# salesforce/LayoutDETR

Measured on AMD Instinct MI355X. Metric: images/sec G+D fwd-bwd, 256x256 bg x9 elems, higher is better.
Workload: dtype f32

## Files before the change

include/ldetr_hip.h:

```cpp
#ifndef LDETR_HIP_H
#define LDETR_HIP_H

#include <stdint.h>

#ifdef __cplusplus
extern "C" {
#endif

const char* ldetr_last_error(void);
int ldetr_abi_version(void);

int ldetr_debug_trace_tiles(int64_t* buffer);

int ldetr_set_split_bf16(int tiles);

int ldetr_engine_launch_counts(int64_t* f32_pipe, int64_t* bf16_split_pipe);

int ldetr_set_workspace(void* ptr, int64_t bytes);

typedef struct ldetr_tensor4 {
    int N, C, H, W;
    int64_t sn, sc, sh, sw;
} ldetr_tensor4;

typedef struct ldetr_epilogue {
    float alpha;
    const float* col_scale;
    const float* col_bias;
    const float* samp_scale;
    int64_t samp_ld;
    const float* residual;
    int64_t ldr;
    int act;
    float act_alpha;
    float act_gain;
    const float* mask_src;
    int64_t ldm;
    int mask_mode;
    float out_scale;
    float p_drop;
    uint64_t seed;
    const uint64_t* seed_ptr;
    int accumulate;
    float* a_rowsum;
} ldetr_epilogue;

int ldetr_bias_act_f32(const float* x, const float* b, const float* xref, const float* yref, const float* dy, float* y,
                       int64_t sizeX, int sizeB, int64_t stepB, int grad, int act, float alpha, float gain, float clamp,
                       void* stream);

int ldetr_upfirdn2d_f32(const float* x, const float* f, float* y, int N, int C, int inH, int inW,
                        const int64_t* x_strides_nchw, int fh, int fw, int64_t f_stride_h, int64_t f_stride_w,
                        int upx, int upy, int downx, int downy, int padx0, int padx1, int pady0, int pady1, int flip,
                        float gain, int outH, int outW, const int64_t* y_strides_nchw,
                        const float* act_bias, int has_act, float act_alpha, float act_gain, void* stream);

int ldetr_gemm_f32(const float* A, int64_t lda, int ta, const float* B, int64_t ldb, int tb, float* C, int64_t ldc,
                   int M, int N, int K, int splitk, const ldetr_epilogue* ep, int pix_per_sample, void* stream);

typedef struct ldetr_gemm_desc {
    const float* A; int64_t lda; int ta;
    const float* B; int64_t ldb; int tb;
    float* C; int64_t ldc;
    int M, N, K, splitk;
    const ldetr_epilogue* ep;
    int pix_per_sample;
} ldetr_gemm_desc;
int ldetr_gemm_pair_f32(const ldetr_gemm_desc* g0, const ldetr_gemm_desc* g1, void* stream);
int ldetr_gemm_pair_is_single_launch(const ldetr_gemm_desc* g0, const ldetr_gemm_desc* g1);

#define LDETR_GEMM_GROUP_MAX 32
int ldetr_gemm_small_group_f32(const ldetr_gemm_desc* g, const float* post_scale, int n, void* stream);

int ldetr_conv2d_fwd_f32(const float* x, const ldetr_tensor4* xt, const float* w, int Cout, int KH, int KW, int stride,
                         int pad, float* y, int64_t ldy, int OH, int OW, const float* in_scale, int64_t in_scale_ld,
                         const ldetr_epilogue* ep, void* stream);
int ldetr_conv2d_bwd_data_f32(const float* dy, const ldetr_tensor4* dyt, const float* w, int Cin, int KH, int KW,
                              int stride, int pad, float* dx, int64_t lddx, int IH, int IW, const float* dy_scale,
                              int64_t dy_scale_ld, const ldetr_epilogue* ep, void* stream);
int ldetr_conv2d_bwd_weight_f32(const float* x, const ldetr_tensor4* xt, const float* dy, const ldetr_tensor4* dyt,
                                float* dw, int KH, int KW, int stride, int pad, int splitk, const float* x_scale,
                                int64_t x_scale_ld, const float* dy_scale, int64_t dy_scale_ld, int accumulate, void* stream);

int ldetr_conv_transpose2d_fwd_f32(const float* x, const ldetr_tensor4* xt, const float* w, int Cout, int KH, int KW,
                                   int stride, int pad, float* y, int64_t ldy, int OH, int OW, const float* in_scale,
                                   int64_t in_scale_ld, const ldetr_epilogue* ep, void* stream);
int ldetr_conv_transpose2d_bwd_data_f32(const float* dy, const ldetr_tensor4* dyt, const float* w, int Cin, int KH,
                                        int KW, int stride, int pad, float* dx, int64_t lddx, int IH, int IW,
                                        const float* dy_scale, int64_t dy_scale_ld, const ldetr_epilogue* ep,
                                        void* stream);
int ldetr_conv_transpose2d_bwd_weight_f32(const float* x, const ldetr_tensor4* xt, const float* dy,
                                          const ldetr_tensor4* dyt, float* dw, int KH, int KW, int stride, int pad,
                                          int splitk, const float* x_scale, int64_t x_scale_ld, const float* dy_scale,
                                          int64_t dy_scale_ld, int accumulate, void* stream);

int ldetr_attention_fwd_f32(const float* q, int64_t ldq, const float* k, int64_t ldk, const float* v, int64_t ldv,
                            const unsigned char* key_padding_mask, float* out, int64_t ldo, float* lse, int B, int H,
                            int Lq, int Lk, int head_dim, float scale, float p_drop, uint64_t seed, const uint64_t* seed_ptr,
                            int causal, void* stream);
int ldetr_attention_bwd_f32(const float* q, int64_t ldq, const float* k, int64_t ldk, const float* v, int64_t ldv,
                            const unsigned char* key_padding_mask, const float* out, int64_t ldo, const float* lse,
                            const float* dout, int64_t lddo, float* dq, int64_t lddq, float* dk, int64_t lddk,
                            float* dv, int64_t lddv, int B, int H, int Lq, int Lk, int head_dim, float scale,
                            float p_drop, uint64_t seed, const uint64_t* seed_ptr, int causal, void* stream);

int ldetr_torgb_bwd_finish_f32(const float* dws, const float* s, const float* w, int B, int C, float* dw, float* ds, void* stream);

int ldetr_loss_combine_fwd_f32(const float* const* x, const float* w, const int* n, const int* fn, const int* red, int K, int ld,
                               float* vals, float* sums, float* total, void* stream);
int ldetr_loss_combine_bwd_f32(const float* const* x, const float* w, const int* n, const int* fn, const int* red, int K, int ld,
                               const float* g, float* grads, void* stream);
int ldetr_masked_mse_fwd_f32(const float* a, const float* b, const uint8_t* valid, int64_t rows, int D, int bdiv, float* out2, void* stream);
int ldetr_masked_mse_bwd_f32(const float* a, const float* b, const uint8_t* valid, int64_t rows, int D, int bdiv, const float* out2,
                             const float* g, float* da, void* stream);

typedef struct ldetr_ln_args {
    const float* x; const float* r; const float* gamma; const float* beta;
    float* y; float* z; float* mean; float* rstd;
    const float* dy; float* dx; float* dr; float* dgamma; float* dbeta;
    int64_t rows; int D; float eps, p_drop; uint64_t seed; const uint64_t* seed_ptr;
    const float* pos; int64_t pos_rows; float* ypos; const float* dy2;
    int r_parts; int64_t r_part_stride; const float* r_bias;
    const float* dy_parts; int dy_nparts; int64_t dy_part_stride;
} ldetr_ln_args;
int ldetr_layernorm_fwd_group_f32(const ldetr_ln_args* a, int n, void* stream);
int ldetr_layernorm_bwd_group_f32(const ldetr_ln_args* a, int n, void* stream);
int ldetr_sum_parts_f32(const float* base, const float* parts, int n_parts, int64_t part_stride, float* out, int64_t n, void* stream);

typedef struct ldetr_ffn_args {
    const float* x; int64_t ldx;
    const float* w1; const float* b1;
    const float* w2;
    float* h;
    float* ypart;
    int M, F;
    float p_drop; uint64_t seed; const uint64_t* seed_ptr;
    const float* dy;
    float* dxpart;
    float* dh;
} ldetr_ffn_args;
int ldetr_ffn_fwd_group_f32(const ldetr_ffn_args* a, int n, void* stream);
int ldetr_ffn_bwd_group_f32(const ldetr_ffn_args* a, int n, void* stream);

typedef struct ldetr_mha_small_args {
    const float* x; int64_t ldx;
    const float* w_in; const float* b_in; const float* w_out;
    const unsigned char* kpm;
    float* qkv; float* o; float* lse; float* ypart;
    int B, L;
    float scale, p_drop; uint64_t seed; const uint64_t* seed_ptr;
    const float* dr;
    float* dqkv; float* dxpart;
} ldetr_mha_small_args;
int ldetr_mha_small_fwd_group_f32(const ldetr_mha_small_args* a, int n, void* stream);
int ldetr_mha_small_bwd_group_f32(const ldetr_mha_small_args* a, int n, void* stream);

typedef struct ldetr_mha_cross_args {
    const float* x; int64_t ldx;
    const float* w_q; const float* b_q;
    const float* k; int64_t ldk; const float* v; int64_t ldv;
    const float* w_out;
    const unsigned char* kpm;
    float* q; float* o; float* lse; float* ypart;
    int B, Lq, Lk;
    float scale, p_drop; uint64_t seed; const uint64_t* seed_ptr;
    const float* dr;
    float* dq; float* dk; int64_t lddk; float* dv; int64_t lddv; float* dxpart;
} ldetr_mha_cross_args;
int ldetr_mha_cross_fwd_f32(const ldetr_mha_cross_args* a, void* stream);
int ldetr_mha_cross_bwd_f32(const ldetr_mha_cross_args* a, void* stream);

typedef struct ldetr_wgrad_desc {
    const float* A; int64_t lda; const float* B; int64_t ldb;
    float* dW; int64_t ldw; float* db;
    int M, rows, cols;
} ldetr_wgrad_desc;
int ldetr_wgrad_multi_f32(const ldetr_wgrad_desc* d, int n, void* stream);

int ldetr_colsum_f32(const float* a, float* red, int B, int64_t P, int C, void* stream);
int ldetr_act_bwd_reduce_f32(const float* dy, const float* y, float* dv, const float* bias, const float* demod,
                             float* dbias, float* ddemod, int B, int64_t P, int C, int act, float alpha, float gain,
                             void* stream);
int ldetr_mul_reduce_f32(const float* a, const float* x, const float* scale, float* out, float* red, int B, int64_t P,
                         int C, void* stream);
int ldetr_torgb_fwd_f32(const float* x, const float* w, const float* styles, const float* bias, float* y,
                        int B, int64_t P, int C, void* stream);
int ldetr_torgb_fwd_add_f32(const float* x, const float* w, const float* styles, const float* bias, const float* addend, float* y,
                            int B, int64_t P, int C, void* stream);
int ldetr_torgb_bwd_f32(const float* x, const float* dy, const float* w, const float* styles, float* dx, float* dws,
                        float* dbias, int B, int64_t P, int C, void* stream);
int ldetr_sg2_handoff_f32(const float* dxs, const float* x, const float* dy_rgb, float* dv, const float* s_conv, const float* s_rgb,
                          const float* w_rgb, const float* bias, const float* demod, float* ds_conv, float* dws_rgb, float* dbias_rgb,
                          float* dbias, float* ddemod, int B, int64_t P, int C, float alpha, float gain, void* stream);

int ldetr_maxpool3x3s2_fwd_f32(const float* x, float* y, unsigned char* idx, int N, int H, int W, int C, void* stream);
int ldetr_maxpool3x3s2_bwd_f32(const float* dy, const unsigned char* idx, float* dx, int N, int H, int W, int C,
                               void* stream);

int ldetr_grad_sanitize_f32(float* g, int64_t n, float scale, float nan_value, float posinf, float neginf,
                            void* stream);
int ldetr_adam_step_f32(float* p, const float* g, float* m, float* v, int64_t n, int64_t step, float lr, float beta1,
                        float beta2, float eps, int fuse_sanitize, float gscale, float nan_value, float posinf,
                        float neginf, void* stream);
int ldetr_adam_ema_step_f32(float* p, const float* g, float* m, float* v, int64_t n, int64_t step, float lr, float beta1, float beta2,
                            float eps, int fuse_sanitize, float gscale, float nan_value, float posinf, float neginf,
                            float* p_ema, float ema_beta, void* stream);
int ldetr_ema_lerp_f32(float* p_ema, const float* p, int64_t n, float beta, void* stream);

int ldetr_softmax_xent_fwd_f32(const float* logits, int64_t ld, const int64_t* targets, float* row_lse, float* loss_sum, float* count,
                               int64_t rows, int V, int64_t ignore_index, float label_smoothing, void* stream);
int ldetr_softmax_xent_bwd_f32(const float* logits, int64_t ld, const int64_t* targets, const float* row_lse, const float* count,
                               const float* grad_out, float* dlogits, int64_t ldd, int64_t rows, int V, int64_t ignore_index,
                               float label_smoothing, void* stream);

int ldetr_embedding_fwd_f32(const float* weight, const float* pos, const int64_t* ids, float* out, int64_t n, int d, int V, int T,
                            void* stream);
int ldetr_embedding_bwd_f32(const float* dy, const int64_t* ids, float* dweight, int64_t n, int d, int V, int64_t padding_idx,
                            void* stream);

int ldetr_resample_coeffs(int in_size, int out_size, int32_t* bounds, int32_t* weights, int64_t weights_capacity, int* ksize_out);
int ldetr_resize_normalize_u8(const uint8_t* src, int64_t images, int H, int W, int out_h, int out_w, const int32_t* hbounds,
                              const int32_t* hweights, int hksize, const int32_t* vbounds, const int32_t* vweights, int vksize,
                              uint8_t* tmp, uint8_t* out_u8, float* out_chw, float mean0, float mean1, float mean2, float std0,
                              float std1, float std2, void* stream);

#define LDETR_PAGE_FILTER_BLUR 1
#define LDETR_PAGE_FILTER_EDGE 2
int ldetr_page_filter_u8(const uint8_t* src, uint8_t* dst, int64_t images, int H, int W, int kind, float radius, void* stream);

int ldetr_demod_fwd_f32(const float* weight, int64_t so, int64_t si, int64_t sh, int64_t sw, const float* styles, float* dcoefs,
                        float* w2, int B, int O, int I, int KH, int KW, float eps, void* stream);
int ldetr_demod_bwd_f32(const float* weight, int64_t so, int64_t si, int64_t sh, int64_t sw, const float* styles, const float* dcoefs,
                        const float* w2, const float* grad_dcoefs, float* dweight, int accumulate_dweight, float* dstyles, int B, int O,
                        int I, int KH, int KW, void* stream);

#define LDETR_DEMOD_GROUP_MAX 24
typedef struct ldetr_demod_desc {
    const float* weight; int64_t so, si, sh, sw;
    const float* styles; float* dcoefs; float* w2;
    const float* grad_dcoefs; float* dweight; float* dstyles;
    int O, I, KH, KW;
} ldetr_demod_desc;
int ldetr_demod_group_fwd_f32(const ldetr_demod_desc* layers, int n, int B, float eps, void* stream);
int ldetr_demod_group_bwd_f32(const ldetr_demod_desc* layers, int n, int B, int accumulate_dweight, int add_dstyles, void* stream);

#define LDETR_AFFINE_GROUP_MAX 32
typedef struct ldetr_affine_desc {
    const float* ds; const float* A; float* dA; float* db;
    int C; float scale; float post;
} ldetr_affine_desc;
int ldetr_sg2_affine_bwd_f32(const ldetr_affine_desc* layers, int n, const float* latent, float* dlatent, int accumulate_dlatent,
                             float* scratch, int64_t scratch_floats, int B, int D, void* stream);

int ldetr_layout_losses_f32(const float* bbox, const float* bbox_ref, const uint8_t* valid, int B, int N, float* losses,
                            float* grads, void* stream);
int ldetr_layout_losses_bwd_f32(const float* grads, const float* grad_losses, int B, int N, float* dbbox, void* stream);

int ldetr_layout_finish_f32(const float* bbox_in, const int* num, const float* factors, const unsigned char* jitter, const unsigned char* mode,
                            float* bbox_out, float* overlap, float* alignment, int* order, int C, int K, int N, void* stream);

#define LDETR_FILTER_BILINEAR 0
#define LDETR_FILTER_LANCZOS 1
typedef struct ldetr_layout_raster_args {
    int struct_bytes;
    int B, N, S, nrow, n_colors, n_pages;
    const float* bbox;
    const uint8_t* valid;
    const int32_t* labels;
    const uint8_t* palette;
    const int32_t* page_wh;
    const uint8_t* pages;
    int64_t pages_bytes;
    const int64_t* page_table;
    const int32_t* page_index;
    const int32_t* coeffs;
    int64_t coeffs_len;
    const int64_t* cell_coeffs;
    int32_t* cells_dev;
    uint8_t* out;
} ldetr_layout_raster_args;
int ldetr_resample_coeffs_filter(int filter, int in_size, int out_size, int32_t* bounds, int32_t* weights, int64_t weights_capacity, int* ksize_out);
int ldetr_layout_raster_cell_size(int W, int H, int S, int* wn_out, int* hn_out);
int ldetr_layout_raster_u8(const ldetr_layout_raster_args* a, void* stream);

typedef struct ldetr_patch_resize_args {
    int struct_bytes;
    int n_jobs;
    const uint8_t* src0;
    int64_t src0_bytes;
    const uint8_t* src1;
    int64_t src1_bytes;
    uint8_t* dst;
    int64_t dst_bytes;
    const int64_t* jobs;
    const int32_t* tables;
    const int32_t* tables_host;
    int64_t tables_len;
    int32_t* jobs_dev;
} ldetr_patch_resize_args;
typedef struct ldetr_image_raster_args {
    int struct_bytes;
    int B, N, S, nrow;
    const float* bbox;
    const uint8_t* valid;
    const int32_t* rects;
    const int64_t* patch_off;
    const int64_t* page_off;
    const int32_t* page_wh;
    const uint8_t* pixels;
    int64_t pixels_bytes;
    const int32_t* coeffs;
    int64_t coeffs_len;
    const int64_t* cell_coeffs;
    int32_t* cells_dev;
    uint8_t* out;
} ldetr_image_raster_args;
int ldetr_patch_resize_u8(const ldetr_patch_resize_args* a, void* stream);
int ldetr_image_raster_u8(const ldetr_image_raster_args* a, void* stream);

#define LDETR_PNG_NOT_ELIGIBLE 3
#define LDETR_PNG_MALFORMED 4
typedef struct ldetr_png_decode_args {
    int struct_bytes;
    int n, H, W;
    int phases;
    int reserved;
    const uint8_t* files;
    int64_t files_bytes;
    const int64_t* file_off;
    const int64_t* file_off_dev;
    const int64_t* segments;
    const int64_t* segments_dev;
    int64_t n_segments;
    const int32_t* jobs;
    const int32_t* jobs_dev;
    int64_t n_jobs;
    uint8_t* scratch;
    int64_t scratch_bytes;
    uint8_t* dst;
} ldetr_png_decode_args;
int ldetr_png_scan(const uint8_t* file, int64_t file_bytes, int* width, int* height, int* channels, int64_t* segments, int64_t segments_capacity,
                   int64_t* segments_count, int32_t* row_starts, int64_t row_starts_capacity, int64_t* row_starts_count);
int ldetr_png_decode_u8(const ldetr_png_decode_args* a, void* stream);

typedef struct ldetr_png_encode_args {
    int struct_bytes;
    int H, W;
    int blocks;
    int filter;
    int reserved;
    const uint8_t* src;
    uint8_t* out;
    int64_t out_capacity;
    int64_t* total_bytes;
    uint8_t* workspace;
    int64_t workspace_bytes;
    int64_t* seg_table;
    int64_t seg_table_rows;
} ldetr_png_encode_args;
int ldetr_png_encode_bound(int H, int W, int64_t* out_bytes, int64_t* workspace_bytes);
int ldetr_png_encode_u8(const ldetr_png_encode_args* a, void* stream);
int ldetr_png_index_bytes(int H, int W, int64_t* bytes);

#define LDETR_PNG_INFLATE_CODE 1
#define LDETR_PNG_INFLATE_COUNT 2
#define LDETR_PNG_INFLATE_HEADER 4
#define LDETR_PNG_INFLATE_DISTANCE 8
#define LDETR_PNG_INFLATE_TRAILER 16
#define LDETR_PNG_INFLATE_FILTER 32
#define LDETR_PNG_INFLATE_STUCK 64
#define LDETR_PNG_INFLATE_TABLE 128
typedef struct ldetr_png_inflate_args {
    int struct_bytes;
    int n, H, W;
    int phases;
    int reserved;
    const uint8_t* files;
    int64_t files_bytes;
    const int64_t* file_off;
    const int64_t* file_off_dev;
    const int64_t* segments;
    const int64_t* segments_dev;
    const int64_t* index_off;
    const int64_t* index_off_dev;
    const int32_t* jobs;
    const int32_t* jobs_dev;
    int64_t n_jobs;
    uint8_t* scratch;
    int64_t scratch_bytes;
    uint8_t* dst;
    int32_t* status;
} ldetr_png_inflate_args;
int ldetr_png_scan_packed(const uint8_t* file, int64_t file_bytes, int* width, int* height, int64_t* segments, int64_t segments_capacity, int64_t* segments_count,
                          int64_t* index_offset, int32_t* row_starts, int64_t row_starts_capacity, int64_t* row_starts_count);
int ldetr_png_inflate_u8(const ldetr_png_inflate_args* a, void* stream);

int ldetr_lsap_f64(const double* cost, int batch, int n, int maximize, int* row_ind, int* col_ind, void* stream);

int ldetr_layoutnet_features_f32(const float* bbox, const int64_t* label, const uint8_t* padding_mask, const int* label_map, int map_len,
                                 const float* weights, int64_t weights_len, int num_label, int B, int N, float* out, void* stream);

int ldetr_layoutnet_forward_f32(const float* bbox, const int64_t* label, const uint8_t* padding_mask, const float* enc_weights,
                                int64_t enc_len, const float* dec_weights, int64_t dec_len, int num_label, int B, int N,
                                float* logit_disc, float* logit_cls, float* bbox_pred, float* features, void* stream);

int ldetr_feature_stats_f64(const float* x, int64_t n, int F, double* raw_mean, double* raw_cov, void* stream);

int ldetr_box_giou_pairwise_f32(const float* boxes1, const float* boxes2, int B, int N, int M, int cxcywh, float* iou, float* uni,
                                float* giou, double* cost, double cost_sign, void* stream);

int ldetr_bmm_strided_f32(const float* A, const int64_t* sa, const float* B, const int64_t* sb, float* C, const int64_t* sc,
                          int nb1, int nb2, int M, int N, int K, float alpha, void* stream);

int ldetr_p3_split_f32(const float* src, int64_t ld, void* dst, int64_t rows, int C, void* stream);
int ldetr_p3_merge_f32(const void* src, float* dst, int64_t ld, int64_t rows, int C, void* stream);
int ldetr_p3_weight_bwd(const float* w_ohwi, const float* o_scale, void* dst, int O, int KH, int KW, int I, void* stream);

int ldetr_p3_weight_prep(const int64_t* table_dev, int nconv, int total_blocks, void* stream);

typedef struct ldetr_p3_epilogue {
    float alpha;
    const float* col_scale;
    const float* col_bias;
    const void* residual_p3;
    const float* residual_f32;
    const void* relu_mask_p3;
    int relu;
} ldetr_p3_epilogue;

int ldetr_p3_conv2d_fwd(const void* x, int N, int H, int W, int Cin, const void* w, int Cout, int KH, int KW, int stride, int pad,
                        const ldetr_p3_epilogue* ep, void* out_p3, float* out_f32, void* stream);
int ldetr_p3_conv2d_fwd_dual(const void* x1, const void* x2, int N, int H, int W, int Cin, const void* w1, const void* w2, int Cout, int KH, int KW,
                             int stride, int pad, const ldetr_p3_epilogue* ep1, const ldetr_p3_epilogue* ep2, void* out1_p3, float* out1_f32,
                             void* out2_p3, float* out2_f32, void* stream);
int ldetr_p3_conv2d_bwd_data(const void* dy, int N, int OH, int OW, int Cout, const void* wb, int Cin, int KH, int KW, int stride, int pad,
                             int IH, int IW, const ldetr_p3_epilogue* ep, void* out_p3, float* out_f32, void* stream);
int ldetr_p3_conv2d_bwd_weight(const void* x, int N, int H, int W, int Cin, const void* dy, int Cout, int KH, int KW, int stride, int pad,
                               const float* dy_scale, float* dw, void* stream);
int ldetr_p3_conv2d_bwd_pair(const void* dy, int N, int OH, int OW, int Cout, const void* wb, const void* x, int Cin, int KH, int KW, int stride, int pad,
                             int IH, int IW, const ldetr_p3_epilogue* ep, void* dx_p3, float* dx_f32, const float* dy_scale, float* dw,
                             int* launches, void* stream);

int ldetr_struct_sizes(int32_t* out6);

int ldetr_p3_last_launch(int32_t* info10);

int ldetr_engine_last_launch(int32_t* info10);

#ifdef __cplusplus
}
#endif
#endif
```

layoutdetr_amd/_lib.py:

```python
import ctypes
import os
from ctypes import (POINTER, Structure, c_char_p, c_double, c_float, c_int, c_int64, c_ubyte, c_uint64, c_void_p)

_HERE = os.path.dirname(os.path.abspath(__file__))
ABI_VERSION = 25
LIB_PATH = os.environ.get('LDETR_LIB') or os.path.join(_HERE, 'lib', 'libldetr_hip.so')


class Tensor4(Structure):
    _fields_ = [('N', c_int), ('C', c_int), ('H', c_int), ('W', c_int),
                ('sn', c_int64), ('sc', c_int64), ('sh', c_int64), ('sw', c_int64)]


class GemmDesc(Structure):
    _fields_ = [('A', c_void_p), ('lda', c_int64), ('ta', c_int), ('B', c_void_p), ('ldb', c_int64), ('tb', c_int),
                ('C', c_void_p), ('ldc', c_int64), ('M', c_int), ('N', c_int), ('K', c_int), ('splitk', c_int),
                ('ep', c_void_p), ('pix_per_sample', c_int)]


class P3Epilogue(Structure):
    _fields_ = [('alpha', c_float), ('col_scale', c_void_p), ('col_bias', c_void_p), ('residual_p3', c_void_p),
                ('residual_f32', c_void_p), ('relu_mask_p3', c_void_p), ('relu', c_int)]


class Epilogue(Structure):
    _fields_ = [('alpha', c_float), ('col_scale', c_void_p), ('col_bias', c_void_p), ('samp_scale', c_void_p),
                ('samp_ld', c_int64), ('residual', c_void_p), ('ldr', c_int64), ('act', c_int),
                ('act_alpha', c_float), ('act_gain', c_float), ('mask_src', c_void_p), ('ldm', c_int64),
                ('mask_mode', c_int), ('out_scale', c_float), ('p_drop', c_float), ('seed', c_uint64),
                ('seed_ptr', c_void_p), ('accumulate', c_int), ('a_rowsum', c_void_p)]


class LnArgs(Structure):
    _fields_ = [('x', c_void_p), ('r', c_void_p), ('gamma', c_void_p), ('beta', c_void_p),
                ('y', c_void_p), ('z', c_void_p), ('mean', c_void_p), ('rstd', c_void_p),
                ('dy', c_void_p), ('dx', c_void_p), ('dr', c_void_p), ('dgamma', c_void_p), ('dbeta', c_void_p),
                ('rows', c_int64), ('D', c_int), ('eps', c_float), ('p_drop', c_float), ('seed', c_uint64), ('seed_ptr', c_void_p),
                ('pos', c_void_p), ('pos_rows', c_int64), ('ypos', c_void_p), ('dy2', c_void_p),
                ('r_parts', c_int), ('r_part_stride', c_int64), ('r_bias', c_void_p),
                ('dy_parts', c_void_p), ('dy_nparts', c_int), ('dy_part_stride', c_int64)]


class FfnArgs(Structure):
    _fields_ = [('x', c_void_p), ('ldx', c_int64), ('w1', c_void_p), ('b1', c_void_p), ('w2', c_void_p), ('h', c_void_p), ('ypart', c_void_p),
                ('M', c_int), ('F', c_int), ('p_drop', c_float), ('seed', c_uint64), ('seed_ptr', c_void_p),
                ('dy', c_void_p), ('dxpart', c_void_p), ('dh', c_void_p)]


class MhaSmallArgs(Structure):
    _fields_ = [('x', c_void_p), ('ldx', c_int64), ('w_in', c_void_p), ('b_in', c_void_p), ('w_out', c_void_p), ('kpm', c_void_p),
                ('qkv', c_void_p), ('o', c_void_p), ('lse', c_void_p), ('ypart', c_void_p), ('B', c_int), ('L', c_int),
                ('scale', c_float), ('p_drop', c_float), ('seed', c_uint64), ('seed_ptr', c_void_p),
                ('dr', c_void_p), ('dqkv', c_void_p), ('dxpart', c_void_p)]


class MhaCrossArgs(Structure):
    _fields_ = [('x', c_void_p), ('ldx', c_int64), ('w_q', c_void_p), ('b_q', c_void_p), ('k', c_void_p), ('ldk', c_int64), ('v', c_void_p), ('ldv', c_int64),
                ('w_out', c_void_p), ('kpm', c_void_p), ('q', c_void_p), ('o', c_void_p), ('lse', c_void_p), ('ypart', c_void_p),
                ('B', c_int), ('Lq', c_int), ('Lk', c_int), ('scale', c_float), ('p_drop', c_float), ('seed', c_uint64), ('seed_ptr', c_void_p),
                ('dr', c_void_p), ('dq', c_void_p), ('dk', c_void_p), ('lddk', c_int64), ('dv', c_void_p), ('lddv', c_int64), ('dxpart', c_void_p)]


class WgradDesc(Structure):
    _fields_ = [('A', c_void_p), ('lda', c_int64), ('B', c_void_p), ('ldb', c_int64), ('dW', c_void_p), ('ldw', c_int64), ('db', c_void_p),
                ('M', c_int), ('rows', c_int), ('cols', c_int)]


class DemodDesc(Structure):
    _fields_ = [('weight', c_void_p), ('so', c_int64), ('si', c_int64), ('sh', c_int64), ('sw', c_int64),
                ('styles', c_void_p), ('dcoefs', c_void_p), ('w2', c_void_p), ('grad_dcoefs', c_void_p), ('dweight', c_void_p), ('dstyles', c_void_p),
                ('O', c_int), ('I', c_int), ('KH', c_int), ('KW', c_int)]


class AffineDesc(Structure):
    _fields_ = [('ds', c_void_p), ('A', c_void_p), ('dA', c_void_p), ('db', c_void_p), ('C', c_int), ('scale', c_float), ('post', c_float)]


class LayoutRasterArgs(Structure):
    _fields_ = [('struct_bytes', c_int), ('B', c_int), ('N', c_int), ('S', c_int), ('nrow', c_int), ('n_colors', c_int), ('n_pages', c_int),
                ('bbox', c_void_p), ('valid', c_void_p), ('labels', c_void_p), ('palette', c_void_p), ('page_wh', c_void_p),
                ('pages', c_void_p), ('pages_bytes', c_int64), ('page_table', c_void_p), ('page_index', c_void_p),
                ('coeffs', c_void_p), ('coeffs_len', c_int64), ('cell_coeffs', c_void_p), ('cells_dev', c_void_p), ('out', c_void_p)]


class PatchResizeArgs(Structure):
    _fields_ = [('struct_bytes', c_int), ('n_jobs', c_int), ('src0', c_void_p), ('src0_bytes', c_int64), ('src1', c_void_p), ('src1_bytes', c_int64),
                ('dst', c_void_p), ('dst_bytes', c_int64), ('jobs', c_void_p), ('tables', c_void_p), ('tables_host', c_void_p), ('tables_len', c_int64),
                ('jobs_dev', c_void_p)]


class ImageRasterArgs(Structure):
    _fields_ = [('struct_bytes', c_int), ('B', c_int), ('N', c_int), ('S', c_int), ('nrow', c_int),
                ('bbox', c_void_p), ('valid', c_void_p), ('rects', c_void_p), ('patch_off', c_void_p), ('page_off', c_void_p), ('page_wh', c_void_p),
                ('pixels', c_void_p), ('pixels_bytes', c_int64), ('coeffs', c_void_p), ('coeffs_len', c_int64), ('cell_coeffs', c_void_p),
                ('cells_dev', c_void_p), ('out', c_void_p)]


class PngDecodeArgs(Structure):
    _fields_ = [('struct_bytes', c_int), ('n', c_int), ('H', c_int), ('W', c_int), ('phases', c_int), ('reserved', c_int),
                ('files', c_void_p), ('files_bytes', c_int64), ('file_off', c_void_p), ('file_off_dev', c_void_p),
                ('segments', c_void_p), ('segments_dev', c_void_p), ('n_segments', c_int64),
                ('jobs', c_void_p), ('jobs_dev', c_void_p), ('n_jobs', c_int64),
                ('scratch', c_void_p), ('scratch_bytes', c_int64), ('dst', c_void_p)]


class PngEncodeArgs(Structure):
    _fields_ = [('struct_bytes', c_int), ('H', c_int), ('W', c_int), ('blocks', c_int), ('filter', c_int), ('reserved', c_int),
                ('src', c_void_p), ('out', c_void_p), ('out_capacity', c_int64), ('total_bytes', c_void_p),
                ('workspace', c_void_p), ('workspace_bytes', c_int64), ('seg_table', c_void_p), ('seg_table_rows', c_int64)]


class PngInflateArgs(Structure):
    _fields_ = [('struct_bytes', c_int), ('n', c_int), ('H', c_int), ('W', c_int), ('phases', c_int), ('reserved', c_int),
                ('files', c_void_p), ('files_bytes', c_int64), ('file_off', c_void_p), ('file_off_dev', c_void_p),
                ('segments', c_void_p), ('segments_dev', c_void_p), ('index_off', c_void_p), ('index_off_dev', c_void_p),
                ('jobs', c_void_p), ('jobs_dev', c_void_p), ('n_jobs', c_int64),
                ('scratch', c_void_p), ('scratch_bytes', c_int64), ('dst', c_void_p), ('status', c_void_p)]


_P = c_void_p
_I = c_int
_L = c_int64
_F = c_float
_T4 = POINTER(Tensor4)
_EP = POINTER(Epilogue)

SIGNATURES = {
    'ldetr_set_workspace': [_P, _L],
    'ldetr_bias_act_f32': [_P, _P, _P, _P, _P, _P, _L, _I, _L, _I, _I, _F, _F, _F, _P],
    'ldetr_upfirdn2d_f32': [_P, _P, _P, _I, _I, _I, _I, POINTER(c_int64), _I, _I, _L, _L, _I, _I, _I, _I, _I, _I, _I, _I,
                            _I, _F, _I, _I, POINTER(c_int64), _P, _I, _F, _F, _P],
    'ldetr_gemm_f32': [_P, _L, _I, _P, _L, _I, _P, _L, _I, _I, _I, _I, _EP, _I, _P],
    'ldetr_conv2d_fwd_f32': [_P, _T4, _P, _I, _I, _I, _I, _I, _P, _L, _I, _I, _P, _L, _EP, _P],
    'ldetr_conv2d_bwd_data_f32': [_P, _T4, _P, _I, _I, _I, _I, _I, _P, _L, _I, _I, _P, _L, _EP, _P],
    'ldetr_conv2d_bwd_weight_f32': [_P, _T4, _P, _T4, _P, _I, _I, _I, _I, _I, _P, _L, _P, _L, _I, _P],
    'ldetr_conv_transpose2d_fwd_f32': [_P, _T4, _P, _I, _I, _I, _I, _I, _P, _L, _I, _I, _P, _L, _EP, _P],
    'ldetr_conv_transpose2d_bwd_data_f32': [_P, _T4, _P, _I, _I, _I, _I, _I, _P, _L, _I, _I, _P, _L, _EP, _P],
    'ldetr_conv_transpose2d_bwd_weight_f32': [_P, _T4, _P, _T4, _P, _I, _I, _I, _I, _I, _P, _L, _P, _L, _I, _P],
    'ldetr_attention_fwd_f32': [_P, _L, _P, _L, _P, _L, _P, _P, _L, _P, _I, _I, _I, _I, _I, _F, _F, c_uint64, _P, _I, _P],
    'ldetr_attention_bwd_f32': [_P, _L, _P, _L, _P, _L, _P, _P, _L, _P, _P, _L, _P, _L, _P, _L, _P, _L,
                                _I, _I, _I, _I, _I, _F, _F, c_uint64, _P, _I, _P],
    'ldetr_colsum_f32': [_P, _P, _I, _L, _I, _P],
    'ldetr_act_bwd_reduce_f32': [_P, _P, _P, _P, _P, _P, _P, _I, _L, _I, _I, _F, _F, _P],
    'ldetr_mul_reduce_f32': [_P, _P, _P, _P, _P, _I, _L, _I, _P],
    'ldetr_torgb_fwd_f32': [_P, _P, _P, _P, _P, _I, _L, _I, _P],
    'ldetr_torgb_bwd_f32': [_P, _P, _P, _P, _P, _P, _P, _I, _L, _I, _P],
    'ldetr_maxpool3x3s2_fwd_f32': [_P, _P, _P, _I, _I, _I, _I, _P],
    'ldetr_maxpool3x3s2_bwd_f32': [_P, _P, _P, _I, _I, _I, _I, _P],
    'ldetr_grad_sanitize_f32': [_P, _L, _F, _F, _F, _F, _P],
    'ldetr_adam_step_f32': [_P, _P, _P, _P, _L, _L, _F, _F, _F, _F, _I, _F, _F, _F, _F, _P],
    'ldetr_adam_ema_step_f32': [_P, _P, _P, _P, _L, _L, _F, _F, _F, _F, _I, _F, _F, _F, _F, _P, _F, _P],
    'ldetr_ema_lerp_f32': [_P, _P, _L, _F, _P],
    'ldetr_lsap_f64': [_P, _I, _I, _I, _P, _P, _P],
    'ldetr_layoutnet_features_f32': [_P, _P, _P, POINTER(c_int), _I, _P, _L, _I, _I, _I, _P, _P],
    'ldetr_layoutnet_forward_f32': [_P, _P, _P, _P, _L, _P, _L, _I, _I, _I, _P, _P, _P, _P, _P],
    'ldetr_feature_stats_f64': [_P, _L, _I, _P, _P, _P],
    'ldetr_box_giou_pairwise_f32': [_P, _P, _I, _I, _I, _I, _P, _P, _P, _P, c_double, _P],
    'ldetr_bmm_strided_f32': [_P, _P, _P, _P, _P, _P, _I, _I, _I, _I, _I, _F, _P],
    'ldetr_softmax_xent_fwd_f32': [_P, _L, _P, _P, _P, _P, _L, _I, _L, _F, _P],
    'ldetr_softmax_xent_bwd_f32': [_P, _L, _P, _P, _P, _P, _P, _L, _L, _I, _L, _F, _P],
    'ldetr_embedding_fwd_f32': [_P, _P, _P, _P, _L, _I, _I, _I, _P],
    'ldetr_embedding_bwd_f32': [_P, _P, _P, _L, _I, _I, _L, _P],
    'ldetr_debug_trace_tiles': [_P],
    'ldetr_set_split_bf16': [c_int],
    'ldetr_engine_launch_counts': [POINTER(c_int64), POINTER(c_int64)],
    'ldetr_layernorm_fwd_group_f32': [_P, _I, _P],
    'ldetr_layernorm_bwd_group_f32': [_P, _I, _P],
    'ldetr_sum_parts_f32': [_P, _P, _I, _L, _P, _L, _P],
    'ldetr_ffn_fwd_group_f32': [_P, _I, _P],
    'ldetr_ffn_bwd_group_f32': [_P, _I, _P],
    'ldetr_mha_small_fwd_group_f32': [_P, _I, _P],
    'ldetr_mha_small_bwd_group_f32': [_P, _I, _P],
    'ldetr_mha_cross_fwd_f32': [_P, _P],
    'ldetr_mha_cross_bwd_f32': [_P, _P],
    'ldetr_wgrad_multi_f32': [_P, _I, _P],
    'ldetr_loss_combine_fwd_f32': [_P, _P, _P, _P, _P, _I, _I, _P, _P, _P, _P],
    'ldetr_loss_combine_bwd_f32': [_P, _P, _P, _P, _P, _I, _I, _P, _P, _P],
    'ldetr_masked_mse_fwd_f32': [_P, _P, _P, _L, _I, _I, _P, _P],
    'ldetr_masked_mse_bwd_f32': [_P, _P, _P, _L, _I, _I, _P, _P, _P, _P],
    'ldetr_torgb_bwd_finish_f32': [_P, _P, _P, _I, _I, _P, _P, _P],
    'ldetr_sg2_handoff_f32': [_P, _P, _P, _P, _P, _P, _P, _P, _P, _P, _P, _P, _P, _P, _I, _L, _I, _F, _F, _P],
    'ldetr_gemm_pair_f32': [_P, _P, _P],
    'ldetr_gemm_pair_is_single_launch': [_P, _P],
    'ldetr_demod_fwd_f32': [_P, _L, _L, _L, _L, _P, _P, _P, _I, _I, _I, _I, _I, _F, _P],
    'ldetr_demod_bwd_f32': [_P, _L, _L, _L, _L, _P, _P, _P, _P, _P, _I, _P, _I, _I, _I, _I, _I, _P],
    'ldetr_demod_group_fwd_f32': [_P, _I, _I, _F, _P],
    'ldetr_demod_group_bwd_f32': [_P, _I, _I, _I, _I, _P],
    'ldetr_sg2_affine_bwd_f32': [_P, _I, _P, _P, _I, _P, _L, _I, _I, _P],
    'ldetr_gemm_small_group_f32': [_P, _P, _I, _P],
    'ldetr_torgb_fwd_add_f32': [_P, _P, _P, _P, _P, _P, _I, _L, _I, _P],
    'ldetr_layout_losses_f32': [_P, _P, _P, _I, _I, _P, _P, _P],
    'ldetr_layout_losses_bwd_f32': [_P, _P, _I, _I, _P, _P],
    'ldetr_layout_finish_f32': [_P, _P, _P, _P, _P, _P, _P, _P, _P, _I, _I, _I, _P],
    'ldetr_resample_coeffs': [_I, _I, _P, _P, _L, _P],
    'ldetr_resample_coeffs_filter': [_I, _I, _I, _P, _P, _L, _P],
    'ldetr_layout_raster_cell_size': [_I, _I, _I, _P, _P],
    'ldetr_layout_raster_u8': [_P, _P],
    'ldetr_patch_resize_u8': [_P, _P],
    'ldetr_image_raster_u8': [_P, _P],
    'ldetr_p3_split_f32': [_P, _L, _P, _L, _I, _P],
    'ldetr_p3_merge_f32': [_P, _P, _L, _L, _I, _P],
    'ldetr_p3_weight_bwd': [_P, _P, _P, _I, _I, _I, _I, _P],
    'ldetr_p3_conv2d_bwd_data': [_P, _I, _I, _I, _I, _P, _I, _I, _I, _I, _I, _I, _I, _P, _P, _P, _P],
    'ldetr_p3_conv2d_fwd': [_P, _I, _I, _I, _I, _P, _I, _I, _I, _I, _I, _P, _P, _P, _P],
    'ldetr_p3_conv2d_bwd_weight': [_P, _I, _I, _I, _I, _P, _I, _I, _I, _I, _I, _P, _P, _P],
    'ldetr_p3_weight_prep': [_P, _I, _I, _P],
    'ldetr_p3_conv2d_fwd_dual': [_P, _P, _I, _I, _I, _I, _P, _P, _I, _I, _I, _I, _I, _P, _P, _P, _P, _P, _P, _P],
    'ldetr_p3_conv2d_bwd_pair': [_P, _I, _I, _I, _I, _P, _P, _I, _I, _I, _I, _I, _I, _I, _P, _P, _P, _P, _P, _P, _P],
    'ldetr_p3_last_launch': [_P],
    'ldetr_engine_last_launch': [_P],
    'ldetr_struct_sizes': [_P],
    'ldetr_resize_normalize_u8': [_P, _L, _I, _I, _I, _I, _P, _P, _I, _P, _P, _I, _P, _P, _P, _F, _F, _F, _F, _F, _F, _P],
    'ldetr_page_filter_u8': [_P, _P, _L, _I, _I, _I, _F, _P],
    'ldetr_png_scan': [_P, _L, _P, _P, _P, _P, _L, _P, _P, _L, _P],
    'ldetr_png_decode_u8': [_P, _P],
    'ldetr_png_encode_bound': [_I, _I, _P, _P],
    'ldetr_png_encode_u8': [_P, _P],
    'ldetr_png_index_bytes': [_I, _I, _P],
    'ldetr_png_scan_packed': [_P, _L, _P, _P, _P, _L, _P, _P, _P, _L, _P],
    'ldetr_png_inflate_u8': [_P, _P],
}

_lib = None


def load():
    global _lib
    if _lib is not None:
        return _lib
    if not os.path.exists(LIB_PATH):
        raise RuntimeError(
            f'{LIB_PATH} not found: build the gfx950 kernels first (python -m layoutdetr_amd.build or '
            f'__graft_entry__.build()).  layoutdetr_amd has no CPU/PyTorch fallback path.')
    import torch
    lib = ctypes.CDLL(LIB_PATH)
    lib.ldetr_last_error.restype = c_char_p
    lib.ldetr_last_error.argtypes = []
    lib.ldetr_abi_version.restype = c_int
    lib.ldetr_abi_version.argtypes = []
    for name, argtypes in SIGNATURES.items():
        fn = getattr(lib, name)
        fn.restype = c_int
        fn.argtypes = argtypes
    if lib.ldetr_abi_version() != ABI_VERSION:
        raise RuntimeError('libldetr_hip.so ABI version mismatch; rebuild it')
    sizes = (ctypes.c_int32 * 6)()
    lib.ldetr_struct_sizes(sizes)
    mirror = [ctypes.sizeof(t) for t in (LnArgs, FfnArgs, MhaSmallArgs, MhaCrossArgs, WgradDesc, P3Epilogue)]
    if list(sizes) != mirror:
        raise RuntimeError(f'libldetr_hip.so argument blocks {list(sizes)} do not match the ctypes mirror {mirror}; rebuild')
    _lib = lib
    return lib


def check(rc, what=''):
    if rc != 0:
        msg = load().ldetr_last_error().decode('utf-8', 'replace')
        raise RuntimeError(f'{what}: {msg}' if what else msg)
```

layoutdetr_amd/build.py:

```python
import hashlib
import os
import shutil
import subprocess
import sys
from concurrent.futures import ThreadPoolExecutor

HERE = os.path.dirname(os.path.abspath(__file__))
CSRC = os.path.join(HERE, 'csrc')
LIBDIR = os.path.join(HERE, 'lib')
OBJDIR = os.path.join(LIBDIR, 'obj')
LIBNAME = 'libldetr_hip.so'
ARCH = 'gfx950'

SOURCES = ['ldetr_core.cpp', 'bias_act.hip', 'upfirdn2d.hip', 'gemm_conv.hip', 'attention.hip', 'layernorm.hip',
           'misc_ops.hip', 'optim.hip', 'lsap.hip', 'xent.hip', 'resample.hip', 'layout_loss.hip', 'demod.hip', 'sg2_affine.hip', 'wgrad_smallc.hip', 'stem_conv.hip', 'box_ops.hip', 'ffn_fused.hip', 'conv_c32.hip', 'mha_small.hip', 'p3_engine.hip', 'bmm_strided.hip', 'layoutnet.hip', 'layoutnet_train.hip', 'layout_finish.hip', 'layout_raster.hip', 'page_filter.hip', 'patch_resize.hip', 'png_decode.hip', 'png_encode.hip', 'png_inflate.hip']
HEADERS = ['ldetr_common.hpp', 'layoutnet_layers.hpp', 'pil_resample.hpp', 'png_pages.hpp', 'png_inflate_kernel.hpp', os.path.join('..', '..', 'include', 'ldetr_hip.h')]

FLAGS = ([] if os.environ.get('LDETR_TILE_TRACE') else ['-DLDETR_TILE_TRACE=0']) + (['-DP3_TRACE'] if os.environ.get('LDETR_P3_TRACE') else []) + ['-O3', '-std=c++17', '-fPIC', f'--offload-arch={ARCH}', '-munsafe-fp-atomics', '-fno-gpu-rdc',
         '-Wno-unused-result', '-Rpass-analysis=kernel-resource-usage']
NO_SCRATCH = ('wgrad_c32_3x3_kernel', 'gemm_f32_kernel', 'gemm_small_kernel', 'gemm_small_group_kernel', 'demod_group', 'sg2_affine_bwd', 'attn_fwd_kernel', 'attn_fwd_wide_kernel', 'attn_bwd_kernel', 'ffn_fwd_kernel', 'ffn_bwd_kernel', 'conv3x3_c32_kernel', 'mha_small_fwd_kernel', 'mha_cross_fwd_kernel', 'mha_small_bwd_kernel', 'mha_cross_bwd_kernel', 'wgrad_multi_kernel', 'ln_fwd_kernel', 'ln_bwd_kernel', 'p3_nt_kernel', 'p3_tn_kernel', 'p3_c3_kernel', 'p3_bwd_pair', 'layoutnet_features_kernel', 'layoutnet_forward_kernel', 'feature_stats_f64_kernel', 'layout_finish_kernel', 'layout_raster_kernel', 'page_blur_kernel', 'page_edge_kernel', 'patch_resize_kernel', 'sg2_handoff_kernel', 'png_gather_kernel', 'png_unfilter_kernel', 'png_enc_filter_kernel', 'png_enc_deflate_kernel', 'png_enc_assemble_kernel', 'png_inflate_kernel')


def _hipcc():
    for cand in (os.environ.get('HIPCC'), shutil.which('hipcc'), '/opt/rocm/bin/hipcc'):
        if cand and os.path.exists(cand):
            return cand
    raise RuntimeError('hipcc not found: the gfx950 kernel library cannot be built')


def _digest(paths):
    h = hashlib.sha256()
    for p in paths:
        with open(p, 'rb') as f:
            h.update(f.read())
    h.update(' '.join(FLAGS).encode())
    return h.hexdigest()


def _kernel_resources(remarks):
    out, cur = {}, None
    for line in remarks.splitlines():
        if 'remark:' not in line:
            continue
        body = line.split('remark:', 1)[1].split('[-Rpass-analysis', 1)[0].strip()
        if body.startswith('Function Name:'):
            cur = body.split(':', 1)[1].strip()
            out[cur] = {}
        elif cur is not None and ':' in body:
            k, v = body.rsplit(':', 1)
            out[cur][k.strip()] = v.strip()
    return out


def source_digest():
    return _digest(sorted(os.path.join(CSRC, f) for f in os.listdir(CSRC) if f.endswith(('.hip', '.cpp', '.hpp')) and not f.startswith('.'))
                   + [os.path.normpath(os.path.join(CSRC, HEADERS[-1]))])


def lib_path():
    return os.path.join(LIBDIR, LIBNAME)


def build(force=False, verbose=True):
    os.makedirs(OBJDIR, exist_ok=True)
    hipcc = _hipcc()
    hdrs = [os.path.normpath(os.path.join(CSRC, h)) for h in HEADERS]
    objs, jobs = [], []
    for src in SOURCES:
        sp = os.path.join(CSRC, src)
        obj = os.path.join(OBJDIR, src + '.o')
        stamp = obj + '.sha'
        dig = _digest([sp] + hdrs)
        objs.append(obj)
        if not force and os.path.exists(obj) and os.path.exists(stamp) and open(stamp).read() == dig:
            continue
        jobs.append((sp, obj, stamp, dig))

    def compile_one(job):
        sp, obj, stamp, dig = job
        cmd = [hipcc] + FLAGS + ['-x', 'hip', '-c', sp, '-o', obj]
        if verbose:
            print('[ldetr build]', os.path.basename(sp), flush=True)
        r = subprocess.run(cmd, capture_output=True, text=True)
        if r.returncode != 0:
            raise RuntimeError(f'hipcc failed for {sp}:\n{r.stdout}\n{r.stderr}')
        res = _kernel_resources(r.stderr)
        with open(obj + '.resources.txt', 'w') as f:
            for name, d in res.items():
                f.write(f"{name} vgprs={d.get('VGPRs', '?')} agprs={d.get('AGPRs', '?')} scratch={d.get('ScratchSize [bytes/lane]', '?')} "
                        f"occupancy={d.get('Occupancy [waves/SIMD]', '?')} lds={d.get('LDS Size [bytes/block]', '?')}\n")
        bad = [n for n, d in res.items() if any(k in n for k in NO_SCRATCH) and d.get('ScratchSize [bytes/lane]', '0') != '0']
        if bad:
            raise RuntimeError(f'{os.path.basename(sp)}: scratch memory in register-budgeted kernels: ' + ', '.join(bad[:4]))
        with open(stamp, 'w') as f:
            f.write(dig)

    if jobs:
        with ThreadPoolExecutor(max_workers=min(8, len(jobs))) as ex:
            list(ex.map(compile_one, jobs))
    out = lib_path()
    if jobs or not os.path.exists(out):
        cmd = [hipcc, '-shared', '-fPIC', f'--offload-arch={ARCH}', '-fno-gpu-rdc', '-o', out] + objs
        r = subprocess.run(cmd, capture_output=True, text=True)
        if r.returncode != 0:
            raise RuntimeError(f'link failed:\n{r.stdout}\n{r.stderr}')
        if verbose:
            print('[ldetr build] linked', out, flush=True)
    return out


if __name__ == '__main__':
    build(force='--force' in sys.argv)
```

layoutdetr_amd/csrc/ffn_fused.hip:

```cpp
#include "ldetr_common.hpp"
#include "../../include/ldetr_hip.h"

namespace ldetr {

typedef ldetr_ffn_args FfnParams;

constexpr int FD = 256, FHS = 64, FHP = 68;

typedef __attribute__((__vector_size__(16 * sizeof(float)))) float ffn_acc_t;

__device__ __forceinline__ void ld_k16(const __amdgpu_buffer_rsrc_t& rs, int voff, int soff, float (&f)[16]) {
#pragma unroll
    for (int j = 0; j < 4; j++) {
        const auto v = __builtin_amdgcn_raw_buffer_load_b128(rs, voff + 16 * j, soff, 0);
        f[4 * j] = __int_as_float(v[0]); f[4 * j + 1] = __int_as_float(v[1]); f[4 * j + 2] = __int_as_float(v[2]); f[4 * j + 3] = __int_as_float(v[3]);
    }
}
__device__ __forceinline__ void ld_r16(const __amdgpu_buffer_rsrc_t& rs, int voff, int soff, int ld4, float (&f)[16]) {
#pragma unroll
    for (int t = 0; t < 16; t++) f[t] = __int_as_float(__builtin_amdgcn_raw_buffer_load_b32(rs, voff, soff + t * ld4, 0));
}
__device__ __forceinline__ __amdgpu_buffer_rsrc_t rsrc(const float* p) {
    return __builtin_amdgcn_make_buffer_rsrc(const_cast<float*>(p), 0, 0x7fffffff, 0x00020000);
}
#define FFN_MFMA16(A, B, ACC) _Pragma("unroll") for (int t_ = 0; t_ < 16; t_++) ACC = __builtin_amdgcn_mfma_f32_32x32x2f32(A[t_], B[t_], ACC, 0, 0, 0)

__global__ __launch_bounds__(256) void ffn_fwd_kernel(FfnParams pa, FfnParams pb, int nb0) {
    __shared__ float red[2][32][33];
    __shared__ float Hs[32][FHP];
    const bool second = (int)blockIdx.x >= nb0;
    const FfnParams& p = second ? pb : pa;
    const int bid = second ? (int)blockIdx.x - nb0 : (int)blockIdx.x, gx = (p.M + 31) >> 5;
    const int tid = threadIdx.x, lane = tid & 63, wave = tid >> 6, cl = lane & 31, kl = lane >> 5;
    const int s = bid / gx, m0 = (bid - s * gx) * 32, j0 = s * FHS;
    const int OOB = (int)0x80000000;
    const int ct = wave & 1, kh = wave >> 1;
    float b2[2][2][16];
    {
        const __amdgpu_buffer_rsrc_t rsX = rsrc(p.x), rsW = rsrc(p.w1), rsW2 = rsrc(p.w2);
        const int vA = (m0 + cl < p.M) ? (int)(((long)(m0 + cl) * p.ldx + kh * 128 + 16 * kl) * 4) : OOB;
        const int vB = ((j0 + ct * 32 + cl) * FD + kh * 128 + 16 * kl) * 4;
        ffn_acc_t acc;
#pragma unroll
        for (int r = 0; r < 16; r++) acc[r] = 0.f;
        float a[4][16], b[4][16];
#pragma unroll
        for (int c = 0; c < 4; c++) { ld_k16(rsX, vA, c * 128, a[c]); ld_k16(rsW, vB, c * 128, b[c]); }
#pragma unroll
        for (int q = 0; q < 2; q++)
#pragma unroll
            for (int c = 0; c < 2; c++) ld_k16(rsW2, (((wave * 2 + q) * 32 + cl) * p.F + j0 + 16 * kl) * 4, c * 128, b2[q][c]);
        __builtin_amdgcn_sched_barrier(0);
#pragma unroll
        for (int c = 0; c < 4; c++) FFN_MFMA16(a[c], b[c], acc);
        if (kh == 1) {
#pragma unroll
            for (int r = 0; r < 16; r++) red[ct][(r & 3) + 8 * (r >> 2) + 4 * kl][cl] = acc[r];
        }
        __syncthreads();
        if (kh == 0) {
            const float bias = p.b1[j0 + ct * 32 + cl];
            const float inv_keep = p.p_drop > 0.f ? 1.f / (1.f - p.p_drop) : 1.f;
            const uint64_t seed = p.seed + (p.seed_ptr ? *p.seed_ptr : 0ull);
#pragma unroll
            for (int r = 0; r < 16; r++) {
                const int row = (r & 3) + 8 * (r >> 2) + 4 * kl;
                float v = acc[r] + red[ct][row][cl] + bias;
                v = v > 0.f ? v : 0.f;
                const long m = m0 + row;
                if (p.p_drop > 0.f) v *= drop_scale(seed, (uint64_t)(m * p.F + j0 + ct * 32 + cl), p.p_drop, inv_keep);
                Hs[row][ct * 32 + cl] = v;
                if (m < p.M) p.h[m * p.F + j0 + ct * 32 + cl] = v;
            }
        }
        __syncthreads();
    }
    {
        ffn_acc_t acc[2];
#pragma unroll
        for (int q = 0; q < 2; q++)
#pragma unroll
            for (int r = 0; r < 16; r++) acc[q][r] = 0.f;
#pragma unroll
        for (int c = 0; c < 2; c++) {
            float a[16];
#pragma unroll
            for (int t = 0; t < 16; t++) a[t] = Hs[cl][c * 32 + 16 * kl + t];
            FFN_MFMA16(a, b2[0][c], acc[0]);
            FFN_MFMA16(a, b2[1][c], acc[1]);
        }
        float* dst = p.ypart + ((long)s * p.M) * FD;
#pragma unroll
        for (int q = 0; q < 2; q++)
#pragma unroll
            for (int r = 0; r < 16; r++) {
                const long m = m0 + (r & 3) + 8 * (r >> 2) + 4 * kl;
                if (m < p.M) dst[m * FD + (wave * 2 + q) * 32 + cl] = acc[q][r];
            }
    }
}

__global__ __launch_bounds__(256) void ffn_bwd_kernel(FfnParams pa, FfnParams pb, int nb0) {
    __shared__ float red[2][32][33];
    __shared__ float dHs[32][FHP];
    const bool second = (int)blockIdx.x >= nb0;
    const FfnParams& p = second ? pb : pa;
    const int bid = second ? (int)blockIdx.x - nb0 : (int)blockIdx.x, gx = (p.M + 31) >> 5;
    const int tid = threadIdx.x, lane = tid & 63, wave = tid >> 6, cl = lane & 31, kl = lane >> 5;
    const int s = bid / gx, m0 = (bid - s * gx) * 32, j0 = s * FHS;
    const int OOB = (int)0x80000000;
    const __amdgpu_buffer_rsrc_t rsDY = rsrc(p.dy), rsW1 = rsrc(p.w1), rsW2 = rsrc(p.w2), rsX = rsrc(p.x);
    const float inv_keep = p.p_drop > 0.f ? 1.f / (1.f - p.p_drop) : 1.f;
    float b2[2][2][16];
    {
        const int ct = wave & 1, kh = wave >> 1;
        const int vA = (m0 + cl < p.M) ? ((m0 + cl) * FD + kh * 128 + 16 * kl) * 4 : OOB;
        const int vB = (j0 + ct * 32 + cl + (kh * 128 + 16 * kl) * p.F) * 4;
        const int ld4 = p.F * 4;
        ffn_acc_t acc;
#pragma unroll
        for (int r = 0; r < 16; r++) acc[r] = 0.f;
        float a[4][16], b[4][16];
#pragma unroll
        for (int c = 0; c < 4; c++) { ld_k16(rsDY, vA, c * 128, a[c]); ld_r16(rsW2, vB, c * 32 * ld4, ld4, b[c]); }
#pragma unroll
        for (int q = 0; q < 2; q++)
#pragma unroll
            for (int c = 0; c < 2; c++)
                ld_r16(rsW1, ((wave * 2 + q) * 32 + cl + (j0 + c * 32 + 16 * kl) * FD) * 4, 0, FD * 4, b2[q][c]);
        float hvs[16];
#pragma unroll
        for (int r = 0; r < 16; r++) {
            const long m = m0 + (r & 3) + 8 * (r >> 2) + 4 * kl;
            hvs[r] = (kh == 0 && m < p.M) ? p.h[m * p.F + j0 + ct * 32 + cl] : 0.f;
        }
        __builtin_amdgcn_sched_barrier(0);
#pragma unroll
        for (int c = 0; c < 4; c++) FFN_MFMA16(a[c], b[c], acc);
        if (kh == 1) {
#pragma unroll
            for (int r = 0; r < 16; r++) red[ct][(r & 3) + 8 * (r >> 2) + 4 * kl][cl] = acc[r];
        }
        __syncthreads();
        if (kh == 0) {
#pragma unroll
            for (int r = 0; r < 16; r++) {
                const int row = (r & 3) + 8 * (r >> 2) + 4 * kl;
                const long m = m0 + row;
                const float hv = hvs[r];
                const float dh = hv > 0.f ? (acc[r] + red[ct][row][cl]) * inv_keep : 0.f;
                dHs[row][ct * 32 + cl] = dh;
                if (p.dh && m < p.M) p.dh[m * p.F + j0 + ct * 32 + cl] = dh;
            }
        }
        __syncthreads();
    }
    {
        ffn_acc_t acc[2];
#pragma unroll
        for (int q = 0; q < 2; q++)
#pragma unroll
            for (int r = 0; r < 16; r++) acc[q][r] = 0.f;
#pragma unroll
        for (int c = 0; c < 2; c++) {
            float a[16];
#pragma unroll
            for (int t = 0; t < 16; t++) a[t] = dHs[cl][c * 32 + 16 * kl + t];
            FFN_MFMA16(a, b2[0][c], acc[0]);
            FFN_MFMA16(a, b2[1][c], acc[1]);
        }
        float* dst = p.dxpart + ((long)s * p.M) * FD;
#pragma unroll
        for (int q = 0; q < 2; q++)
#pragma unroll
            for (int r = 0; r < 16; r++) {
                const long m = m0 + (r & 3) + 8 * (r >> 2) + 4 * kl;
                if (m < p.M) dst[m * FD + (wave * 2 + q) * 32 + cl] = acc[q][r];
            }
    }
}

}

using namespace ldetr;

static int ffn_check_args(const char* what, const FfnParams& p, bool bwd) {
    LDETR_CHECK(p.F >= FHS && p.F % FHS == 0, "%s: hidden width must be a multiple of 64 (got %d)", what, p.F);
    LDETR_CHECK(p.M >= 0 && p.M <= (1 << 20), "%s: bad row count", what);
    LDETR_CHECK(p.x && p.ldx >= FD && p.ldx % 4 == 0 && (((uintptr_t)p.x) & 15) == 0, "%s: x must be 16-byte aligned rows with a pitch that is a multiple of 4", what);
    LDETR_CHECK((long)p.M * p.ldx * 4 < 0x7fffffffL && (long)p.M * p.F * 4 < 0x7fffffffL && (long)(p.F / FHS) * p.M * FD * 4 < 0x7fffffffL, "%s: operand above 2 GiB", what);
    if (!bwd) {
        LDETR_CHECK(p.w1 && p.b1 && p.w2 && p.h && p.ypart, "%s: null pointer", what);
        LDETR_CHECK(p.p_drop >= 0.f && p.p_drop < 1.f, "%s: p_drop out of range", what);
    } else {
        LDETR_CHECK(p.dy && p.h && p.w1 && p.w2 && p.dxpart, "%s: null pointer", what);
        LDETR_CHECK((((uintptr_t)p.dy) & 15) == 0, "%s: dy must be 16-byte aligned", what);
    }
    return LDETR_OK;
}

static int ffn_launch(const ldetr_ffn_args* a, int n, bool bwd, void* stream) {
    const char* what = bwd ? "ffn_bwd" : "ffn_fwd";
    LDETR_CHECK(a && (n == 1 || n == 2), "%s: 1 or 2 problems", what);
    FfnParams p[2]; p[0] = a[0]; p[1] = n == 2 ? a[1] : a[0];
    int nb[2] = {0, 0};
    for (int i = 0; i < n; i++) {
        if (int rc = ffn_check_args(what, p[i], bwd)) return rc;
        nb[i] = cdiv(p[i].M, 32) * (p[i].F / FHS);
    }
    if (nb[0] + nb[1] == 0) return LDETR_OK;
    if (bwd) hipLaunchKernelGGL(ffn_bwd_kernel, dim3(nb[0] + nb[1]), dim3(256), 0, (hipStream_t)stream, p[0], p[1], nb[0]);
    else hipLaunchKernelGGL(ffn_fwd_kernel, dim3(nb[0] + nb[1]), dim3(256), 0, (hipStream_t)stream, p[0], p[1], nb[0]);
    count_engine_launch(false);
    return check_launch(what);
}

extern "C" int ldetr_ffn_fwd_group_f32(const ldetr_ffn_args* a, int n, void* stream) { return ffn_launch(a, n, false, stream); }
extern "C" int ldetr_ffn_bwd_group_f32(const ldetr_ffn_args* a, int n, void* stream) { return ffn_launch(a, n, true, stream); }
```

layoutdetr_amd/csrc/layernorm.hip:

```cpp
#include "ldetr_common.hpp"
#include "../../include/ldetr_hip.h"

namespace ldetr {

typedef ldetr_ln_args LnParams;

template <int NV>
__global__ __launch_bounds__(256) void ln_fwd_kernel(LnParams pa, LnParams pb, int nb0) {
    const bool second = (int)blockIdx.x >= nb0;
    const LnParams& p = second ? pb : pa;
    const int lane = threadIdx.x & 63, wave = threadIdx.x >> 6;
    const long row = (long)(second ? (int)blockIdx.x - nb0 : (int)blockIdx.x) * 4 + wave;
    if (row >= p.rows) return;
    const int D4 = p.D >> 2;
    const float inv_keep = p.p_drop > 0.f ? 1.f / (1.f - p.p_drop) : 1.f;
    const uint64_t seed = p.seed + (p.seed_ptr ? *p.seed_ptr : 0ull);
    float4 v[NV];
    float s = 0.f;
#pragma unroll
    for (int i = 0; i < NV; i++) {
        int c4 = lane + i * 64;
        v[i] = make_float4(0.f, 0.f, 0.f, 0.f);
        if (c4 < D4) {
            v[i] = reinterpret_cast<const float4*>(p.x + row * p.D)[c4];
            if (p.r) {
                float4 rr = reinterpret_cast<const float4*>(p.r + row * p.D)[c4];
                if (p.r_parts > 0) {
                    if (p.r_bias) { const float4 bb = reinterpret_cast<const float4*>(p.r_bias)[c4]; rr.x += bb.x; rr.y += bb.y; rr.z += bb.z; rr.w += bb.w; }
                    constexpr int PW = NV == 1 ? 16 : 8;
                    for (int s = 1; s < p.r_parts; s += PW) {
                        float4 q[PW];
#pragma unroll
                        for (int j = 0; j < PW; j++)
                            q[j] = (s + j < p.r_parts) ? reinterpret_cast<const float4*>(p.r + (s + j) * p.r_part_stride + row * p.D)[c4] : make_float4(0.f, 0.f, 0.f, 0.f);
#pragma unroll
                        for (int j = 0; j < PW; j++)
                            if (s + j < p.r_parts) { rr.x += q[j].x; rr.y += q[j].y; rr.z += q[j].z; rr.w += q[j].w; }
                    }
                }
                if (p.p_drop > 0.f) {
                    uint64_t e = (uint64_t)row * p.D + (c4 << 2);
                    rr.x *= drop_scale(seed, e, p.p_drop, inv_keep);
                    rr.y *= drop_scale(seed, e + 1, p.p_drop, inv_keep);
                    rr.z *= drop_scale(seed, e + 2, p.p_drop, inv_keep);
                    rr.w *= drop_scale(seed, e + 3, p.p_drop, inv_keep);
                }
                v[i].x += rr.x; v[i].y += rr.y; v[i].z += rr.z; v[i].w += rr.w;
            }
            if (p.z) reinterpret_cast<float4*>(p.z + row * p.D)[c4] = v[i];
            s += v[i].x + v[i].y + v[i].z + v[i].w;
        }
    }
    const float mean = wave_sum(s) / p.D;
    float q = 0.f;
#pragma unroll
    for (int i = 0; i < NV; i++) {
        int c4 = lane + i * 64;
        if (c4 < D4) {
            float a = v[i].x - mean, b = v[i].y - mean, c = v[i].z - mean, d = v[i].w - mean;
            q += a * a + b * b + c * c + d * d;
        }
    }
    const float rstd = rsqrtf(wave_sum(q) / p.D + p.eps);
    if (lane == 0) { if (p.mean) p.mean[row] = mean; if (p.rstd) p.rstd[row] = rstd; }
#pragma unroll
    for (int i = 0; i < NV; i++) {
        int c4 = lane + i * 64;
        if (c4 < D4) {
            float4 g = reinterpret_cast<const float4*>(p.gamma)[c4];
            float4 b = reinterpret_cast<const float4*>(p.beta)[c4];
            float4 o;
            o.x = (v[i].x - mean) * rstd * g.x + b.x; o.y = (v[i].y - mean) * rstd * g.y + b.y;
            o.z = (v[i].z - mean) * rstd * g.z + b.z; o.w = (v[i].w - mean) * rstd * g.w + b.w;
            reinterpret_cast<float4*>(p.y + row * p.D)[c4] = o;
            if (p.ypos) {
                const float4 pp = reinterpret_cast<const float4*>(p.pos + (row % p.pos_rows) * p.D)[c4];
                o.x += pp.x; o.y += pp.y; o.z += pp.z; o.w += pp.w;
                reinterpret_cast<float4*>(p.ypos + row * p.D)[c4] = o;
            }
        }
    }
}

template <int NV, int WAVES>
__global__ __launch_bounds__(WAVES * 64) void ln_bwd_kernel(LnParams pa, LnParams pb, int nb0) {
    __shared__ float red[2][WAVES][256 * NV];
    const bool second = (int)blockIdx.x >= nb0;
    const LnParams& p = second ? pb : pa;
    const int bx = second ? (int)blockIdx.x - nb0 : (int)blockIdx.x, gx = second ? (int)gridDim.x - nb0 : nb0;
    const int lane = threadIdx.x & 63, wave = threadIdx.x >> 6;
    const int D4 = p.D >> 2;
    const float inv_keep = p.p_drop > 0.f ? 1.f / (1.f - p.p_drop) : 1.f;
    const uint64_t seed = p.seed + (p.seed_ptr ? *p.seed_ptr : 0ull);
    float4 ag[NV], ab[NV];
#pragma unroll
    for (int i = 0; i < NV; i++) { ag[i] = make_float4(0.f, 0.f, 0.f, 0.f); ab[i] = ag[i]; }
    for (long row = (long)bx * WAVES + wave; row < p.rows; row += (long)gx * WAVES) {
        const float mean = p.mean[row], rstd = p.rstd[row];
        float4 xh[NV], g[NV];
        float s1 = 0.f, s2 = 0.f;
#pragma unroll
        for (int i = 0; i < NV; i++) {
            int c4 = lane + i * 64;
            xh[i] = make_float4(0.f, 0.f, 0.f, 0.f); g[i] = xh[i];
            if (c4 < D4) {
                float4 zz = reinterpret_cast<const float4*>(p.z + row * p.D)[c4];
                float4 dy = reinterpret_cast<const float4*>(p.dy + row * p.D)[c4];
                if (p.dy2) {
                    const float4 d2 = reinterpret_cast<const float4*>(p.dy2 + row * p.D)[c4];
                    dy.x += d2.x; dy.y += d2.y; dy.z += d2.z; dy.w += d2.w;
                }
                constexpr int PW = NV == 1 ? 16 : 8;
                for (int s = 0; s < p.dy_nparts; s += PW) {
                    float4 q[PW];
#pragma unroll
                    for (int j = 0; j < PW; j++)
                        q[j] = (s + j < p.dy_nparts) ? reinterpret_cast<const float4*>(p.dy_parts + (s + j) * p.dy_part_stride + row * p.D)[c4] : make_float4(0.f, 0.f, 0.f, 0.f);
#pragma unroll
                    for (int j = 0; j < PW; j++)
                        if (s + j < p.dy_nparts) { dy.x += q[j].x; dy.y += q[j].y; dy.z += q[j].z; dy.w += q[j].w; }
                }
                float4 gm = reinterpret_cast<const float4*>(p.gamma)[c4];
                xh[i].x = (zz.x - mean) * rstd; xh[i].y = (zz.y - mean) * rstd;
                xh[i].z = (zz.z - mean) * rstd; xh[i].w = (zz.w - mean) * rstd;
                g[i].x = dy.x * gm.x; g[i].y = dy.y * gm.y; g[i].z = dy.z * gm.z; g[i].w = dy.w * gm.w;
                s1 += g[i].x + g[i].y + g[i].z + g[i].w;
                s2 += g[i].x * xh[i].x + g[i].y * xh[i].y + g[i].z * xh[i].z + g[i].w * xh[i].w;
                ag[i].x += dy.x * xh[i].x; ag[i].y += dy.y * xh[i].y; ag[i].z += dy.z * xh[i].z; ag[i].w += dy.w * xh[i].w;
                ab[i].x += dy.x; ab[i].y += dy.y; ab[i].z += dy.z; ab[i].w += dy.w;
            }
        }
        const float c1 = wave_sum(s1) / p.D, c2 = wave_sum(s2) / p.D;
#pragma unroll
        for (int i = 0; i < NV; i++) {
            int c4 = lane + i * 64;
            if (c4 < D4) {
                float4 dz;
                dz.x = rstd * (g[i].x - c1 - xh[i].x * c2); dz.y = rstd * (g[i].y - c1 - xh[i].y * c2);
                dz.z = rstd * (g[i].z - c1 - xh[i].z * c2); dz.w = rstd * (g[i].w - c1 - xh[i].w * c2);
                if (p.dx) reinterpret_cast<float4*>(p.dx + row * p.D)[c4] = dz;
                if (p.dr) {
                    if (p.p_drop > 0.f) {
                        uint64_t e = (uint64_t)row * p.D + (c4 << 2);
                        dz.x *= drop_scale(seed, e, p.p_drop, inv_keep);
                        dz.y *= drop_scale(seed, e + 1, p.p_drop, inv_keep);
                        dz.z *= drop_scale(seed, e + 2, p.p_drop, inv_keep);
                        dz.w *= drop_scale(seed, e + 3, p.p_drop, inv_keep);
                    }
                    reinterpret_cast<float4*>(p.dr + row * p.D)[c4] = dz;
                }
            }
        }
    }
    if (!p.dgamma) return;
#pragma unroll
    for (int i = 0; i < NV; i++) {
        int c = (lane + i * 64) << 2;
        red[0][wave][c + 0] = ag[i].x; red[0][wave][c + 1] = ag[i].y; red[0][wave][c + 2] = ag[i].z; red[0][wave][c + 3] = ag[i].w;
        red[1][wave][c + 0] = ab[i].x; red[1][wave][c + 1] = ab[i].y; red[1][wave][c + 2] = ab[i].z; red[1][wave][c + 3] = ab[i].w;
    }
    __syncthreads();
    for (int c = threadIdx.x; c < 2 * p.D; c += WAVES * 64) {
        const int k = c >= p.D, cc = c - k * p.D;
        float sum = red[k][0][cc];
#pragma unroll
        for (int w = 1; w < WAVES; w++) sum += red[k][w][cc];
        atomicAdd((k ? p.dbeta : p.dgamma) + cc, sum);
    }
}

}

using namespace ldetr;

static int ln_check_fwd(const LnParams& p) {
    LDETR_CHECK(p.r_parts >= 0 && (p.r_parts == 0 || (p.r && p.r_part_stride >= p.rows * p.D)), "layernorm_fwd: bad partial-sum arguments");
    LDETR_CHECK(p.x && p.gamma && p.beta && p.y, "layernorm_fwd: null pointer");
    LDETR_CHECK((p.pos == nullptr) == (p.ypos == nullptr) && (!p.pos || p.pos_rows > 0), "layernorm_fwd: pos, pos_rows and ypos go together");
    LDETR_CHECK(p.D % 4 == 0 && p.D >= 4 && p.D <= 1024, "layernorm_fwd: D must be a multiple of 4 in [4, 1024]");
    LDETR_CHECK(p.rows >= 0 && p.rows < (1L << 31) - 8, "layernorm_fwd: bad row count");
    return LDETR_OK;
}

extern "C" int ldetr_layernorm_fwd_group_f32(const ldetr_ln_args* a, int n, void* stream) {
    LDETR_CHECK(a && (n == 1 || n == 2), "layernorm_fwd_group: 1 or 2 problems");
    LnParams p[2]; p[0] = a[0]; p[1] = n == 2 ? a[1] : a[0];
    for (int i = 0; i < n; i++) {
        if (int rc = ln_check_fwd(p[i])) return rc;
        if (p[i].r_parts == 0) p[i].r_bias = nullptr;
    }
    LDETR_CHECK(n == 1 || p[0].D == p[1].D, "layernorm_fwd_group: both problems must have the same D");
    const int nb0 = (int)((p[0].rows + 3) / 4), nb1 = n == 2 ? (int)((p[1].rows + 3) / 4) : 0;
    if (nb0 + nb1 == 0) return LDETR_OK;
    hipStream_t st = (hipStream_t)stream;
    const int nv = (p[0].D + 255) / 256, grid = nb0 + nb1;
    if (nv == 1) hipLaunchKernelGGL(ln_fwd_kernel<1>, grid, 256, 0, st, p[0], p[1], nb0);
    else if (nv == 2) hipLaunchKernelGGL(ln_fwd_kernel<2>, grid, 256, 0, st, p[0], p[1], nb0);
    else if (nv == 3) hipLaunchKernelGGL(ln_fwd_kernel<3>, grid, 256, 0, st, p[0], p[1], nb0);
    else hipLaunchKernelGGL(ln_fwd_kernel<4>, grid, 256, 0, st, p[0], p[1], nb0);
    return check_launch("layernorm_fwd");
}

static int ln_check_bwd(const LnParams& p) {
    LDETR_CHECK(p.dy_nparts >= 0 && (p.dy_nparts == 0 || (p.dy_parts && p.dy_part_stride >= p.rows * p.D)), "layernorm_bwd: bad partial-sum arguments");
    LDETR_CHECK(p.dy && p.z && p.mean && p.rstd && p.gamma, "layernorm_bwd: null pointer");
    LDETR_CHECK(p.D % 4 == 0 && p.D >= 4 && p.D <= 1024, "layernorm_bwd: D must be a multiple of 4 in [4, 1024]");
    LDETR_CHECK((p.dgamma == nullptr) == (p.dbeta == nullptr), "layernorm_bwd: dgamma and dbeta go together");
    return LDETR_OK;
}

extern "C" int ldetr_layernorm_bwd_group_f32(const ldetr_ln_args* a, int n, void* stream) {
    LDETR_CHECK(a && (n == 1 || n == 2), "layernorm_bwd_group: 1 or 2 problems");
    LnParams p[2]; p[0] = a[0]; p[1] = n == 2 ? a[1] : a[0];
    for (int i = 0; i < n; i++)
        if (int rc = ln_check_bwd(p[i])) return rc;
    LDETR_CHECK(n == 1 || p[0].D == p[1].D, "layernorm_bwd_group: both problems must have the same D");
    static const long wide_rows = knob("LN_BWD_WIDE_ROWS", 256);
    const int nv = (p[0].D + 255) / 256;
    const int waves = nv == 1 && std::max<int64_t>(p[0].rows, n == 2 ? p[1].rows : 0) >= wide_rows ? 16 : 4;
    auto blocks = [waves](long rows) { long g = (rows + waves - 1) / waves; return (int)(g > 2048 / waves ? 2048 / waves : g); };
    const int nb0 = blocks(p[0].rows), nb1 = n == 2 ? blocks(p[1].rows) : 0;
    if (nb0 + nb1 == 0) return LDETR_OK;
    hipStream_t st = (hipStream_t)stream;
    const int grid = nb0 + nb1;
    if (waves == 16) hipLaunchKernelGGL((ln_bwd_kernel<1, 16>), grid, 1024, 0, st, p[0], p[1], nb0);
    else if (nv == 1) hipLaunchKernelGGL((ln_bwd_kernel<1, 4>), grid, 256, 0, st, p[0], p[1], nb0);
    else if (nv == 2) hipLaunchKernelGGL((ln_bwd_kernel<2, 4>), grid, 256, 0, st, p[0], p[1], nb0);
    else if (nv == 3) hipLaunchKernelGGL((ln_bwd_kernel<3, 4>), grid, 256, 0, st, p[0], p[1], nb0);
    else hipLaunchKernelGGL((ln_bwd_kernel<4, 4>), grid, 256, 0, st, p[0], p[1], nb0);
    return check_launch("layernorm_bwd");
}

__global__ __launch_bounds__(256) void sum_parts_kernel(const float4* __restrict__ base, const float4* __restrict__ parts, int n_parts, long part_stride4, float4* __restrict__ out, long n4) {
    for (long i = (long)blockIdx.x * 256 + threadIdx.x; i < n4; i += (long)gridDim.x * 256) {
        float4 v = base ? base[i] : make_float4(0.f, 0.f, 0.f, 0.f);
        for (int s = 0; s < n_parts; s += 8) {
            float4 q[8];
#pragma unroll
            for (int j = 0; j < 8; j++) q[j] = (s + j < n_parts) ? parts[(long)(s + j) * part_stride4 + i] : make_float4(0.f, 0.f, 0.f, 0.f);
#pragma unroll
            for (int j = 0; j < 8; j++)
                if (s + j < n_parts) { v.x += q[j].x; v.y += q[j].y; v.z += q[j].z; v.w += q[j].w; }
        }
        out[i] = v;
    }
}

extern "C" int ldetr_sum_parts_f32(const float* base, const float* parts, int n_parts, int64_t part_stride, float* out, int64_t n, void* stream) {
    LDETR_CHECK(out && n >= 0 && n % 4 == 0 && part_stride % 4 == 0 && n_parts >= 0 && (n_parts == 0 || parts), "sum_parts: bad arguments");
    LDETR_CHECK(((((uintptr_t)base) | ((uintptr_t)parts) | ((uintptr_t)out)) & 15) == 0, "sum_parts: buffers must be 16-byte aligned");
    if (n == 0) return LDETR_OK;
    const long n4 = n / 4;
    const int grid = (int)std::min<long>((n4 + 255) / 256, 1024);
    hipLaunchKernelGGL(sum_parts_kernel, grid, 256, 0, (hipStream_t)stream, (const float4*)base, (const float4*)parts, n_parts, (long)(part_stride / 4), (float4*)out, n4);
    return check_launch("sum_parts");
}
```

layoutdetr_amd/csrc/mha_small.hip:

```cpp
#include "ldetr_common.hpp"
#include "../../include/ldetr_hip.h"

namespace ldetr {

typedef ldetr_mha_small_args MhaSmallParams;

constexpr int MS_D = 256, MS_H = 8, MS_DH = 32;
constexpr int MS_RP = 97, MS_QP = 100, MS_OP = 36;

#define MS_MFMA16(a, b, c) __builtin_amdgcn_mfma_f32_16x16x4f32((a), (b), (c), 0, 0, 0)

__global__ __launch_bounds__(256) void mha_small_fwd_kernel(MhaSmallParams pa, MhaSmallParams pb, int nb0) {
    __shared__ float red[4 * 16 * MS_RP];
    __shared__ __attribute__((aligned(16))) float qs[16 * MS_QP];
    __shared__ __attribute__((aligned(16))) float os[16 * MS_OP];
    const bool second = (int)blockIdx.x >= nb0;
    const MhaSmallParams& p = second ? pb : pa;
    const int bid = second ? (int)blockIdx.x - nb0 : (int)blockIdx.x;
    const int tid = threadIdx.x, lane = tid & 63, w = tid >> 6, li = lane & 15, g = lane >> 4;
    const int b = bid / MS_H, h = bid - b * MS_H;
    const int L = p.L;
    const long row0 = (long)b * L;

    f32x4 wo[4][2];
#pragma unroll
    for (int t = 0; t < 4; t++)
#pragma unroll
        for (int gg = 0; gg < 2; gg++)
            wo[t][gg] = *reinterpret_cast<const f32x4*>(p.w_out + (long)(16 * (4 * w + t) + li) * MS_D + h * MS_DH + 16 * gg + 4 * g);

    f32x4 xa[4], wb[6][4];
    {
        const bool rok = li < L;
        const float* xr = p.x + (row0 + (rok ? li : 0)) * p.ldx + 64 * w + 4 * g;
#pragma unroll
        for (int gg = 0; gg < 4; gg++) {
            const f32x4 v = *reinterpret_cast<const f32x4*>(xr + 16 * gg);
            xa[gg] = rok ? v : f32x4{0.f, 0.f, 0.f, 0.f};
        }
#pragma unroll
        for (int ct = 0; ct < 6; ct++) {
            const float* wr = p.w_in + (long)((ct >> 1) * MS_D + h * MS_DH + (ct & 1) * 16 + li) * MS_D + 64 * w + 4 * g;
#pragma unroll
            for (int gg = 0; gg < 4; gg++) wb[ct][gg] = *reinterpret_cast<const f32x4*>(wr + 16 * gg);
        }
    }
    float bias6[6];
#pragma unroll
    for (int i = 0; i < 6; i++) {
        const int col = (tid + 256 * i) % 96;
        bias6[i] = p.b_in[(col >> 5) * MS_D + h * MS_DH + (col & 31)];
    }
    unsigned km = 0;
#pragma unroll
    for (int r = 0; r < 4; r++) {
        const int key = 4 * g + r;
        const bool masked = key >= L || (p.kpm && p.kpm[row0 + (key < L ? key : 0)]);
        km |= masked ? (1u << r) : 0u;
    }
    const uint64_t seed = p.seed + ((p.p_drop > 0.f && p.seed_ptr) ? *p.seed_ptr : 0ull);
    __builtin_amdgcn_sched_barrier(0);
    f32x4 acc[6];
#pragma unroll
    for (int ct = 0; ct < 6; ct++) acc[ct] = f32x4{0.f, 0.f, 0.f, 0.f};
#pragma unroll
    for (int gg = 0; gg < 4; gg++)
#pragma unroll
        for (int j = 0; j < 4; j++)
#pragma unroll
            for (int ct = 0; ct < 6; ct++) acc[ct] = MS_MFMA16(xa[gg][j], wb[ct][gg][j], acc[ct]);
#pragma unroll
    for (int ct = 0; ct < 6; ct++)
#pragma unroll
        for (int r = 0; r < 4; r++) red[(w * 16 + 4 * g + r) * MS_RP + 16 * ct + li] = acc[ct][r];
    __syncthreads();
#pragma unroll
    for (int i = 0; i < 6; i++) {
        const int e = tid + 256 * i, row = e / 96, col = e - row * 96, part = col >> 5, c = col & 31;
        float v = bias6[i];
#pragma unroll
        for (int ww = 0; ww < 4; ww++) v += red[(ww * 16 + row) * MS_RP + col];
        qs[row * MS_QP + col] = v;
        if (row < L) p.qkv[(row0 + row) * (3 * MS_D) + part * MS_D + h * MS_DH + c] = v;
    }
    __syncthreads();

    if (w == 0) {
        const int bh = b * MS_H + h;
        f32x4 s = {0.f, 0.f, 0.f, 0.f};
#pragma unroll
        for (int kk = 0; kk < 8; kk++) s = MS_MFMA16(qs[li * MS_QP + 32 + 4 * kk + g], qs[li * MS_QP + 4 * kk + g] * p.scale, s);
        float mx = -INFINITY;
#pragma unroll
        for (int r = 0; r < 4; r++) {
            s[r] = ((km >> r) & 1u) ? -INFINITY : s[r];
            mx = fmaxf(mx, s[r]);
        }
        mx = fmaxf(mx, __shfl_xor(mx, 16, 64));
        mx = fmaxf(mx, __shfl_xor(mx, 32, 64));
        float sum = 0.f;
#pragma unroll
        for (int r = 0; r < 4; r++) { const float e = expf(s[r] - mx); s[r] = e; sum += e; }
        sum += __shfl_xor(sum, 16, 64);
        sum += __shfl_xor(sum, 32, 64);
        const float inv = 1.f / sum;
        const bool qok = li < L;
        if (g == 0 && qok) p.lse[(long)bh * L + li] = mx + logf(sum);
        const float inv_keep = p.p_drop > 0.f ? 1.f / (1.f - p.p_drop) : 1.f;
        f32x4 oc[2] = {f32x4{0.f, 0.f, 0.f, 0.f}, f32x4{0.f, 0.f, 0.f, 0.f}};
#pragma unroll
        for (int t = 0; t < 4; t++) {
            const int key = 4 * g + t;
            float pv = s[t] * inv;
            if (p.p_drop > 0.f) pv *= drop_scale(seed, ((uint64_t)bh * L + li) * L + key, p.p_drop, inv_keep);
#pragma unroll
            for (int c = 0; c < 2; c++) oc[c] = MS_MFMA16(qs[key * MS_QP + 64 + 16 * c + li], pv, oc[c]);
        }
#pragma unroll
        for (int c = 0; c < 2; c++) {
            *reinterpret_cast<f32x4*>(os + li * MS_OP + 16 * c + 4 * g) = oc[c];
            if (qok) *reinterpret_cast<f32x4*>(p.o + (row0 + li) * MS_D + h * MS_DH + 16 * c + 4 * g) = oc[c];
        }
    }
    __syncthreads();

    f32x4 oa[2];
#pragma unroll
    for (int gg = 0; gg < 2; gg++) oa[gg] = *reinterpret_cast<const f32x4*>(os + li * MS_OP + 16 * gg + 4 * g);
    float* yp = p.ypart + ((long)h * p.B * L + row0) * MS_D;
#pragma unroll
    for (int t = 0; t < 4; t++) {
        f32x4 y = {0.f, 0.f, 0.f, 0.f};
#pragma unroll
        for (int gg = 0; gg < 2; gg++)
#pragma unroll
            for (int j = 0; j < 4; j++) y = MS_MFMA16(oa[gg][j], wo[t][gg][j], y);
#pragma unroll
        for (int r = 0; r < 4; r++)
            if (4 * g + r < L) yp[(long)(4 * g + r) * MS_D + 16 * (4 * w + t) + li] = y[r];
    }
}

typedef ldetr_mha_cross_args MhaCrossParams;

__global__ __launch_bounds__(256) void mha_cross_fwd_kernel(MhaCrossParams p) {
    constexpr int KP = MS_DH + 4;
    __shared__ float red[4 * 16 * 33];
    __shared__ __attribute__((aligned(16))) float qs[16 * KP], os[16 * MS_OP], Ks[64 * KP], Vs[64 * KP];
    const int tid = threadIdx.x, lane = tid & 63, w = tid >> 6, li = lane & 15, g = lane >> 4;
    const int b = blockIdx.x / MS_H, h = blockIdx.x - b * MS_H;
    const int Lq = p.Lq, Lk = p.Lk;
    const long row0 = (long)b * Lq, krow0 = (long)b * Lk;

    f32x4 wo[4][2];
#pragma unroll
    for (int t = 0; t < 4; t++)
#pragma unroll
        for (int gg = 0; gg < 2; gg++)
            wo[t][gg] = *reinterpret_cast<const f32x4*>(p.w_out + (long)(16 * (4 * w + t) + li) * MS_D + h * MS_DH + 16 * gg + 4 * g);
    f32x4 xa[4], wb[2][4];
    {
        const bool rok = li < Lq;
        const float* xr = p.x + (row0 + (rok ? li : 0)) * p.ldx + 64 * w + 4 * g;
#pragma unroll
        for (int gg = 0; gg < 4; gg++) {
            const f32x4 v = *reinterpret_cast<const f32x4*>(xr + 16 * gg);
            xa[gg] = rok ? v : f32x4{0.f, 0.f, 0.f, 0.f};
        }
#pragma unroll
        for (int ct = 0; ct < 2; ct++) {
            const float* wr = p.w_q + (long)(h * MS_DH + ct * 16 + li) * MS_D + 64 * w + 4 * g;
#pragma unroll
            for (int gg = 0; gg < 4; gg++) wb[ct][gg] = *reinterpret_cast<const f32x4*>(wr + 16 * gg);
        }
    }
    f32x4 kst[2], vst[2];
#pragma unroll
    for (int i = 0; i < 2; i++) {
        const int e = tid + 256 * i, row = e >> 3, c4 = (e & 7) * 4;
        const bool ok = row < Lk;
        const long r = krow0 + (ok ? row : 0);
        const f32x4 kv = *reinterpret_cast<const f32x4*>(p.k + r * p.ldk + h * MS_DH + c4);
        const f32x4 vv = *reinterpret_cast<const f32x4*>(p.v + r * p.ldv + h * MS_DH + c4);
        kst[i] = ok ? kv : f32x4{0.f, 0.f, 0.f, 0.f}; vst[i] = ok ? vv : f32x4{0.f, 0.f, 0.f, 0.f};
    }
    const float qbias = (tid < 16 * 32) ? p.b_q[h * MS_DH + (tid & 31)] : 0.f;
    unsigned km = 0;
#pragma unroll
    for (int j = 0; j < 4; j++)
#pragma unroll
        for (int r = 0; r < 4; r++) {
            const int key = 16 * j + 4 * g + r;
            const bool masked = key >= Lk || (p.kpm && p.kpm[krow0 + (key < Lk ? key : 0)]);
            km |= masked ? (1u << (4 * j + r)) : 0u;
        }
    const uint64_t seed = p.seed + ((p.p_drop > 0.f && p.seed_ptr) ? *p.seed_ptr : 0ull);
    __builtin_amdgcn_sched_barrier(0);
#pragma unroll
    for (int i = 0; i < 2; i++) {
        const int e = tid + 256 * i, row = e >> 3, c4 = (e & 7) * 4;
        *reinterpret_cast<f32x4*>(Ks + row * KP + c4) = kst[i];
        *reinterpret_cast<f32x4*>(Vs + row * KP + c4) = vst[i];
    }
    f32x4 acc[2] = {f32x4{0.f, 0.f, 0.f, 0.f}, f32x4{0.f, 0.f, 0.f, 0.f}};
#pragma unroll
    for (int gg = 0; gg < 4; gg++)
#pragma unroll
        for (int j = 0; j < 4; j++)
#pragma unroll
            for (int ct = 0; ct < 2; ct++) acc[ct] = MS_MFMA16(xa[gg][j], wb[ct][gg][j], acc[ct]);
#pragma unroll
    for (int ct = 0; ct < 2; ct++)
#pragma unroll
        for (int r = 0; r < 4; r++) red[(w * 16 + 4 * g + r) * 33 + 16 * ct + li] = acc[ct][r];
    __syncthreads();
#pragma unroll
    for (int i = 0; i < 2; i++) {
        const int e = tid + 256 * i, row = e >> 5, c = e & 31;
        float v = qbias;
#pragma unroll
        for (int ww = 0; ww < 4; ww++) v += red[(ww * 16 + row) * 33 + c];
        qs[row * KP + c] = v;
        if (row < Lq) p.q[(row0 + row) * MS_D + h * MS_DH + c] = v;
    }
    __syncthreads();

    if (w == 0) {
        const int bh = b * MS_H + h;
        float qf[8];
#pragma unroll
        for (int kk = 0; kk < 8; kk++) qf[kk] = qs[li * KP + 4 * kk + g] * p.scale;
        f32x4 s[4];
        float mx = -INFINITY;
#pragma unroll
        for (int j = 0; j < 4; j++) {
            f32x4 a = {0.f, 0.f, 0.f, 0.f};
            const float* kp = Ks + (16 * j + li) * KP + g;
#pragma unroll
            for (int kk = 0; kk < 8; kk++) a = MS_MFMA16(kp[4 * kk], qf[kk], a);
#pragma unroll
            for (int r = 0; r < 4; r++) {
                a[r] = ((km >> (4 * j + r)) & 1u) ? -INFINITY : a[r];
                mx = fmaxf(mx, a[r]);
            }
            s[j] = a;
        }
        mx = fmaxf(mx, __shfl_xor(mx, 16, 64));
        mx = fmaxf(mx, __shfl_xor(mx, 32, 64));
        float sum = 0.f;
#pragma unroll
        for (int j = 0; j < 4; j++)
#pragma unroll
            for (int r = 0; r < 4; r++) { const float e = expf(s[j][r] - mx); s[j][r] = e; sum += e; }
        sum += __shfl_xor(sum, 16, 64);
        sum += __shfl_xor(sum, 32, 64);
        const float inv = 1.f / sum;
        const bool qok = li < Lq;
        if (g == 0 && qok) p.lse[(long)bh * Lq + li] = mx + logf(sum);
        const float inv_keep = p.p_drop > 0.f ? 1.f / (1.f - p.p_drop) : 1.f;
        f32x4 oc[2] = {f32x4{0.f, 0.f, 0.f, 0.f}, f32x4{0.f, 0.f, 0.f, 0.f}};
#pragma unroll
        for (int j = 0; j < 4; j++)
#pragma unroll
            for (int t = 0; t < 4; t++) {
                const int key = 16 * j + 4 * g + t;
                float pv = s[j][t] * inv;
                if (p.p_drop > 0.f) pv *= drop_scale(seed, ((uint64_t)bh * Lq + li) * Lk + key, p.p_drop, inv_keep);
                const float* vp = Vs + key * KP + li;
#pragma unroll
                for (int c = 0; c < 2; c++) oc[c] = MS_MFMA16(vp[16 * c], pv, oc[c]);
            }
#pragma unroll
        for (int c = 0; c < 2; c++) {
            *reinterpret_cast<f32x4*>(os + li * MS_OP + 16 * c + 4 * g) = oc[c];
            if (qok) *reinterpret_cast<f32x4*>(p.o + (row0 + li) * MS_D + h * MS_DH + 16 * c + 4 * g) = oc[c];
        }
    }
    __syncthreads();

    f32x4 oa[2];
#pragma unroll
    for (int gg = 0; gg < 2; gg++) oa[gg] = *reinterpret_cast<const f32x4*>(os + li * MS_OP + 16 * gg + 4 * g);
    float* yp = p.ypart + ((long)h * p.B * Lq + row0) * MS_D;
#pragma unroll
    for (int t = 0; t < 4; t++) {
        f32x4 y = {0.f, 0.f, 0.f, 0.f};
#pragma unroll
        for (int gg = 0; gg < 2; gg++)
#pragma unroll
            for (int j = 0; j < 4; j++) y = MS_MFMA16(oa[gg][j], wo[t][gg][j], y);
#pragma unroll
        for (int r = 0; r < 4; r++)
            if (4 * g + r < Lq) yp[(long)(4 * g + r) * MS_D + 16 * (4 * w + t) + li] = y[r];
    }
}


__global__ __launch_bounds__(256) void mha_small_bwd_kernel(MhaSmallParams pa, MhaSmallParams pb, int nb0) {
    constexpr int KP = MS_DH + 4;
    __shared__ float red[4 * 16 * 33];
    __shared__ __attribute__((aligned(16))) float Qs[16 * KP], Ks[16 * KP], Vs[16 * KP], Ds[16 * KP];
    __shared__ __attribute__((aligned(16))) float Gs[16 * MS_QP];
    __shared__ float delta_s[16], lse_s[16];
    const bool second = (int)blockIdx.x >= nb0;
    const MhaSmallParams& p = second ? pb : pa;
    const int bid = second ? (int)blockIdx.x - nb0 : (int)blockIdx.x;
    const int tid = threadIdx.x, lane = tid & 63, w = tid >> 6, li = lane & 15, g = lane >> 4;
    const int b = bid / MS_H, h = bid - b * MS_H, bh = bid;
    const int L = p.L;
    const long row0 = (long)b * L;

    f32x4 wi[24];
#pragma unroll
    for (int kk = 0; kk < 24; kk++) {
        const int c = 4 * kk + g;
        wi[kk] = *reinterpret_cast<const f32x4*>(p.w_in + (long)((c >> 5) * MS_D + h * MS_DH + (c & 31)) * MS_D + 64 * w + 4 * li);
    }
    float wo[2][4][4];
#pragma unroll
    for (int gg = 0; gg < 4; gg++)
#pragma unroll
        for (int j = 0; j < 4; j++)
#pragma unroll
            for (int ct = 0; ct < 2; ct++)
                wo[ct][gg][j] = p.w_out[(long)(64 * w + 16 * gg + 4 * g + j) * MS_D + h * MS_DH + 16 * ct + li];
    f32x4 xa[4];
    {
        const bool rok = li < L;
        const float* xr = p.dr + (row0 + (rok ? li : 0)) * MS_D + 64 * w + 4 * g;
#pragma unroll
        for (int gg = 0; gg < 4; gg++) {
            const f32x4 v = *reinterpret_cast<const f32x4*>(xr + 16 * gg);
            xa[gg] = rok ? v : f32x4{0.f, 0.f, 0.f, 0.f};
        }
    }
    f32x4 st[2];
#pragma unroll
    for (int i = 0; i < 2; i++) {
        const int e = tid + 256 * i, row = e / 24, rem = e - row * 24, part = rem >> 3, c4 = (rem & 7) * 4;
        const bool ok = e < 384 && row < L;
        const f32x4 v = *reinterpret_cast<const f32x4*>(p.qkv + (row0 + (ok ? row : 0)) * (3 * MS_D) + (ok ? part : 0) * MS_D + h * MS_DH + c4);
        st[i] = ok ? v : f32x4{0.f, 0.f, 0.f, 0.f};
    }
    f32x4 o4 = {0.f, 0.f, 0.f, 0.f};
    if (tid < 128) {
        const int row = tid >> 3, c4 = (tid & 7) * 4;
        const f32x4 v = *reinterpret_cast<const f32x4*>(p.o + (row0 + (row < L ? row : 0)) * MS_D + h * MS_DH + c4);
        o4 = row < L ? v : o4;
    }
    if (tid < 16) lse_s[tid] = tid < L ? p.lse[(long)bh * L + tid] : 0.f;
    unsigned km = 0;
#pragma unroll
    for (int r = 0; r < 4; r++) {
        const int key = 4 * g + r;
        km |= (key >= L || (p.kpm && p.kpm[row0 + (key < L ? key : 0)])) ? (1u << r) : 0u;
    }
    km |= (li >= L || (p.kpm && p.kpm[row0 + (li < L ? li : 0)])) ? 16u : 0u;
    const uint64_t seed = p.seed + ((p.p_drop > 0.f && p.seed_ptr) ? *p.seed_ptr : 0ull);
    const float inv_keep = p.p_drop > 0.f ? 1.f / (1.f - p.p_drop) : 1.f;
    __builtin_amdgcn_sched_barrier(0);

    {
        f32x4 acc[2] = {f32x4{0.f, 0.f, 0.f, 0.f}, f32x4{0.f, 0.f, 0.f, 0.f}};
#pragma unroll
        for (int gg = 0; gg < 4; gg++)
#pragma unroll
            for (int j = 0; j < 4; j++)
#pragma unroll
                for (int ct = 0; ct < 2; ct++) acc[ct] = MS_MFMA16(xa[gg][j], wo[ct][gg][j], acc[ct]);
#pragma unroll
        for (int ct = 0; ct < 2; ct++)
#pragma unroll
            for (int r = 0; r < 4; r++) red[(w * 16 + 4 * g + r) * 33 + 16 * ct + li] = acc[ct][r];
    }
#pragma unroll
    for (int i = 0; i < 2; i++) {
        const int e = tid + 256 * i, row = e / 24, rem = e - row * 24, part = rem >> 3, c4 = (rem & 7) * 4;
        if (e < 384) *reinterpret_cast<f32x4*>((part == 0 ? Qs : (part == 1 ? Ks : Vs)) + row * KP + c4) = st[i];
    }
    __syncthreads();
#pragma unroll
    for (int i = 0; i < 2; i++) {
        const int e = tid + 256 * i, row = e >> 5, c = e & 31;
        float v = 0.f;
#pragma unroll
        for (int ww = 0; ww < 4; ww++) v += red[(ww * 16 + row) * 33 + c];
        Ds[row * KP + c] = v;
    }
    __syncthreads();
    if (tid < 128) {
        const int row = tid >> 3, c4 = (tid & 7) * 4;
        const f32x4 d4 = *reinterpret_cast<const f32x4*>(Ds + row * KP + c4);
        float part = o4[0] * d4[0] + o4[1] * d4[1] + o4[2] * d4[2] + o4[3] * d4[3];
        part += __shfl_xor(part, 1, 64); part += __shfl_xor(part, 2, 64); part += __shfl_xor(part, 4, 64);
        if ((tid & 7) == 0) delta_s[row] = part;
    }
    __syncthreads();

    if (w == 0) {
        float qf[8], dof[8];
#pragma unroll
        for (int kk = 0; kk < 8; kk++) { qf[kk] = Qs[li * KP + 4 * kk + g] * p.scale; dof[kk] = Ds[li * KP + 4 * kk + g]; }
        const float delta = delta_s[li], lse = lse_s[li];
        f32x4 sacc = {0.f, 0.f, 0.f, 0.f}, dpacc = {0.f, 0.f, 0.f, 0.f};
#pragma unroll
        for (int kk = 0; kk < 8; kk++) {
            sacc = MS_MFMA16(Ks[li * KP + 4 * kk + g], qf[kk], sacc);
            dpacc = MS_MFMA16(Vs[li * KP + 4 * kk + g], dof[kk], dpacc);
        }
        f32x4 ds;
#pragma unroll
        for (int r = 0; r < 4; r++) {
            const int key = 4 * g + r;
            const float pr = ((km >> r) & 1u) ? 0.f : expf(sacc[r] - lse);
            float dpv = dpacc[r];
            if (p.p_drop > 0.f) dpv *= drop_scale(seed, ((uint64_t)bh * L + li) * L + key, p.p_drop, inv_keep);
            ds[r] = pr * (dpv - delta) * p.scale;
        }
        f32x4 dq[2] = {f32x4{0.f, 0.f, 0.f, 0.f}, f32x4{0.f, 0.f, 0.f, 0.f}};
#pragma unroll
        for (int t = 0; t < 4; t++)
#pragma unroll
            for (int c = 0; c < 2; c++) dq[c] = MS_MFMA16(Ks[(4 * g + t) * KP + 16 * c + li], ds[t], dq[c]);
#pragma unroll
        for (int c = 0; c < 2; c++) {
            *reinterpret_cast<f32x4*>(Gs + li * MS_QP + 16 * c + 4 * g) = dq[c];
            if (li < L && p.dqkv) *reinterpret_cast<f32x4*>(p.dqkv + (row0 + li) * (3 * MS_D) + h * MS_DH + 16 * c + 4 * g) = dq[c];
        }
    } else if (w == 1) {
        const bool kmasked = (km & 16u) != 0;
        float kf[8], vf[8];
#pragma unroll
        for (int kk = 0; kk < 8; kk++) { kf[kk] = Ks[li * KP + 4 * kk + g]; vf[kk] = Vs[li * KP + 4 * kk + g]; }
        f32x4 sacc = {0.f, 0.f, 0.f, 0.f}, dpacc = {0.f, 0.f, 0.f, 0.f};
#pragma unroll
        for (int kk = 0; kk < 8; kk++) {
            sacc = MS_MFMA16(Qs[li * KP + 4 * kk + g] * p.scale, kf[kk], sacc);
            dpacc = MS_MFMA16(Ds[li * KP + 4 * kk + g], vf[kk], dpacc);
        }
        float pd[4], ds[4];
#pragma unroll
        for (int r = 0; r < 4; r++) {
            const int qr = 4 * g + r;
            const float pr = (kmasked || qr >= L) ? 0.f : expf(sacc[r] - lse_s[qr]);
            float dm = 1.f;
            if (p.p_drop > 0.f) dm = drop_scale(seed, ((uint64_t)bh * L + qr) * L + li, p.p_drop, inv_keep);
            pd[r] = pr * dm;
            ds[r] = pr * (dpacc[r] * dm - delta_s[qr]) * p.scale;
        }
        f32x4 dk[2] = {f32x4{0.f, 0.f, 0.f, 0.f}, f32x4{0.f, 0.f, 0.f, 0.f}}, dv[2] = {f32x4{0.f, 0.f, 0.f, 0.f}, f32x4{0.f, 0.f, 0.f, 0.f}};
#pragma unroll
        for (int t = 0; t < 4; t++) {
            const int qr = 4 * g + t;
#pragma unroll
            for (int c = 0; c < 2; c++) {
                dv[c] = MS_MFMA16(Ds[qr * KP + 16 * c + li], pd[t], dv[c]);
                dk[c] = MS_MFMA16(Qs[qr * KP + 16 * c + li], ds[t], dk[c]);
            }
        }
#pragma unroll
        for (int c = 0; c < 2; c++) {
            *reinterpret_cast<f32x4*>(Gs + li * MS_QP + 32 + 16 * c + 4 * g) = dk[c];
            *reinterpret_cast<f32x4*>(Gs + li * MS_QP + 64 + 16 * c + 4 * g) = dv[c];
            if (li < L && p.dqkv) {
                float* gq = p.dqkv + (row0 + li) * (3 * MS_D) + h * MS_DH + 16 * c + 4 * g;
                *reinterpret_cast<f32x4*>(gq + MS_D) = dk[c];
                *reinterpret_cast<f32x4*>(gq + 2 * MS_D) = dv[c];
            }
        }
    }
    __syncthreads();

    f32x4 acc[4] = {f32x4{0.f, 0.f, 0.f, 0.f}, f32x4{0.f, 0.f, 0.f, 0.f}, f32x4{0.f, 0.f, 0.f, 0.f}, f32x4{0.f, 0.f, 0.f, 0.f}};
#pragma unroll
    for (int kk = 0; kk < 24; kk++) {
        const float a = Gs[li * MS_QP + 4 * kk + g];
#pragma unroll
        for (int t = 0; t < 4; t++) acc[t] = MS_MFMA16(a, wi[kk][t], acc[t]);
    }
    float* xp = p.dxpart + ((long)h * p.B * L + row0) * MS_D + 64 * w + 4 * li;
#pragma unroll
    for (int r = 0; r < 4; r++)
        if (4 * g + r < L) *reinterpret_cast<f32x4*>(xp + (long)(4 * g + r) * MS_D) = f32x4{acc[0][r], acc[1][r], acc[2][r], acc[3][r]};
}

__global__ __launch_bounds__(320) void mha_cross_bwd_kernel(MhaCrossParams p) {
    constexpr int KP = MS_DH + 4;
    __shared__ float red[4 * 16 * 33];
    __shared__ __attribute__((aligned(16))) float Qs[16 * KP], Ds[16 * KP], Gq[16 * KP], Ks[64 * KP], Vs[64 * KP];
    __shared__ float delta_s[16], lse_s[16];
    __shared__ unsigned char km_s[64];
    const int tid = threadIdx.x, lane = tid & 63, w = tid >> 6, li = lane & 15, g = lane >> 4;
    const int b = blockIdx.x / MS_H, h = blockIdx.x - b * MS_H, bh = blockIdx.x;
    const int Lq = p.Lq, Lk = p.Lk;
    const long row0 = (long)b * Lq, krow0 = (long)b * Lk;
    const int nkt = (Lk + 15) >> 4;

    f32x4 wq[8];
    float wo[2][4][4];
    f32x4 xa[4];
    if (w < 4) {
#pragma unroll
        for (int kk = 0; kk < 8; kk++) wq[kk] = *reinterpret_cast<const f32x4*>(p.w_q + (long)(h * MS_DH + 4 * kk + g) * MS_D + 64 * w + 4 * li);
#pragma unroll
        for (int gg = 0; gg < 4; gg++)
#pragma unroll
            for (int j = 0; j < 4; j++)
#pragma unroll
                for (int ct = 0; ct < 2; ct++)
                    wo[ct][gg][j] = p.w_out[(long)(64 * w + 16 * gg + 4 * g + j) * MS_D + h * MS_DH + 16 * ct + li];
        const bool rok = li < Lq;
        const float* xr = p.dr + (row0 + (rok ? li : 0)) * MS_D + 64 * w + 4 * g;
#pragma unroll
        for (int gg = 0; gg < 4; gg++) {
            const f32x4 v = *reinterpret_cast<const f32x4*>(xr + 16 * gg);
            xa[gg] = rok ? v : f32x4{0.f, 0.f, 0.f, 0.f};
        }
    }
    f32x4 kst[2], vst[2];
#pragma unroll
    for (int i = 0; i < 2; i++) {
        const int e = tid + 320 * i, row = (e >> 3) & 63, c4 = (e & 7) * 4;
        const bool ok = e < 512 && row < Lk;
        const long r = krow0 + (ok ? row : 0);
        const f32x4 kv = *reinterpret_cast<const f32x4*>(p.k + r * p.ldk + h * MS_DH + c4);
        const f32x4 vv = *reinterpret_cast<const f32x4*>(p.v + r * p.ldv + h * MS_DH + c4);
        kst[i] = ok ? kv : f32x4{0.f, 0.f, 0.f, 0.f}; vst[i] = ok ? vv : f32x4{0.f, 0.f, 0.f, 0.f};
    }
    f32x4 q4 = {0.f, 0.f, 0.f, 0.f}, o4 = {0.f, 0.f, 0.f, 0.f};
    if (tid < 128) {
        const int row = tid >> 3, c4 = (tid & 7) * 4;
        const long r = row0 + (row < Lq ? row : 0);
        const f32x4 qv = *reinterpret_cast<const f32x4*>(p.q + r * MS_D + h * MS_DH + c4);
        const f32x4 ov = *reinterpret_cast<const f32x4*>(p.o + r * MS_D + h * MS_DH + c4);
        if (row < Lq) { q4 = qv; o4 = ov; }
    }
    if (tid < 16) lse_s[tid] = tid < Lq ? p.lse[(long)bh * Lq + tid] : 0.f;
    if (tid < 64) km_s[tid] = (tid >= Lk || (p.kpm && p.kpm[krow0 + (tid < Lk ? tid : 0)])) ? 1 : 0;
    const uint64_t seed = p.seed + ((p.p_drop > 0.f && p.seed_ptr) ? *p.seed_ptr : 0ull);
    const float inv_keep = p.p_drop > 0.f ? 1.f / (1.f - p.p_drop) : 1.f;
    __builtin_amdgcn_sched_barrier(0);

    if (w < 4) {
        f32x4 acc[2] = {f32x4{0.f, 0.f, 0.f, 0.f}, f32x4{0.f, 0.f, 0.f, 0.f}};
#pragma unroll
        for (int gg = 0; gg < 4; gg++)
#pragma unroll
            for (int j = 0; j < 4; j++)
#pragma unroll
                for (int ct = 0; ct < 2; ct++) acc[ct] = MS_MFMA16(xa[gg][j], wo[ct][gg][j], acc[ct]);
#pragma unroll
        for (int ct = 0; ct < 2; ct++)
#pragma unroll
            for (int r = 0; r < 4; r++) red[(w * 16 + 4 * g + r) * 33 + 16 * ct + li] = acc[ct][r];
    }
#pragma unroll
    for (int i = 0; i < 2; i++) {
        const int e = tid + 320 * i, row = (e >> 3) & 63, c4 = (e & 7) * 4;
        if (e < 512) {
            *reinterpret_cast<f32x4*>(Ks + row * KP + c4) = kst[i];
            *reinterpret_cast<f32x4*>(Vs + row * KP + c4) = vst[i];
        }
    }
    if (tid < 128) *reinterpret_cast<f32x4*>(Qs + (tid >> 3) * KP + (tid & 7) * 4) = q4;
    __syncthreads();
    for (int e = tid; e < 512; e += 320) {
        const int row = e >> 5, c = e & 31;
        float v = 0.f;
#pragma unroll
        for (int ww = 0; ww < 4; ww++) v += red[(ww * 16 + row) * 33 + c];
        Ds[row * KP + c] = v;
    }
    __syncthreads();
    if (tid < 128) {
        const int row = tid >> 3, c4 = (tid & 7) * 4;
        const f32x4 d4 = *reinterpret_cast<const f32x4*>(Ds + row * KP + c4);
        float part = o4[0] * d4[0] + o4[1] * d4[1] + o4[2] * d4[2] + o4[3] * d4[3];
        part += __shfl_xor(part, 1, 64); part += __shfl_xor(part, 2, 64); part += __shfl_xor(part, 4, 64);
        if ((tid & 7) == 0) delta_s[row] = part;
    }
    __syncthreads();

    if (w == 4) {
        float qf[8], dof[8];
#pragma unroll
        for (int kk = 0; kk < 8; kk++) { qf[kk] = Qs[li * KP + 4 * kk + g] * p.scale; dof[kk] = Ds[li * KP + 4 * kk + g]; }
        const float delta = delta_s[li], lse = lse_s[li];
        f32x4 dq[2] = {f32x4{0.f, 0.f, 0.f, 0.f}, f32x4{0.f, 0.f, 0.f, 0.f}};
        for (int j = 0; j < nkt; j++) {
            f32x4 sacc = {0.f, 0.f, 0.f, 0.f}, dpacc = {0.f, 0.f, 0.f, 0.f};
            const float* kp = Ks + (16 * j + li) * KP + g;
            const float* vp = Vs + (16 * j + li) * KP + g;
#pragma unroll
            for (int kk = 0; kk < 8; kk++) {
                sacc = MS_MFMA16(kp[4 * kk], qf[kk], sacc);
                dpacc = MS_MFMA16(vp[4 * kk], dof[kk], dpacc);
            }
            f32x4 ds;
#pragma unroll
            for (int r = 0; r < 4; r++) {
                const int key = 16 * j + 4 * g + r;
                const float pr = km_s[key] ? 0.f : expf(sacc[r] - lse);
                float dpv = dpacc[r];
                if (p.p_drop > 0.f) dpv *= drop_scale(seed, ((uint64_t)bh * Lq + li) * Lk + key, p.p_drop, inv_keep);
                ds[r] = pr * (dpv - delta) * p.scale;
            }
#pragma unroll
            for (int t = 0; t < 4; t++) {
                const float* kp2 = Ks + (16 * j + 4 * g + t) * KP + li;
#pragma unroll
                for (int c = 0; c < 2; c++) dq[c] = MS_MFMA16(kp2[16 * c], ds[t], dq[c]);
            }
        }
#pragma unroll
        for (int c = 0; c < 2; c++) {
            *reinterpret_cast<f32x4*>(Gq + li * KP + 16 * c + 4 * g) = dq[c];
            if (li < Lq && p.dq) *reinterpret_cast<f32x4*>(p.dq + (row0 + li) * MS_D + h * MS_DH + 16 * c + 4 * g) = dq[c];
        }
    } else if (w < nkt) {
        const int krow = 16 * w + li;
        const bool kmasked = km_s[krow] != 0;
        float kf[8], vf[8];
#pragma unroll
        for (int kk = 0; kk < 8; kk++) { kf[kk] = Ks[krow * KP + 4 * kk + g]; vf[kk] = Vs[krow * KP + 4 * kk + g]; }
        f32x4 sacc = {0.f, 0.f, 0.f, 0.f}, dpacc = {0.f, 0.f, 0.f, 0.f};
#pragma unroll
        for (int kk = 0; kk < 8; kk++) {
            sacc = MS_MFMA16(Qs[li * KP + 4 * kk + g] * p.scale, kf[kk], sacc);
            dpacc = MS_MFMA16(Ds[li * KP + 4 * kk + g], vf[kk], dpacc);
        }
        float pd[4], ds[4];
#pragma unroll
        for (int r = 0; r < 4; r++) {
            const int qr = 4 * g + r;
            const float pr = (kmasked || qr >= Lq) ? 0.f : expf(sacc[r] - lse_s[qr]);
            float dm = 1.f;
            if (p.p_drop > 0.f) dm = drop_scale(seed, ((uint64_t)bh * Lq + qr) * Lk + krow, p.p_drop, inv_keep);
            pd[r] = pr * dm;
            ds[r] = pr * (dpacc[r] * dm - delta_s[qr]) * p.scale;
        }
        f32x4 dk[2] = {f32x4{0.f, 0.f, 0.f, 0.f}, f32x4{0.f, 0.f, 0.f, 0.f}}, dv[2] = {f32x4{0.f, 0.f, 0.f, 0.f}, f32x4{0.f, 0.f, 0.f, 0.f}};
#pragma unroll
        for (int t = 0; t < 4; t++) {
            const int qr = 4 * g + t;
#pragma unroll
            for (int c = 0; c < 2; c++) {
                dv[c] = MS_MFMA16(Ds[qr * KP + 16 * c + li], pd[t], dv[c]);
                dk[c] = MS_MFMA16(Qs[qr * KP + 16 * c + li], ds[t], dk[c]);
            }
        }
        if (krow < Lk) {
            float* dkp = p.dk + (krow0 + krow) * p.lddk + h * MS_DH + 4 * g;
            float* dvp = p.dv + (krow0 + krow) * p.lddv + h * MS_DH + 4 * g;
#pragma unroll
            for (int c = 0; c < 2; c++) {
                *reinterpret_cast<f32x4*>(dkp + 16 * c) = dk[c];
                *reinterpret_cast<f32x4*>(dvp + 16 * c) = dv[c];
            }
        }
    }
    __syncthreads();

    if (w < 4) {
        f32x4 acc[4] = {f32x4{0.f, 0.f, 0.f, 0.f}, f32x4{0.f, 0.f, 0.f, 0.f}, f32x4{0.f, 0.f, 0.f, 0.f}, f32x4{0.f, 0.f, 0.f, 0.f}};
#pragma unroll
        for (int kk = 0; kk < 8; kk++) {
            const float a = Gq[li * KP + 4 * kk + g];
#pragma unroll
            for (int t = 0; t < 4; t++) acc[t] = MS_MFMA16(a, wq[kk][t], acc[t]);
        }
        float* xp = p.dxpart + ((long)h * p.B * Lq + row0) * MS_D + 64 * w + 4 * li;
#pragma unroll
        for (int r = 0; r < 4; r++)
            if (4 * g + r < Lq) *reinterpret_cast<f32x4*>(xp + (long)(4 * g + r) * MS_D) = f32x4{acc[0][r], acc[1][r], acc[2][r], acc[3][r]};
    }
}

struct WgradMulti { ldetr_wgrad_desc d[8]; int start[9]; int n; };

__global__ __launch_bounds__(256) void wgrad_multi_kernel(WgradMulti m) {
    using acc_t = __attribute__((__vector_size__(16 * sizeof(float)))) float;
    __shared__ float red[4][32][33];
    __shared__ float rsum[4][32];
    int pi = 0;
#pragma unroll
    for (int i = 1; i < 8; i++) pi += (i < m.n && (int)blockIdx.x >= m.start[i]) ? 1 : 0;
    const ldetr_wgrad_desc& d = m.d[pi];
    const int bid = (int)blockIdx.x - m.start[pi];
    const int gx = (d.cols + 31) >> 5;
    const int by = bid / gx, bx = bid - by * gx;
    const int tid = threadIdx.x, lane = tid & 63, wave = tid >> 6, cl = lane & 31, kl = lane >> 5;
    const int m0 = by * 32, n0 = bx * 32;
    const int units = (d.M + 15) >> 4, ubeg = wave * units / 4, uend = (wave + 1) * units / 4;
    const __amdgpu_buffer_rsrc_t rsA = __builtin_amdgcn_make_buffer_rsrc(const_cast<float*>(d.A), 0, (int)((long)d.M * d.lda * 4), 0x00020000);
    const __amdgpu_buffer_rsrc_t rsB = __builtin_amdgcn_make_buffer_rsrc(const_cast<float*>(d.B), 0, (int)((long)d.M * d.ldb * 4), 0x00020000);
    const int OOB = (int)0x80000000;
    const int lda4 = (int)d.lda * 4, ldb4 = (int)d.ldb * 4;
    const int voffA = (m0 + cl < d.rows) ? (8 * kl * (int)d.lda + m0 + cl) * 4 : OOB;
    const int voffB = (n0 + cl < d.cols) ? (8 * kl * (int)d.ldb + n0 + cl) * 4 : OOB;
    acc_t acc;
#pragma unroll
    for (int r = 0; r < 16; r++) acc[r] = 0.f;
    const bool want_rs = d.db != nullptr && bx == 0;
    float rs = 0.f;
    for (int u0 = ubeg; u0 < uend; u0 += 4) {
        float a[4][8], bq[4][8];
#pragma unroll
        for (int q = 0; q < 4; q++) {
            const bool on = u0 + q < uend;
            const int soff = (u0 + q) * 16;
#pragma unroll
            for (int t = 0; t < 8; t++) {
                a[q][t] = __int_as_float(__builtin_amdgcn_raw_buffer_load_b32(rsA, on ? voffA : OOB, (soff + t) * lda4, 0));
                bq[q][t] = __int_as_float(__builtin_amdgcn_raw_buffer_load_b32(rsB, on ? voffB : OOB, (soff + t) * ldb4, 0));
            }
        }
#pragma unroll
        for (int q = 0; q < 4; q++)
#pragma unroll
            for (int t = 0; t < 8; t++) {
                acc = __builtin_amdgcn_mfma_f32_32x32x2f32(a[q][t], bq[q][t], acc, 0, 0, 0);
                rs += a[q][t];
            }
    }
    if (want_rs) {
        rs += __shfl_xor(rs, 32);
        if (kl == 0) rsum[wave][cl] = rs;
    }
#pragma unroll
    for (int r = 0; r < 16; r++) red[wave][(r & 3) + 8 * (r >> 2) + 4 * kl][cl] = acc[r];
    __syncthreads();
    if (want_rs && tid < 32 && m0 + tid < d.rows) d.db[m0 + tid] += rsum[0][tid] + rsum[1][tid] + rsum[2][tid] + rsum[3][tid];
    const bool vec = (d.ldw & 3) == 0 && ((((uintptr_t)d.dW) & 15) == 0);
    for (int q = tid; q < 256; q += 256) {
        const int row = q >> 3, c4 = (q & 7) * 4;
        if (m0 + row >= d.rows) continue;
        float v[4];
#pragma unroll
        for (int e = 0; e < 4; e++) v[e] = red[0][row][c4 + e] + red[1][row][c4 + e] + red[2][row][c4 + e] + red[3][row][c4 + e];
        float* dst = d.dW + (long)(m0 + row) * d.ldw + n0 + c4;
        if (vec && n0 + c4 + 3 < d.cols) {
            float4 c = *reinterpret_cast<float4*>(dst);
            c.x += v[0]; c.y += v[1]; c.z += v[2]; c.w += v[3];
            *reinterpret_cast<float4*>(dst) = c;
        } else {
#pragma unroll
            for (int e = 0; e < 4; e++)
                if (n0 + c4 + e < d.cols) dst[e] += v[e];
        }
    }
}

}

using namespace ldetr;

static int mha_small_check(const char* what, const MhaSmallParams& p, bool bwd) {
    LDETR_CHECK(p.L >= 1 && p.L <= 16 && p.B >= 0, "%s: 1 <= L <= 16 tokens per sample", what);
    LDETR_CHECK(p.w_in && p.w_out && p.qkv && p.o && p.lse, "%s: null pointer", what);
    LDETR_CHECK(p.p_drop >= 0.f && p.p_drop < 1.f, "%s: p_drop out of range", what);
    if (!bwd) {
        LDETR_CHECK(p.x && p.b_in && p.ypart, "%s: null pointer", what);
        LDETR_CHECK(p.ldx >= MS_D && p.ldx % 4 == 0, "%s: row pitch of x must be a multiple of 4 floats, >= 256", what);
        LDETR_CHECK((((uintptr_t)p.x | (uintptr_t)p.w_in | (uintptr_t)p.w_out | (uintptr_t)p.o | (uintptr_t)p.qkv | (uintptr_t)p.ypart) & 15) == 0,
                    "%s: buffers must be 16-byte aligned", what);
    } else {
        LDETR_CHECK(p.dr && p.dxpart, "%s: null pointer", what);
        LDETR_CHECK((((uintptr_t)p.dr | (uintptr_t)p.w_in | (uintptr_t)p.w_out | (uintptr_t)p.o | (uintptr_t)p.qkv | (uintptr_t)p.dqkv | (uintptr_t)p.dxpart) & 15) == 0,
                    "%s: buffers must be 16-byte aligned", what);
    }
    return LDETR_OK;
}

static int mha_small_launch(const ldetr_mha_small_args* a, int n, bool bwd, void* stream) {
    const char* what = bwd ? "mha_small_bwd" : "mha_small_fwd";
    LDETR_CHECK(a && (n == 1 || n == 2), "%s: 1 or 2 problems", what);
    MhaSmallParams p[2]; p[0] = a[0]; p[1] = n == 2 ? a[1] : a[0];
    int nb[2] = {0, 0};
    for (int i = 0; i < n; i++) {
        if (int rc = mha_small_check(what, p[i], bwd)) return rc;
        nb[i] = p[i].B * MS_H;
    }
    if (nb[0] + nb[1] == 0) return LDETR_OK;
    if (bwd) hipLaunchKernelGGL(mha_small_bwd_kernel, dim3((unsigned)(nb[0] + nb[1])), dim3(256), 0, (hipStream_t)stream, p[0], p[1], nb[0]);
    else hipLaunchKernelGGL(mha_small_fwd_kernel, dim3((unsigned)(nb[0] + nb[1])), dim3(256), 0, (hipStream_t)stream, p[0], p[1], nb[0]);
    count_engine_launch(false);
    return check_launch(what);
}

extern "C" int ldetr_mha_small_fwd_group_f32(const ldetr_mha_small_args* a, int n, void* stream) { return mha_small_launch(a, n, false, stream); }
extern "C" int ldetr_mha_small_bwd_group_f32(const ldetr_mha_small_args* a, int n, void* stream) { return mha_small_launch(a, n, true, stream); }

static int mha_cross_check(const char* what, const MhaCrossParams& p, bool bwd) {
    LDETR_CHECK(p.Lq >= 1 && p.Lq <= 16 && p.Lk >= 1 && p.Lk <= 64 && p.B >= 0, "%s: 1 <= Lq <= 16 queries and 1 <= Lk <= 64 keys per sample", what);
    LDETR_CHECK(p.w_q && p.k && p.v && p.w_out && p.q && p.o && p.lse, "%s: null pointer", what);
    if (!bwd) {
        LDETR_CHECK(p.x && p.b_q && p.ypart, "%s: null pointer", what);
        LDETR_CHECK(p.ldx >= MS_D && p.ldx % 4 == 0 && p.ldk % 4 == 0 && p.ldv % 4 == 0, "%s: row pitches must be multiples of 4 floats", what);
        LDETR_CHECK((((uintptr_t)p.x | (uintptr_t)p.w_q | (uintptr_t)p.w_out | (uintptr_t)p.k | (uintptr_t)p.v | (uintptr_t)p.o | (uintptr_t)p.q | (uintptr_t)p.ypart) & 15) == 0,
                    "%s: buffers must be 16-byte aligned", what);
    } else {
        LDETR_CHECK(p.dr && p.dk && p.dv && p.dxpart, "%s: null pointer", what);
        LDETR_CHECK(p.ldk % 4 == 0 && p.ldv % 4 == 0 && p.lddk % 4 == 0 && p.lddv % 4 == 0, "%s: row pitches must be multiples of 4 floats", what);
        LDETR_CHECK((((uintptr_t)p.dr | (uintptr_t)p.w_q | (uintptr_t)p.w_out | (uintptr_t)p.k | (uintptr_t)p.v | (uintptr_t)p.o | (uintptr_t)p.q | (uintptr_t)p.dq |
                      (uintptr_t)p.dk | (uintptr_t)p.dv | (uintptr_t)p.dxpart) & 15) == 0, "%s: buffers must be 16-byte aligned", what);
    }
    LDETR_CHECK(p.p_drop >= 0.f && p.p_drop < 1.f, "%s: p_drop out of range", what);
    return LDETR_OK;
}

static int mha_cross_launch(const ldetr_mha_cross_args* a, bool bwd, void* stream) {
    const char* what = bwd ? "mha_cross_bwd" : "mha_cross_fwd";
    LDETR_CHECK(a != nullptr, "%s: null argument block", what);
    const MhaCrossParams& p = *a;
    if (int rc = mha_cross_check(what, p, bwd)) return rc;
    if (p.B == 0) return LDETR_OK;
    if (bwd) hipLaunchKernelGGL(mha_cross_bwd_kernel, dim3((unsigned)(p.B * MS_H)), dim3(320), 0, (hipStream_t)stream, p);
    else hipLaunchKernelGGL(mha_cross_fwd_kernel, dim3((unsigned)(p.B * MS_H)), dim3(256), 0, (hipStream_t)stream, p);
    count_engine_launch(false);
    return check_launch(what);
}

extern "C" int ldetr_mha_cross_fwd_f32(const ldetr_mha_cross_args* a, void* stream) { return mha_cross_launch(a, false, stream); }
extern "C" int ldetr_mha_cross_bwd_f32(const ldetr_mha_cross_args* a, void* stream) { return mha_cross_launch(a, true, stream); }

extern "C" int ldetr_wgrad_multi_f32(const ldetr_wgrad_desc* d, int n, void* stream) {
    LDETR_CHECK(d && n >= 1 && n <= 8, "wgrad_multi: 1..8 problems");
    WgradMulti m; memset(&m, 0, sizeof(m));
    int total = 0;
    for (int i = 0; i < n; i++) {
        const ldetr_wgrad_desc& q = d[i];
        LDETR_CHECK(q.A && q.B && q.dW && q.M >= 0 && q.rows > 0 && q.cols > 0 && q.lda >= q.rows && q.ldb >= q.cols && q.ldw >= q.cols, "wgrad_multi: bad problem %d", i);
        LDETR_CHECK((long)q.M * q.lda * 4 < 0x7fffffffL && (long)q.M * q.ldb * 4 < 0x7fffffffL, "wgrad_multi: operand above 2 GiB");
        m.d[i] = q; m.start[i] = total;
        total += q.M > 0 ? cdiv(q.rows, 32) * cdiv(q.cols, 32) : 0;
    }
    for (int i = n; i <= 8; i++) m.start[i] = total;
    m.n = n;
    if (total == 0) return LDETR_OK;
    hipLaunchKernelGGL(wgrad_multi_kernel, dim3((unsigned)total), dim3(256), 0, (hipStream_t)stream, m);
    count_engine_launch(false);
    return check_launch("wgrad_multi");
}
```

layoutdetr_amd/hip/blocks.py:

```python
import math

from .. import _lib
from . import core

D_MODEL, N_HEAD = 256, 8
SCALE = 1.0 / math.sqrt(D_MODEL // N_HEAD)

_ENTRIES = {'layernorm_fwd': ('ldetr_layernorm_fwd_group_f32', True), 'layernorm_bwd': ('ldetr_layernorm_bwd_group_f32', True),
            'ffn_fwd': ('ldetr_ffn_fwd_group_f32', True), 'ffn_bwd': ('ldetr_ffn_bwd_group_f32', True),
            'mha_small_fwd': ('ldetr_mha_small_fwd_group_f32', True), 'mha_small_bwd': ('ldetr_mha_small_bwd_group_f32', True),
            'mha_cross_fwd': ('ldetr_mha_cross_fwd_f32', False), 'mha_cross_bwd': ('ldetr_mha_cross_bwd_f32', False)}


def launch(what, args, flops=0.0, nbytes=0.0):
    entry, grouped = _ENTRIES[what]
    fn = getattr(core.lib(), entry)
    n = len(args)
    arr = (type(args[0]) * n)(*args)
    if grouped:
        call = lambda: core.check(fn(arr, n, core.stream()), what)
    else:
        assert n == 1
        call = lambda: core.check(fn(arr, core.stream()), what)
    if flops > 0:
        core.engine_call('ldetr_token_stack', flops, call, nbytes=nbytes)
    else:
        call()


def draw_seed(p_drop):
    return core.next_seed() if p_drop > 0 else 0


def _set_dropout(a, p_drop, seed):
    a.p_drop, a.seed, a.seed_ptr = p_drop, seed, (core.iter_seed().data_ptr() if p_drop > 0 else None)


def _p(t):
    return t.data_ptr() if t is not None else None


def ln_fwd(x, r, gamma, beta, eps, p_drop, seed, y, z, mean, rstd, r_parts=0, r_bias=None, pos=None, ypos=None):
    a = _lib.LnArgs()
    M, D = x.shape
    a.x, a.r, a.gamma, a.beta, a.y, a.z, a.mean, a.rstd = x.data_ptr(), _p(r), gamma.data_ptr(), beta.data_ptr(), y.data_ptr(), _p(z), mean.data_ptr(), rstd.data_ptr()
    a.rows, a.D, a.eps = M, D, eps
    if r is not None:
        _set_dropout(a, p_drop, seed)
    a.r_parts, a.r_part_stride = r_parts, M * D
    a.r_bias = _p(r_bias) if r_parts > 0 else None
    if pos is not None:
        a.pos, a.pos_rows, a.ypos = pos.data_ptr(), pos.shape[0], ypos.data_ptr()
    return a


def ln_bwd(dy, z, mean, rstd, gamma, dx, dr, dgamma, dbeta, p_drop, seed, dy2=None, parts=None, n_parts=0):
    a = _lib.LnArgs()
    M, D = z.shape
    a.dy, a.z, a.mean, a.rstd, a.gamma, a.dx = dy.data_ptr(), z.data_ptr(), mean.data_ptr(), rstd.data_ptr(), gamma.data_ptr(), dx.data_ptr()
    a.dy2, a.dr, a.dgamma, a.dbeta = _p(dy2), _p(dr), _p(dgamma), _p(dbeta)
    a.dy_parts = parts.data_ptr() if n_parts else None
    a.dy_nparts, a.dy_part_stride = n_parts, M * D
    a.rows, a.D = M, D
    _set_dropout(a, p_drop, seed)
    return a


def ffn_fwd(x, w1, b1, w2, h, ypart, p_drop, seed):
    a = _lib.FfnArgs()
    a.x, a.ldx, a.w1, a.b1, a.w2, a.h, a.ypart = x.data_ptr(), x.stride(0), w1.data_ptr(), b1.data_ptr(), w2.data_ptr(), h.data_ptr(), ypart.data_ptr()
    a.M, a.F = h.shape
    _set_dropout(a, p_drop, seed)
    return a


def ffn_bwd(dy, x, h, w1, w2, dxpart, dh, p_drop):
    a = _lib.FfnArgs()
    a.dy, a.x, a.ldx, a.h, a.w1, a.w2, a.dxpart, a.dh = dy.data_ptr(), x.data_ptr(), x.stride(0), h.data_ptr(), w1.data_ptr(), w2.data_ptr(), dxpart.data_ptr(), _p(dh)
    a.M, a.F = h.shape
    a.p_drop = p_drop
    return a


def mha_small_fwd(x, w_in, b_in, w_out, kpm, qkv, o, lse, ypart, B, L, p_drop, seed):
    a = _lib.MhaSmallArgs()
    a.x, a.ldx, a.w_in, a.b_in, a.w_out, a.kpm = x.data_ptr(), x.stride(0), w_in.data_ptr(), b_in.data_ptr(), w_out.data_ptr(), _p(kpm)
    a.qkv, a.o, a.lse, a.ypart, a.B, a.L, a.scale = qkv.data_ptr(), o.data_ptr(), lse.data_ptr(), ypart.data_ptr(), B, L, SCALE
    _set_dropout(a, p_drop, seed)
    return a


def mha_small_bwd(dr, w_in, w_out, kpm, qkv, o, lse, dqkv, dxpart, B, L, p_drop, seed):
    a = _lib.MhaSmallArgs()
    a.w_in, a.w_out, a.kpm, a.qkv, a.o, a.lse = w_in.data_ptr(), w_out.data_ptr(), _p(kpm), qkv.data_ptr(), o.data_ptr(), lse.data_ptr()
    a.dr, a.dqkv, a.dxpart, a.B, a.L, a.scale = dr.data_ptr(), _p(dqkv), dxpart.data_ptr(), B, L, SCALE
    _set_dropout(a, p_drop, seed)
    return a


def mha_cross_fwd(x, w_q, b_q, k, v, w_out, kpm, q, o, lse, ypart, B, Lq, Lk, p_drop, seed):
    a = _lib.MhaCrossArgs()
    a.x, a.ldx, a.w_q, a.b_q, a.w_out, a.kpm = x.data_ptr(), x.stride(0), w_q.data_ptr(), b_q.data_ptr(), w_out.data_ptr(), _p(kpm)
    a.k, a.ldk, a.v, a.ldv = k.data_ptr(), k.stride(0), v.data_ptr(), v.stride(0)
    a.q, a.o, a.lse, a.ypart, a.B, a.Lq, a.Lk, a.scale = q.data_ptr(), o.data_ptr(), lse.data_ptr(), ypart.data_ptr(), B, Lq, Lk, SCALE
    _set_dropout(a, p_drop, seed)
    return a


def mha_cross_bwd(dr, w_q, k, v, w_out, kpm, q, o, lse, dq, dk, dv, dxpart, B, Lq, Lk, p_drop, seed):
    a = _lib.MhaCrossArgs()
    a.w_q, a.w_out, a.kpm, a.q, a.o, a.lse = w_q.data_ptr(), w_out.data_ptr(), _p(kpm), q.data_ptr(), o.data_ptr(), lse.data_ptr()
    a.k, a.ldk, a.v, a.ldv = k.data_ptr(), k.stride(0), v.data_ptr(), v.stride(0)
    a.dr, a.dq, a.dk, a.lddk, a.dv, a.lddv, a.dxpart = dr.data_ptr(), dq.data_ptr(), dk.data_ptr(), dk.stride(0), dv.data_ptr(), dv.stride(0), dxpart.data_ptr()
    a.B, a.Lq, a.Lk, a.scale = B, Lq, Lk, SCALE
    _set_dropout(a, p_drop, seed)
    return a
```

layoutdetr_amd/hip/stacks.py:

```python
from operator import attrgetter

import torch

from .. import _lib
from . import blocks, core
from .blocks import D_MODEL, N_HEAD

MAX_TOKENS, MAX_ROWS, MAX_CROSS_KEYS = 16, 512, 64
ENABLED = core.knob('TOKEN_STACKS', 1) != 0

NODE_RUNS = [0]

_SELF = (('sa_w_in', 'self_attn.in_proj_weight'), ('sa_b_in', 'self_attn.in_proj_bias'), ('sa_w_out', 'self_attn.out_proj.weight'), ('sa_b_out', 'self_attn.out_proj.bias'))
_CROSS = (('n1_g', 'norm1.weight'), ('n1_b', 'norm1.bias'),
          ('ca_w_in', 'multihead_attn.in_proj_weight'), ('ca_b_in', 'multihead_attn.in_proj_bias'), ('ca_w_out', 'multihead_attn.out_proj.weight'), ('ca_b_out', 'multihead_attn.out_proj.bias'))


def _tail(norm_a, norm_b):
    return (('na_g', norm_a + '.weight'), ('na_b', norm_a + '.bias'), ('w1', 'linear1.weight'), ('b1', 'linear1.bias'), ('w2', 'linear2.weight'), ('b2', 'linear2.bias'),
            ('nb_g', norm_b + '.weight'), ('nb_b', norm_b + '.bias'))


LAYOUT = {'enc': _SELF + _tail('norm1', 'norm2'), 'dec': _SELF + _CROSS + _tail('norm2', 'norm3')}
_OFFSET = {kind: {name: j for j, (name, _) in enumerate(fields)} for kind, fields in LAYOUT.items()}
_TAIL_MODULES = {'enc': ('norm1', 'dropout1', 'norm2', 'dropout2'), 'dec': ('norm2', 'dropout2', 'norm3', 'dropout3')}
ENC_PARAMS, DEC_PARAMS = len(LAYOUT['enc']), len(LAYOUT['dec'])


class Prog(object):

    def __init__(self, kind, layers, x, B, L, kpm, training, final_norm=None, kvs=None, S=0, mem_kpm=None):
        self.kind, self.layers, self.x, self.B, self.L, self.kpm, self.training = kind, list(layers), x, B, L, kpm, training
        self.final_norm, self.kvs, self.S, self.mem_kpm = final_norm, kvs, S, mem_kpm


def layer_params(kind, layer):
    return [attrgetter(path)(layer) for _, path in LAYOUT[kind]]


def usable(prog):
    x = prog.x
    if not (x.is_cuda and x.dtype == torch.float32 and x.dim() == 2 and x.shape[1] == D_MODEL and 1 <= prog.L <= MAX_TOKENS and x.shape[0] == prog.B * prog.L
            and x.shape[0] <= MAX_ROWS and len(prog.layers) >= 1):
        return False
    for l in prog.layers:
        sa = l.self_attn
        if sa.num_heads != N_HEAD or sa.in_proj_weight.shape[1] != D_MODEL or l.linear1.weight.shape[0] % 64 != 0 or l.linear1.bias is None or l.linear2.bias is None:
            return False
        if sa.in_proj_bias is None or sa.out_proj.bias is None:
            return False
        if prog.kind == 'dec' and (l.multihead_attn.num_heads != N_HEAD or l.multihead_attn.in_proj_bias is None or l.multihead_attn.out_proj.bias is None):
            return False
    if prog.kind == 'dec' and (prog.kvs is None or len(prog.kvs) != len(prog.layers)):
        return False
    return True


def _new(dev, *shape):
    return torch.empty(shape, device=dev, dtype=torch.float32)


def _rows(t):
    if t.dtype == torch.float32 and t.dim() == 2 and t.stride(1) == 1 and t.stride(0) % 4 == 0 and t.data_ptr() % 16 == 0 and t.stride(0) >= t.shape[1]:
        return t
    return core.f32c(t)


def _fl_self(pr, bwd=False):
    M, D, att = pr.B * pr.L, D_MODEL, pr.B * N_HEAD * 2.0 * pr.L * pr.L * (D_MODEL // N_HEAD)
    fl = 2.0 * M * D * 3 * D + 2.0 * M * D * D + (5 if bwd else 2) * att
    return fl, 4.0 * (M * D * (6 if bwd else 5) + 4 * D * D + N_HEAD * M * D)


def _fl_cross(pr, bwd=False):
    M, D, att = pr.B * pr.L, D_MODEL, pr.B * N_HEAD * 2.0 * pr.L * pr.S * (D_MODEL // N_HEAD)
    fl = 2.0 * M * D * D * 2 + (5 if bwd else 2) * att
    return fl, 4.0 * (M * D * 4 + 2 * D * D + (4 if bwd else 2) * pr.B * pr.S * D + N_HEAD * M * D)


def _fl_ffn(M, F):
    return 4.0 * M * D_MODEL * F, 4.0 * (2 * D_MODEL * F + M * F + (F // 64 + 1) * M * D_MODEL)


def _launch_sum(what, args, costs):
    blocks.launch(what, args, sum(f for f, _ in costs), sum(b for _, b in costs))


class _LayerParams(object):

    def __init__(self, kind, tensors, base):
        self.kind, self.base = kind, base
        for j, (name, _) in enumerate(LAYOUT[kind]):
            setattr(self, name, core.f32c(tensors[base + j].detach()))

    def index(self, name):
        return self.base + _OFFSET[self.kind][name]


class _Stack(object):
    __slots__ = ('prog', 'M', 'dev', 'x_index', 'params', 'final', 'final_index', 'K', 'V', 'kv_index', 'saved', 'final_saved', 'cur', 'res', 'keep', 'need_w', 'g', 't')

    def __init__(self, prog, x, x_index):
        self.prog, self.M, self.dev, self.x_index, self.cur = prog, prog.B * prog.L, x.device, x_index, _rows(x)
        self.params, self.saved = [], []
        self.final = self.final_index = self.K = self.V = self.kv_index = self.final_saved = self.res = self.keep = self.need_w = self.g = self.t = None


class _Saved(object):
    __slots__ = ('x', 'qkv', 'o', 'lse', 'p_att', 'seed_att', 'p1', 'seed1', 'z1', 'mean1', 'rstd1', 't1', 'p_c', 'seed_c', 'qc', 'oc', 'lse_c', 'cross_small',
                 'p_a', 'seed_a', 'p_h', 'seed_h', 'p_b', 'seed_b', 'F', 'x1', 'za', 'mean_a', 'rstd_a', 'h', 'zb', 'mean_b', 'rstd_b')


class _Scratch(object):
    __slots__ = ('gin', 'dz', 'dr', 'dxpart', 'dh', 'dsum', 'da', 'da_ca', 'dq', 'dk', 'dv', 'dqkv', 'dxpart_sa')


class _Grad(object):

    def __init__(self, res, parts=None, n=0, dy2=None):
        self.res, self.parts, self.n, self.dy2 = res, parts, n, dy2


def _unpack(progs, tensors):
    st, pos = [], 0
    for pr in progs:
        s = _Stack(pr, tensors[pos], pos); pos += 1
        for _ in pr.layers:
            s.params.append(_LayerParams(pr.kind, tensors, pos)); pos += len(LAYOUT[pr.kind])
        if pr.final_norm is not None:
            s.final, s.final_index = [core.f32c(t.detach()) for t in tensors[pos:pos + 2]], pos
            pos += 2
        if pr.kind == 'dec':
            n = len(pr.layers)
            s.K, s.V, s.kv_index = list(tensors[pos:pos + n]), list(tensors[pos + n:pos + 2 * n]), pos
            pos += 2 * n
        st.append(s)
    assert pos == len(tensors)
    return st


def _fwd_self_attn(act, i):
    H, D, args = N_HEAD, D_MODEL, []
    for s in act:
        pr, M, W, dev = s.prog, s.M, s.params[i], s.dev
        sv = _Saved()
        sv.p_att = pr.layers[i].self_attn.dropout if pr.training else 0.0
        sv.x, sv.qkv, sv.o, sv.lse, sv.seed_att = s.cur, _new(dev, M, 3 * D), _new(dev, M, D), _new(dev, pr.B * H * pr.L), blocks.draw_seed(sv.p_att)
        ypart = _new(dev, H, M, D)
        args.append(blocks.mha_small_fwd(sv.x, W.sa_w_in, W.sa_b_in, W.sa_w_out, pr.kpm, sv.qkv, sv.o, sv.lse, ypart, pr.B, pr.L, sv.p_att, sv.seed_att))
        s.res = (ypart, W.sa_b_out, H)
        s.saved.append(sv)
    _launch_sum('mha_small_fwd', args, [_fl_self(s.prog) for s in act])


def _fwd_norm1_cross(s, i):
    H, D = N_HEAD, D_MODEL
    pr, M, W, sv, dev = s.prog, s.M, s.params[i], s.saved[i], s.dev
    layer = pr.layers[i]
    sv.p1 = layer.dropout1.p if pr.training else 0.0
    sv.seed1, sv.z1, sv.mean1, sv.rstd1, sv.t1 = blocks.draw_seed(sv.p1), _new(dev, M, D), _new(dev, M), _new(dev, M), _new(dev, M, D)
    r, r_bias, r_parts = s.res
    blocks.launch('layernorm_fwd', [blocks.ln_fwd(s.cur, r, W.n1_g, W.n1_b, layer.norm1.eps, sv.p1, sv.seed1, sv.t1, sv.z1, sv.mean1, sv.rstd1, r_parts=r_parts, r_bias=r_bias)])
    s.cur = sv.t1
    K, V = s.K[i], s.V[i]
    sv.p_c = layer.multihead_attn.dropout if pr.training else 0.0
    sv.seed_c, sv.qc, sv.oc, sv.lse_c = blocks.draw_seed(sv.p_c), _new(dev, M, D), _new(dev, M, D), _new(dev, pr.B * H * pr.L)
    Wq, Bq = W.ca_w_in[:D], W.ca_b_in[:D]
    sv.cross_small = (1 <= pr.S <= MAX_CROSS_KEYS and K.stride(1) == 1 and V.stride(1) == 1 and K.stride(0) % 4 == 0 and V.stride(0) % 4 == 0
                      and K.data_ptr() % 16 == 0 and V.data_ptr() % 16 == 0)
    if sv.cross_small:
        ypart = _new(dev, H, M, D)
        _launch_sum('mha_cross_fwd', [blocks.mha_cross_fwd(sv.t1, Wq, Bq, K, V, W.ca_w_out, pr.mem_kpm, sv.qc, sv.oc, sv.lse_c, ypart, pr.B, pr.L, pr.S, sv.p_c, sv.seed_c)],
                    [_fl_cross(pr)])
        s.res = (ypart, W.ca_b_out, H)
    else:
        lib = core.lib()
        core.gemm(sv.t1, Wq, 0, 0, M, D, D, out=sv.qc, ep=core.epilogue(col_bias=Bq))
        core.check(lib.ldetr_attention_fwd_f32(
            core.ptr(sv.qc), D, core.ptr(K), K.stride(0), core.ptr(V), V.stride(0), core.ptr(pr.mem_kpm), core.ptr(sv.oc), D, core.ptr(sv.lse_c),
            pr.B, H, pr.L, pr.S, D // H, blocks.SCALE, sv.p_c, sv.seed_c, core.seed_ptr() if sv.p_c > 0 else None, 0, core.stream()), 'attention_fwd')
        s.res = (core.gemm(sv.oc, W.ca_w_out, 0, 0, M, D, D, ep=core.epilogue(col_bias=W.ca_b_out)), None, 0)


def _fwd_tail(act, i):
    D, ln_a, ffn, ln_b = D_MODEL, [], [], []
    for s in act:
        pr, M, W, sv, dev = s.prog, s.M, s.params[i], s.saved[i], s.dev
        layer = pr.layers[i]
        norm_a, drop_a, norm_b, drop_b = [getattr(layer, m) for m in _TAIL_MODULES[pr.kind]]
        sv.p_a, sv.p_h, sv.p_b = (drop_a.p, layer.dropout.p, drop_b.p) if pr.training else (0.0, 0.0, 0.0)
        sv.seed_a, sv.seed_h, sv.seed_b = blocks.draw_seed(sv.p_a), blocks.draw_seed(sv.p_h), blocks.draw_seed(sv.p_b)
        sv.F = W.w1.shape[0]
        ns = sv.F // 64
        sv.x1, sv.za, sv.mean_a, sv.rstd_a, sv.h = _new(dev, M, D), _new(dev, M, D), _new(dev, M), _new(dev, M), _new(dev, M, sv.F)
        sv.zb, sv.mean_b, sv.rstd_b = _new(dev, M, D), _new(dev, M), _new(dev, M)
        parts, y = _new(dev, ns, M, D), _new(dev, M, D)
        r, r_bias, r_parts = s.res
        ln_a.append(blocks.ln_fwd(s.cur, r, W.na_g, W.na_b, norm_a.eps, sv.p_a, sv.seed_a, sv.x1, sv.za, sv.mean_a, sv.rstd_a, r_parts=r_parts, r_bias=r_bias))
        ffn.append(blocks.ffn_fwd(sv.x1, W.w1, W.b1, W.w2, sv.h, parts, sv.p_h, sv.seed_h))
        ln_b.append(blocks.ln_fwd(sv.x1, parts, W.nb_g, W.nb_b, norm_b.eps, sv.p_b, sv.seed_b, y, sv.zb, sv.mean_b, sv.rstd_b, r_parts=ns, r_bias=W.b2))
        s.keep = (r, parts)
        s.cur, s.res = y, None
    blocks.launch('layernorm_fwd', ln_a)
    _launch_sum('ffn_fwd', ffn, [_fl_ffn(s.M, s.saved[i].F) for s in act])
    blocks.launch('layernorm_fwd', ln_b)


def _fwd_final_norm(s):
    M, dev = s.M, s.dev
    z, mean, rstd, y = s.cur, _new(dev, M), _new(dev, M), _new(dev, M, D_MODEL)
    blocks.launch('layernorm_fwd', [blocks.ln_fwd(z, None, s.final[0], s.final[1], s.prog.final_norm.eps, 0.0, 0, y, z, mean, rstd)])
    s.final_saved, s.cur = (z, mean, rstd), y


class _Backward(object):

    def __init__(self, ctx):
        self.tensors, self.need = ctx.params, ctx.needs_input_grad
        self.grads = [None] * (1 + len(self.tensors))
        self.wg_off = core.WEIGHT_GRADIENTS_DISABLED[0]
        self.temps = {}

    def target(self, idx):
        fg = core.flat_grad(self.tensors[idx])
        if fg is not None and fg.is_contiguous():
            return fg
        if idx not in self.temps:
            self.temps[idx] = torch.zeros_like(self.tensors[idx], memory_format=torch.contiguous_format)
            self.grads[1 + idx] = self.temps[idx]
        return self.temps[idx]

    def norm_targets(self, W, gamma, beta, wanted):
        return (self.target(W.index(gamma)), self.target(W.index(beta))) if wanted else (None, None)


def _bwd_enter(s, dy, bw):
    pr, M, dev = s.prog, s.M, s.dev
    npar = len(LAYOUT[pr.kind])
    s.need_w = (not bw.wg_off) and any(bw.need[1 + j] for W in s.params for j in range(W.base, W.base + npar))
    g = _Grad(_rows(dy.reshape(M, D_MODEL)))
    if pr.final_norm is not None:
        z, mean, rstd = s.final_saved
        dx = _new(dev, M, D_MODEL)
        want = (not bw.wg_off) and (bw.need[1 + s.final_index] or bw.need[2 + s.final_index])
        dgamma, dbeta = (bw.target(s.final_index), bw.target(s.final_index + 1)) if want else (None, None)
        blocks.launch('layernorm_bwd', [blocks.ln_bwd(g.res, z, mean, rstd, s.final[0], dx, None, dgamma, dbeta, 0.0, 0)])
        g = _Grad(dx)
    s.g = g


def _bwd_tail(act, i, bw):
    D, ln_b, ffn, ln_a = D_MODEL, [], [], []
    for s in act:
        sv, M, W, dev, g = s.saved[i], s.M, s.params[i], s.dev, s.g
        ns = sv.F // 64
        t = s.t = _Scratch()
        t.gin = g
        t.dz = _new(dev, M, D)
        t.dr = _new(dev, M, D) if sv.p_b > 0 else t.dz
        dgamma, dbeta = bw.norm_targets(W, 'nb_g', 'nb_b', s.need_w)
        ln_b.append(blocks.ln_bwd(g.res, sv.zb, sv.mean_b, sv.rstd_b, W.nb_g, t.dz, t.dr if sv.p_b > 0 else None, dgamma, dbeta, sv.p_b, sv.seed_b,
                                  dy2=g.dy2, parts=g.parts, n_parts=g.n))
        t.dxpart, t.dh = _new(dev, ns, M, D), (_new(dev, M, sv.F) if s.need_w else None)
        ffn.append(blocks.ffn_bwd(t.dr, sv.x1, sv.h, W.w1, W.w2, t.dxpart, t.dh, sv.p_h))
        t.dsum = _new(dev, M, D)
        t.da = _new(dev, M, D) if sv.p_a > 0 else t.dsum
        dgamma, dbeta = bw.norm_targets(W, 'na_g', 'na_b', s.need_w)
        ln_a.append(blocks.ln_bwd(t.dz, sv.za, sv.mean_a, sv.rstd_a, W.na_g, t.dsum, t.da if sv.p_a > 0 else None, dgamma, dbeta, sv.p_a, sv.seed_a,
                                  parts=t.dxpart, n_parts=ns))
    blocks.launch('layernorm_bwd', ln_b)
    _launch_sum('ffn_bwd', ffn, [_fl_ffn(s.M, s.saved[i].F) for s in act])
    blocks.launch('layernorm_bwd', ln_a)


def _bwd_cross_norm1(s, i, bw):
    H, D = N_HEAD, D_MODEL
    pr, sv, M, W, t, dev = s.prog, s.saved[i], s.M, s.params[i], s.t, s.dev
    K, V = s.K[i], s.V[i]
    dk, dv = pr.kvs[i][2]()
    Wq = W.ca_w_in[:D]
    dq = _new(dev, M, D)
    if sv.cross_small:
        dxpart_c = _new(dev, H, M, D)
        _launch_sum('mha_cross_bwd', [blocks.mha_cross_bwd(t.da, Wq, K, V, W.ca_w_out, pr.mem_kpm, sv.qc, sv.oc, sv.lse_c, dq, dk, dv, dxpart_c, pr.B, pr.L, pr.S, sv.p_c, sv.seed_c)],
                    [_fl_cross(pr, bwd=True)])
        g1 = _Grad(t.dsum, dxpart_c, H)
    else:
        d_o = core.gemm(t.da, W.ca_w_out, 0, 1, M, D, D)
        core.check(core.lib().ldetr_attention_bwd_f32(
            core.ptr(sv.qc), D, core.ptr(K), K.stride(0), core.ptr(V), V.stride(0), core.ptr(pr.mem_kpm), core.ptr(sv.oc), D, core.ptr(sv.lse_c),
            core.ptr(d_o), D, core.ptr(dq), D, core.ptr(dk), dk.stride(0), core.ptr(dv), dv.stride(0), pr.B, H, pr.L, pr.S, D // H, blocks.SCALE, sv.p_c, sv.seed_c,
            core.seed_ptr() if sv.p_c > 0 else None, 0, core.stream()), 'attention_bwd')
        g1 = _Grad(t.dsum, dy2=core.gemm(dq, Wq, 0, 1, M, D, D))
    t.dq, t.dk, t.dv = dq, dk, dv
    i_k, i_v = 1 + s.kv_index + i, 1 + s.kv_index + len(pr.layers) + i
    if bw.need[i_k]:
        bw.grads[i_k] = dk
    if bw.need[i_v]:
        bw.grads[i_v] = dv
    dsum1 = _new(dev, M, D)
    da1 = _new(dev, M, D) if sv.p1 > 0 else dsum1
    dgamma, dbeta = bw.norm_targets(W, 'n1_g', 'n1_b', s.need_w)
    blocks.launch('layernorm_bwd', [blocks.ln_bwd(g1.res, sv.z1, sv.mean1, sv.rstd1, W.n1_g, dsum1, da1 if sv.p1 > 0 else None, dgamma, dbeta, sv.p1, sv.seed1,
                                                   dy2=g1.dy2, parts=g1.parts, n_parts=g1.n)])
    t.da_ca, t.da, t.dsum = t.da, da1, dsum1


def _bwd_self_attn(act, i):
    H, D, args = N_HEAD, D_MODEL, []
    for s in act:
        pr, sv, M, W, t, dev = s.prog, s.saved[i], s.M, s.params[i], s.t, s.dev
        t.dqkv = _new(dev, M, 3 * D) if s.need_w else None
        t.dxpart_sa = _new(dev, H, M, D)
        args.append(blocks.mha_small_bwd(t.da, W.sa_w_in, W.sa_w_out, pr.kpm, sv.qkv, sv.o, sv.lse, t.dqkv, t.dxpart_sa, pr.B, pr.L, sv.p_att, sv.seed_att))
    _launch_sum('mha_small_bwd', args, [_fl_self(s.prog, bwd=True) for s in act])


def _bwd_weights(act, i, bw):
    descs = []
    for s in act:
        if not s.need_w:
            continue
        sv, M, W, t = s.saved[i], s.M, s.params[i], s.t

        def desc(A, Bm, weight, bias, rows=None):
            d = _lib.WgradDesc()
            dW, db = bw.target(W.index(weight)), bw.target(W.index(bias))
            nrows = A.shape[1] if rows is None else rows
            d.A, d.lda, d.B, d.ldb, d.dW, d.ldw, d.db = A.data_ptr(), A.stride(0), Bm.data_ptr(), Bm.stride(0), dW.data_ptr(), dW.shape[1], db.data_ptr()
            d.M, d.rows, d.cols = M, nrows, Bm.shape[1]
            return d
        descs.append(desc(t.dr, sv.h, 'w2', 'b2'))
        descs.append(desc(t.dh, sv.x1, 'w1', 'b1'))
        descs.append(desc(t.da, sv.o, 'sa_w_out', 'sa_b_out'))
        descs.append(desc(t.dqkv, sv.x, 'sa_w_in', 'sa_b_in'))
        if s.prog.kind == 'dec':
            descs.append(desc(t.da_ca, sv.oc, 'ca_w_out', 'ca_b_out'))
            descs.append(desc(t.dq, sv.t1, 'ca_w_in', 'ca_b_in', rows=D_MODEL))
    lib = core.lib()
    for j in range(0, len(descs), 8):
        chunk = descs[j:j + 8]
        arr = (_lib.WgradDesc * len(chunk))(*chunk)
        wf = sum(2.0 * d.M * d.rows * d.cols for d in chunk)
        wb = sum(4.0 * (d.M * (d.rows + d.cols) + d.rows * d.cols) for d in chunk)
        core.engine_call('ldetr_token_stack', wf, lambda: core.check(lib.ldetr_wgrad_multi_f32(arr, len(chunk), core.stream()), 'wgrad_multi'), nbytes=wb)


def _bwd_leave(s, bw):
    if bw.need[1 + s.x_index]:
        g, M = s.g, s.M
        dx = _new(s.dev, M, D_MODEL)
        core.check(core.lib().ldetr_sum_parts_f32(core.ptr(g.res), core.ptr(g.parts), g.n, M * D_MODEL, core.ptr(dx), M * D_MODEL, core.stream()), 'sum_parts')
        bw.grads[1 + s.x_index] = dx.reshape(bw.tensors[s.x_index].shape)


class _TokenStacksFn(torch.autograd.Function):

    @staticmethod
    def forward(ctx, progs, *tensors):
        ctx.set_materialize_grads(False)
        core.require_gpu(*[t for t in tensors if t is not None])
        st = _unpack(progs, tensors)
        for i in range(max(len(s.prog.layers) for s in st)):
            act = [s for s in st if i < len(s.prog.layers)]
            _fwd_self_attn(act, i)
            for s in act:
                if s.prog.kind == 'dec':
                    _fwd_norm1_cross(s, i)
            _fwd_tail(act, i)
        outs = []
        for s in st:
            if s.prog.final_norm is not None:
                _fwd_final_norm(s)
            outs.append(s.cur)
            s.cur = s.res = s.keep = None
        ctx.progs, ctx.params, ctx.state = progs, tensors, st
        return tuple(outs)

    @staticmethod
    def backward(ctx, *douts):
        bw = _Backward(ctx)
        live = []
        for s, dy in zip(ctx.state, douts):
            if dy is not None:
                _bwd_enter(s, dy, bw)
                live.append(s)
        if not live:
            return tuple(bw.grads)
        for i in reversed(range(max(len(s.prog.layers) for s in live))):
            act = [s for s in live if i < len(s.prog.layers)]
            _bwd_tail(act, i, bw)
            for s in act:
                if s.prog.kind == 'dec':
                    _bwd_cross_norm1(s, i, bw)
            _bwd_self_attn(act, i)
            _bwd_weights(act, i, bw)
            for s in act:
                s.g, s.t = _Grad(s.t.dsum, s.t.dxpart_sa, N_HEAD), None
        for s in live:
            _bwd_leave(s, bw)
        return tuple(bw.grads)


def run(progs):
    NODE_RUNS[0] += 1
    tensors = []
    for pr in progs:
        tensors.append(pr.x)
        for layer in pr.layers:
            tensors += layer_params(pr.kind, layer)
        if pr.final_norm is not None:
            tensors += [pr.final_norm.weight, pr.final_norm.bias]
        if pr.kind == 'dec':
            tensors += [kv[0] for kv in pr.kvs] + [kv[1] for kv in pr.kvs]
    return list(_TokenStacksFn.apply(progs, *tensors))
```

Baseline: 511.4.

## Fuse LayerNorm prologue into cross-attention and FFN forward kernels

Adds templated LN-prologue variants of the cross-attention and FFN forward kernels. Each block now computes the LayerNorm of its 32 or 16 row tile (residual plus partial sums plus dropout) into shared memory, instead of running a separate layernorm launch first. It still writes y, z, mean and rstd from one writer block. This removes a launch and a global round trip of the normalized activations per layer, at the cost of redundant LN computation across the blocks that share a row tile, plus extra LDS and register pressure. A knob and fallback paths keep the old sequence available.

```diff
diff --git a/include/ldetr_hip.h b/include/ldetr_hip.h
--- a/include/ldetr_hip.h
+++ b/include/ldetr_hip.h
@@ -169,6 +169,9 @@
 } ldetr_mha_cross_args;
 int ldetr_mha_cross_fwd_f32(const ldetr_mha_cross_args* a, void* stream);
 int ldetr_mha_cross_bwd_f32(const ldetr_mha_cross_args* a, void* stream);
+
+int ldetr_mha_cross_ln_fwd_f32(const ldetr_ln_args* ln, const ldetr_mha_cross_args* a, void* stream);
+int ldetr_ffn_ln_fwd_group_f32(const ldetr_ln_args* ln, const ldetr_ffn_args* a, int n, void* stream);
 
 typedef struct ldetr_wgrad_desc {
     const float* A; int64_t lda; const float* B; int64_t ldb;
diff --git a/layoutdetr_amd/_lib.py b/layoutdetr_amd/_lib.py
--- a/layoutdetr_amd/_lib.py
+++ b/layoutdetr_amd/_lib.py
@@ -173,6 +173,8 @@
     'ldetr_mha_small_bwd_group_f32': [_P, _I, _P],
     'ldetr_mha_cross_fwd_f32': [_P, _P],
     'ldetr_mha_cross_bwd_f32': [_P, _P],
+    'ldetr_mha_cross_ln_fwd_f32': [_P, _P, _P],
+    'ldetr_ffn_ln_fwd_group_f32': [_P, _P, _I, _P],
     'ldetr_wgrad_multi_f32': [_P, _I, _P],
     'ldetr_loss_combine_fwd_f32': [_P, _P, _P, _P, _P, _I, _I, _P, _P, _P, _P],
     'ldetr_loss_combine_bwd_f32': [_P, _P, _P, _P, _P, _I, _I, _P, _P, _P],
diff --git a/layoutdetr_amd/build.py b/layoutdetr_amd/build.py
--- a/layoutdetr_amd/build.py
+++ b/layoutdetr_amd/build.py
@@ -14,7 +14,7 @@
 
 SOURCES = ['ldetr_core.cpp', 'bias_act.hip', 'upfirdn2d.hip', 'gemm_conv.hip', 'attention.hip', 'layernorm.hip',
            'misc_ops.hip', 'optim.hip', 'lsap.hip', 'xent.hip', 'resample.hip', 'layout_loss.hip', 'demod.hip', 'sg2_affine.hip', 'wgrad_smallc.hip', 'stem_conv.hip', 'box_ops.hip', 'ffn_fused.hip', 'conv_c32.hip', 'mha_small.hip', 'p3_engine.hip', 'bmm_strided.hip', 'layoutnet.hip', 'layoutnet_train.hip', 'layout_finish.hip', 'layout_raster.hip', 'page_filter.hip', 'patch_resize.hip', 'png_decode.hip', 'png_encode.hip', 'png_inflate.hip']
-HEADERS = ['ldetr_common.hpp', 'layoutnet_layers.hpp', 'pil_resample.hpp', 'png_pages.hpp', 'png_inflate_kernel.hpp', os.path.join('..', '..', 'include', 'ldetr_hip.h')]
+HEADERS = ['ldetr_common.hpp', 'ln_row.hpp', 'layoutnet_layers.hpp', 'pil_resample.hpp', 'png_pages.hpp', 'png_inflate_kernel.hpp', os.path.join('..', '..', 'include', 'ldetr_hip.h')]
 
 FLAGS = ([] if os.environ.get('LDETR_TILE_TRACE') else ['-DLDETR_TILE_TRACE=0']) + (['-DP3_TRACE'] if os.environ.get('LDETR_P3_TRACE') else []) + ['-O3', '-std=c++17', '-fPIC', f'--offload-arch={ARCH}', '-munsafe-fp-atomics', '-fno-gpu-rdc',
          '-Wno-unused-result', '-Rpass-analysis=kernel-resource-usage']
diff --git a/layoutdetr_amd/csrc/ffn_fused.hip b/layoutdetr_amd/csrc/ffn_fused.hip
--- a/layoutdetr_amd/csrc/ffn_fused.hip
+++ b/layoutdetr_amd/csrc/ffn_fused.hip
@@ -1,4 +1,6 @@
+#include <type_traits>
 #include "ldetr_common.hpp"
+#include "ln_row.hpp"
 #include "../../include/ldetr_hip.h"
 
 namespace ldetr {
@@ -25,7 +27,8 @@
 }
 #define FFN_MFMA16(A, B, ACC) _Pragma("unroll") for (int t_ = 0; t_ < 16; t_++) ACC = __builtin_amdgcn_mfma_f32_32x32x2f32(A[t_], B[t_], ACC, 0, 0, 0)
 
-__global__ __launch_bounds__(256) void ffn_fwd_kernel(FfnParams pa, FfnParams pb, int nb0) {
+template <bool LN>
+__global__ __launch_bounds__(256) void ffn_fwd_kernel(FfnParams pa, FfnParams pb, int nb0, std::conditional_t<LN, LnPair, LnNone> ln) {
     __shared__ float red[2][32][33];
     __shared__ float Hs[32][FHP];
     const bool second = (int)blockIdx.x >= nb0;
@@ -44,12 +47,32 @@
 #pragma unroll
         for (int r = 0; r < 16; r++) acc[r] = 0.f;
         float a[4][16], b[4][16];
-#pragma unroll
-        for (int c = 0; c < 4; c++) { ld_k16(rsX, vA, c * 128, a[c]); ld_k16(rsW, vB, c * 128, b[c]); }
-#pragma unroll
-        for (int q = 0; q < 2; q++)
-#pragma unroll
-            for (int c = 0; c < 2; c++) ld_k16(rsW2, (((wave * 2 + q) * 32 + cl) * p.F + j0 + 16 * kl) * 4, c * 128, b2[q][c]);
+        if constexpr (LN) {
+            __shared__ __attribute__((aligned(16))) float Xs[32 * LN_TILE_PITCH];
+#pragma unroll
+            for (int c = 0; c < 4; c++) ld_k16(rsW, vB, c * 128, b[c]);
+#pragma unroll
+            for (int q = 0; q < 2; q++)
+#pragma unroll
+                for (int c = 0; c < 2; c++) ld_k16(rsW2, (((wave * 2 + q) * 32 + cl) * p.F + j0 + 16 * kl) * 4, c * 128, b2[q][c]);
+            __builtin_amdgcn_sched_barrier(0);
+            ln_fwd_tile<32>(second ? ln.b : ln.a, m0, p.M - m0 < 32 ? p.M - m0 : 32, s == 0, wave, lane, Xs);
+            __syncthreads();
+#pragma unroll
+            for (int c = 0; c < 4; c++)
+#pragma unroll
+                for (int j = 0; j < 4; j++) {
+                    const float4 v = *reinterpret_cast<const float4*>(Xs + cl * LN_TILE_PITCH + kh * 128 + 16 * kl + 32 * c + 4 * j);
+                    a[c][4 * j] = v.x; a[c][4 * j + 1] = v.y; a[c][4 * j + 2] = v.z; a[c][4 * j + 3] = v.w;
+                }
+        } else {
+#pragma unroll
+            for (int c = 0; c < 4; c++) { ld_k16(rsX, vA, c * 128, a[c]); ld_k16(rsW, vB, c * 128, b[c]); }
+#pragma unroll
+            for (int q = 0; q < 2; q++)
+#pragma unroll
+                for (int c = 0; c < 2; c++) ld_k16(rsW2, (((wave * 2 + q) * 32 + cl) * p.F + j0 + 16 * kl) * 4, c * 128, b2[q][c]);
+        }
         __builtin_amdgcn_sched_barrier(0);
 #pragma unroll
         for (int c = 0; c < 4; c++) FFN_MFMA16(a[c], b[c], acc);
@@ -199,21 +222,34 @@
     return LDETR_OK;
 }
 
-static int ffn_launch(const ldetr_ffn_args* a, int n, bool bwd, void* stream) {
-    const char* what = bwd ? "ffn_bwd" : "ffn_fwd";
+static int ffn_launch(const ldetr_ln_args* ln, const ldetr_ffn_args* a, int n, bool bwd, void* stream) {
+    const char* what = ln ? "ffn_ln_fwd" : (bwd ? "ffn_bwd" : "ffn_fwd");
     LDETR_CHECK(a && (n == 1 || n == 2), "%s: 1 or 2 problems", what);
     FfnParams p[2]; p[0] = a[0]; p[1] = n == 2 ? a[1] : a[0];
     int nb[2] = {0, 0};
     for (int i = 0; i < n; i++) {
-        if (int rc = ffn_check_args(what, p[i], bwd)) return rc;
+        if (int rc = ffn_check_args(what, p[i], bwd)) return ln ? LDETR_ERR_UNSUPPORTED : rc;
+        if (ln)
+            if (int rc = ln_check_fused(what, ln[i], p[i].M, p[i].x, p[i].ldx)) return rc;
         nb[i] = cdiv(p[i].M, 32) * (p[i].F / FHS);
     }
     if (nb[0] + nb[1] == 0) return LDETR_OK;
-    if (bwd) hipLaunchKernelGGL(ffn_bwd_kernel, dim3(nb[0] + nb[1]), dim3(256), 0, (hipStream_t)stream, p[0], p[1], nb[0]);
-    else hipLaunchKernelGGL(ffn_fwd_kernel, dim3(nb[0] + nb[1]), dim3(256), 0, (hipStream_t)stream, p[0], p[1], nb[0]);
+    const dim3 grid(nb[0] + nb[1]), block(256);
+    hipStream_t st = (hipStream_t)stream;
+    if (ln) {
+        LnPair lp; lp.a = ln[0]; lp.b = n == 2 ? ln[1] : ln[0];
+        if (lp.a.r_parts == 0) lp.a.r_bias = nullptr;
+        if (lp.b.r_parts == 0) lp.b.r_bias = nullptr;
+        hipLaunchKernelGGL(ffn_fwd_kernel<true>, grid, block, 0, st, p[0], p[1], nb[0], lp);
+    } else if (bwd) hipLaunchKernelGGL(ffn_bwd_kernel, grid, block, 0, st, p[0], p[1], nb[0]);
+    else hipLaunchKernelGGL(ffn_fwd_kernel<false>, grid, block, 0, st, p[0], p[1], nb[0], LnNone{});
     count_engine_launch(false);
     return check_launch(what);
 }
 
-extern "C" int ldetr_ffn_fwd_group_f32(const ldetr_ffn_args* a, int n, void* stream) { return ffn_launch(a, n, false, stream); }
-extern "C" int ldetr_ffn_bwd_group_f32(const ldetr_ffn_args* a, int n, void* stream) { return ffn_launch(a, n, true, stream); }
+extern "C" int ldetr_ffn_fwd_group_f32(const ldetr_ffn_args* a, int n, void* stream) { return ffn_launch(nullptr, a, n, false, stream); }
+extern "C" int ldetr_ffn_bwd_group_f32(const ldetr_ffn_args* a, int n, void* stream) { return ffn_launch(nullptr, a, n, true, stream); }
+extern "C" int ldetr_ffn_ln_fwd_group_f32(const ldetr_ln_args* ln, const ldetr_ffn_args* a, int n, void* stream) {
+    LDETR_CHECK(ln, "ffn_ln_fwd: null LayerNorm block");
+    return ffn_launch(ln, a, n, false, stream);
+}
diff --git a/layoutdetr_amd/csrc/layernorm.hip b/layoutdetr_amd/csrc/layernorm.hip
--- a/layoutdetr_amd/csrc/layernorm.hip
+++ b/layoutdetr_amd/csrc/layernorm.hip
@@ -1,4 +1,5 @@
 #include "ldetr_common.hpp"
+#include "ln_row.hpp"
 #include "../../include/ldetr_hip.h"
 
 namespace ldetr {
@@ -12,9 +13,16 @@
     const int lane = threadIdx.x & 63, wave = threadIdx.x >> 6;
     const long row = (long)(second ? (int)blockIdx.x - nb0 : (int)blockIdx.x) * 4 + wave;
     if (row >= p.rows) return;
-    const int D4 = p.D >> 2;
     const float inv_keep = p.p_drop > 0.f ? 1.f / (1.f - p.p_drop) : 1.f;
     const uint64_t seed = p.seed + (p.seed_ptr ? *p.seed_ptr : 0ull);
+    if constexpr (NV == 1) {
+        const long rows[1] = {row};
+        const bool wr[1] = {true};
+        float4 o[1][NV];
+        ln_fwd_rows<NV, 1, 16>(p, rows, rows, wr, lane, seed, inv_keep, o);
+        return;
+    }
+    const int D4 = p.D >> 2;
     float4 v[NV];
     float s = 0.f;
 #pragma unroll
@@ -172,15 +180,6 @@
 }
 
 using namespace ldetr;
-
-static int ln_check_fwd(const LnParams& p) {
-    LDETR_CHECK(p.r_parts >= 0 && (p.r_parts == 0 || (p.r && p.r_part_stride >= p.rows * p.D)), "layernorm_fwd: bad partial-sum arguments");
-    LDETR_CHECK(p.x && p.gamma && p.beta && p.y, "layernorm_fwd: null pointer");
-    LDETR_CHECK((p.pos == nullptr) == (p.ypos == nullptr) && (!p.pos || p.pos_rows > 0), "layernorm_fwd: pos, pos_rows and ypos go together");
-    LDETR_CHECK(p.D % 4 == 0 && p.D >= 4 && p.D <= 1024, "layernorm_fwd: D must be a multiple of 4 in [4, 1024]");
-    LDETR_CHECK(p.rows >= 0 && p.rows < (1L << 31) - 8, "layernorm_fwd: bad row count");
-    return LDETR_OK;
-}
 
 extern "C" int ldetr_layernorm_fwd_group_f32(const ldetr_ln_args* a, int n, void* stream) {
     LDETR_CHECK(a && (n == 1 || n == 2), "layernorm_fwd_group: 1 or 2 problems");
diff --git a/layoutdetr_amd/csrc/ln_row.hpp b/layoutdetr_amd/csrc/ln_row.hpp
--- /dev/null
+++ b/layoutdetr_amd/csrc/ln_row.hpp
@@ -0,0 +1,156 @@
+#pragma once
+#include "ldetr_common.hpp"
+#include "../../include/ldetr_hip.h"
+
+namespace ldetr {
+
+template <int NV, int R, int PW>
+__device__ __forceinline__ void ln_fwd_rows(const ldetr_ln_args& p, const long (&row)[R], const long (&lrow)[R], const bool (&wr)[R], int lane,
+                                            uint64_t seed, float inv_keep, float4 (&o)[R][NV]) {
+    const int D4 = p.D >> 2;
+    float4 v[R][NV];
+    float s[R];
+#pragma unroll
+    for (int k = 0; k < R; k++) s[k] = 0.f;
+#pragma unroll
+    for (int i = 0; i < NV; i++) {
+        int c4 = lane + i * 64;
+#pragma unroll
+        for (int k = 0; k < R; k++) v[k][i] = make_float4(0.f, 0.f, 0.f, 0.f);
+        if (c4 < D4) {
+#pragma unroll
+            for (int k = 0; k < R; k++) v[k][i] = reinterpret_cast<const float4*>(p.x + lrow[k] * p.D)[c4];
+            if (p.r) {
+                float4 rr[R];
+#pragma unroll
+                for (int k = 0; k < R; k++) rr[k] = reinterpret_cast<const float4*>(p.r + lrow[k] * p.D)[c4];
+                if (p.r_parts > 0) {
+                    if (p.r_bias) {
+                        const float4 bb = reinterpret_cast<const float4*>(p.r_bias)[c4];
+#pragma unroll
+                        for (int k = 0; k < R; k++) { rr[k].x += bb.x; rr[k].y += bb.y; rr[k].z += bb.z; rr[k].w += bb.w; }
+                    }
+                    for (int s0 = 1; s0 < p.r_parts; s0 += PW) {
+                        float4 q[R][PW];
+#pragma unroll
+                        for (int j = 0; j < PW; j++)
+#pragma unroll
+                            for (int k = 0; k < R; k++)
+                                q[k][j] = (s0 + j < p.r_parts) ? reinterpret_cast<const float4*>(p.r + (s0 + j) * p.r_part_stride + lrow[k] * p.D)[c4] : make_float4(0.f, 0.f, 0.f, 0.f);
+#pragma unroll
+                        for (int j = 0; j < PW; j++)
+                            if (s0 + j < p.r_parts) {
+#pragma unroll
+                                for (int k = 0; k < R; k++) { rr[k].x += q[k][j].x; rr[k].y += q[k][j].y; rr[k].z += q[k][j].z; rr[k].w += q[k][j].w; }
+                            }
+                    }
+                }
+                if (p.p_drop > 0.f) {
+#pragma unroll
+                    for (int k = 0; k < R; k++) {
+                        uint64_t e = (uint64_t)row[k] * p.D + (c4 << 2);
+                        rr[k].x *= drop_scale(seed, e, p.p_drop, inv_keep);
+                        rr[k].y *= drop_scale(seed, e + 1, p.p_drop, inv_keep);
+                        rr[k].z *= drop_scale(seed, e + 2, p.p_drop, inv_keep);
+                        rr[k].w *= drop_scale(seed, e + 3, p.p_drop, inv_keep);
+                    }
+                }
+#pragma unroll
+                for (int k = 0; k < R; k++) { v[k][i].x += rr[k].x; v[k][i].y += rr[k].y; v[k][i].z += rr[k].z; v[k][i].w += rr[k].w; }
+            }
+#pragma unroll
+            for (int k = 0; k < R; k++) {
+                if (p.z && wr[k]) reinterpret_cast<float4*>(p.z + row[k] * p.D)[c4] = v[k][i];
+                s[k] += v[k][i].x + v[k][i].y + v[k][i].z + v[k][i].w;
+            }
+        }
+    }
+#pragma unroll
+    for (int k = 0; k < R; k++) {
+        const float mean = wave_sum(s[k]) / p.D;
+        float q = 0.f;
+#pragma unroll
+        for (int i = 0; i < NV; i++) {
+            int c4 = lane + i * 64;
+            if (c4 < D4) {
+                float a = v[k][i].x - mean, b = v[k][i].y - mean, c = v[k][i].z - mean, d = v[k][i].w - mean;
+                q += a * a + b * b + c * c + d * d;
+            }
+        }
+        const float rstd = rsqrtf(wave_sum(q) / p.D + p.eps);
+        if (lane == 0 && wr[k]) { if (p.mean) p.mean[row[k]] = mean; if (p.rstd) p.rstd[row[k]] = rstd; }
+#pragma unroll
+        for (int i = 0; i < NV; i++) {
+            int c4 = lane + i * 64;
+            o[k][i] = make_float4(0.f, 0.f, 0.f, 0.f);
+            if (c4 < D4) {
+                float4 g = reinterpret_cast<const float4*>(p.gamma)[c4];
+                float4 b = reinterpret_cast<const float4*>(p.beta)[c4];
+                float4 y;
+                y.x = (v[k][i].x - mean) * rstd * g.x + b.x; y.y = (v[k][i].y - mean) * rstd * g.y + b.y;
+                y.z = (v[k][i].z - mean) * rstd * g.z + b.z; y.w = (v[k][i].w - mean) * rstd * g.w + b.w;
+                o[k][i] = y;
+                if (wr[k]) {
+                    reinterpret_cast<float4*>(p.y + row[k] * p.D)[c4] = y;
+                    if (p.ypos) {
+                        const float4 pp = reinterpret_cast<const float4*>(p.pos + (row[k] % p.pos_rows) * p.D)[c4];
+                        y.x += pp.x; y.y += pp.y; y.z += pp.z; y.w += pp.w;
+                        reinterpret_cast<float4*>(p.ypos + row[k] * p.D)[c4] = y;
+                    }
+                }
+            }
+        }
+    }
+}
+
+constexpr int LN_TILE_PITCH = 256 + 4;
+constexpr int LN_FUSED_MAX_PARTS = 16;
+
+struct LnNone {};
+struct LnPair { ldetr_ln_args a, b; };
+
+template <int NR>
+__device__ __forceinline__ void ln_fwd_tile(const ldetr_ln_args& q, long row0, int nvalid, bool writer, int wave, int lane, float* tile) {
+    const float inv_keep = q.p_drop > 0.f ? 1.f / (1.f - q.p_drop) : 1.f;
+    const uint64_t seed = q.seed + (q.seed_ptr ? *q.seed_ptr : 0ull);
+#pragma unroll 1
+    for (int pass = 0; pass < NR / 16; pass++) {
+        long row[4], lrow[4];
+        bool wr[4], ok[4];
+#pragma unroll
+        for (int k = 0; k < 4; k++) {
+            const int t = pass * 16 + 4 * k + wave;
+            ok[k] = t < nvalid; row[k] = row0 + t; lrow[k] = ok[k] ? row0 + t : row0; wr[k] = writer && ok[k];
+        }
+        float4 o[4][1];
+        ln_fwd_rows<1, 4, 8>(q, row, lrow, wr, lane, seed, inv_keep, o);
+#pragma unroll
+        for (int k = 0; k < 4; k++)
+            *reinterpret_cast<float4*>(tile + (pass * 16 + 4 * k + wave) * LN_TILE_PITCH + 4 * lane) = ok[k] ? o[k][0] : make_float4(0.f, 0.f, 0.f, 0.f);
+    }
+}
+
+inline int ln_check_fwd(const ldetr_ln_args& p) {
+    LDETR_CHECK(p.r_parts >= 0 && (p.r_parts == 0 || (p.r && p.r_part_stride >= p.rows * p.D)), "layernorm_fwd: bad partial-sum arguments");
+    LDETR_CHECK(p.x && p.gamma && p.beta && p.y, "layernorm_fwd: null pointer");
+    LDETR_CHECK((p.pos == nullptr) == (p.ypos == nullptr) && (!p.pos || p.pos_rows > 0), "layernorm_fwd: pos, pos_rows and ypos go together");
+    LDETR_CHECK(p.D % 4 == 0 && p.D >= 4 && p.D <= 1024, "layernorm_fwd: D must be a multiple of 4 in [4, 1024]");
+    LDETR_CHECK(p.rows >= 0 && p.rows < (1L << 31) - 8, "layernorm_fwd: bad row count");
+    return LDETR_OK;
+}
+
+inline int ln_check_fused(const char* what, const ldetr_ln_args& p, long rows, const float* input, long ld) {
+    if (ln_check_fwd(p)) return LDETR_ERR_UNSUPPORTED;
+    if (p.D != 256 || p.pos || p.ypos || p.r_parts > LN_FUSED_MAX_PARTS) {
+        set_error("%s: a LayerNorm prologue takes D = 256, no position output and at most %d partial sums", what, LN_FUSED_MAX_PARTS);
+        return LDETR_ERR_UNSUPPORTED;
+    }
+    if (p.y == p.x || p.z == p.x || p.y == p.r || p.z == p.r) {
+        set_error("%s: a LayerNorm prologue cannot run in place", what);
+        return LDETR_ERR_UNSUPPORTED;
+    }
+    LDETR_CHECK(p.y == input && ld == 256 && p.rows == rows, "%s: the consumer's input must be the LayerNorm's output y (%ld rows of pitch 256)", what, (long)p.rows);
+    return LDETR_OK;
+}
+
+}
diff --git a/layoutdetr_amd/csrc/mha_small.hip b/layoutdetr_amd/csrc/mha_small.hip
--- a/layoutdetr_amd/csrc/mha_small.hip
+++ b/layoutdetr_amd/csrc/mha_small.hip
@@ -1,4 +1,6 @@
+#include <type_traits>
 #include "ldetr_common.hpp"
+#include "ln_row.hpp"
 #include "../../include/ldetr_hip.h"
 
 namespace ldetr {
@@ -143,7 +145,8 @@
 
 typedef ldetr_mha_cross_args MhaCrossParams;
 
-__global__ __launch_bounds__(256) void mha_cross_fwd_kernel(MhaCrossParams p) {
+template <bool LN>
+__global__ __launch_bounds__(256) void mha_cross_fwd_kernel(MhaCrossParams p, std::conditional_t<LN, ldetr_ln_args, LnNone> ln) {
     constexpr int KP = MS_DH + 4;
     __shared__ float red[4 * 16 * 33];
     __shared__ __attribute__((aligned(16))) float qs[16 * KP], os[16 * MS_OP], Ks[64 * KP], Vs[64 * KP];
@@ -160,12 +163,14 @@
             wo[t][gg] = *reinterpret_cast<const f32x4*>(p.w_out + (long)(16 * (4 * w + t) + li) * MS_D + h * MS_DH + 16 * gg + 4 * g);
     f32x4 xa[4], wb[2][4];
     {
-        const bool rok = li < Lq;
-        const float* xr = p.x + (row0 + (rok ? li : 0)) * p.ldx + 64 * w + 4 * g;
-#pragma unroll
-        for (int gg = 0; gg < 4; gg++) {
-            const f32x4 v = *reinterpret_cast<const f32x4*>(xr + 16 * gg);
-            xa[gg] = rok ? v : f32x4{0.f, 0.f, 0.f, 0.f};
+        if constexpr (!LN) {
+            const bool rok = li < Lq;
+            const float* xr = p.x + (row0 + (rok ? li : 0)) * p.ldx + 64 * w + 4 * g;
+#pragma unroll
+            for (int gg = 0; gg < 4; gg++) {
+                const f32x4 v = *reinterpret_cast<const f32x4*>(xr + 16 * gg);
+                xa[gg] = rok ? v : f32x4{0.f, 0.f, 0.f, 0.f};
+            }
         }
 #pragma unroll
         for (int ct = 0; ct < 2; ct++) {
@@ -196,6 +201,13 @@
         }
     const uint64_t seed = p.seed + ((p.p_drop > 0.f && p.seed_ptr) ? *p.seed_ptr : 0ull);
     __builtin_amdgcn_sched_barrier(0);
+    if constexpr (LN) {
+        __shared__ __attribute__((aligned(16))) float Xs[16 * LN_TILE_PITCH];
+        ln_fwd_tile<16>(ln, row0, Lq, h == 0, w, lane, Xs);
+        __syncthreads();
+#pragma unroll
+        for (int gg = 0; gg < 4; gg++) xa[gg] = *reinterpret_cast<const f32x4*>(Xs + li * LN_TILE_PITCH + 64 * w + 4 * g + 16 * gg);
+    }
 #pragma unroll
     for (int i = 0; i < 2; i++) {
         const int e = tid + 256 * i, row = e >> 3, c4 = (e & 7) * 4;
@@ -809,20 +821,30 @@
     return LDETR_OK;
 }
 
-static int mha_cross_launch(const ldetr_mha_cross_args* a, bool bwd, void* stream) {
-    const char* what = bwd ? "mha_cross_bwd" : "mha_cross_fwd";
+static int mha_cross_launch(const ldetr_ln_args* ln, const ldetr_mha_cross_args* a, bool bwd, void* stream) {
+    const char* what = ln ? "mha_cross_ln_fwd" : (bwd ? "mha_cross_bwd" : "mha_cross_fwd");
     LDETR_CHECK(a != nullptr, "%s: null argument block", what);
     const MhaCrossParams& p = *a;
-    if (int rc = mha_cross_check(what, p, bwd)) return rc;
+    if (int rc = mha_cross_check(what, p, bwd)) return ln ? LDETR_ERR_UNSUPPORTED : rc;
+    if (ln)
+        if (int rc = ln_check_fused(what, *ln, (long)p.B * p.Lq, p.x, p.ldx)) return rc;
     if (p.B == 0) return LDETR_OK;
-    if (bwd) hipLaunchKernelGGL(mha_cross_bwd_kernel, dim3((unsigned)(p.B * MS_H)), dim3(320), 0, (hipStream_t)stream, p);
-    else hipLaunchKernelGGL(mha_cross_fwd_kernel, dim3((unsigned)(p.B * MS_H)), dim3(256), 0, (hipStream_t)stream, p);
+    if (ln) {
+        ldetr_ln_args q = *ln;
+        if (q.r_parts == 0) q.r_bias = nullptr;
+        hipLaunchKernelGGL(mha_cross_fwd_kernel<true>, dim3((unsigned)(p.B * MS_H)), dim3(256), 0, (hipStream_t)stream, p, q);
+    } else if (bwd) hipLaunchKernelGGL(mha_cross_bwd_kernel, dim3((unsigned)(p.B * MS_H)), dim3(320), 0, (hipStream_t)stream, p);
+    else hipLaunchKernelGGL(mha_cross_fwd_kernel<false>, dim3((unsigned)(p.B * MS_H)), dim3(256), 0, (hipStream_t)stream, p, LnNone{});
     count_engine_launch(false);
     return check_launch(what);
 }
 
-extern "C" int ldetr_mha_cross_fwd_f32(const ldetr_mha_cross_args* a, void* stream) { return mha_cross_launch(a, false, stream); }
-extern "C" int ldetr_mha_cross_bwd_f32(const ldetr_mha_cross_args* a, void* stream) { return mha_cross_launch(a, true, stream); }
+extern "C" int ldetr_mha_cross_fwd_f32(const ldetr_mha_cross_args* a, void* stream) { return mha_cross_launch(nullptr, a, false, stream); }
+extern "C" int ldetr_mha_cross_bwd_f32(const ldetr_mha_cross_args* a, void* stream) { return mha_cross_launch(nullptr, a, true, stream); }
+extern "C" int ldetr_mha_cross_ln_fwd_f32(const ldetr_ln_args* ln, const ldetr_mha_cross_args* a, void* stream) {
+    LDETR_CHECK(ln, "mha_cross_ln_fwd: null LayerNorm block");
+    return mha_cross_launch(ln, a, false, stream);
+}
 
 extern "C" int ldetr_wgrad_multi_f32(const ldetr_wgrad_desc* d, int n, void* stream) {
     LDETR_CHECK(d && n >= 1 && n <= 8, "wgrad_multi: 1..8 problems");
diff --git a/layoutdetr_amd/hip/blocks.py b/layoutdetr_amd/hip/blocks.py
--- a/layoutdetr_amd/hip/blocks.py
+++ b/layoutdetr_amd/hip/blocks.py
@@ -9,19 +9,34 @@
 _ENTRIES = {'layernorm_fwd': ('ldetr_layernorm_fwd_group_f32', True), 'layernorm_bwd': ('ldetr_layernorm_bwd_group_f32', True),
             'ffn_fwd': ('ldetr_ffn_fwd_group_f32', True), 'ffn_bwd': ('ldetr_ffn_bwd_group_f32', True),
             'mha_small_fwd': ('ldetr_mha_small_fwd_group_f32', True), 'mha_small_bwd': ('ldetr_mha_small_bwd_group_f32', True),
-            'mha_cross_fwd': ('ldetr_mha_cross_fwd_f32', False), 'mha_cross_bwd': ('ldetr_mha_cross_bwd_f32', False)}
+            'mha_cross_fwd': ('ldetr_mha_cross_fwd_f32', False), 'mha_cross_bwd': ('ldetr_mha_cross_bwd_f32', False),
+            'mha_cross_ln_fwd': ('ldetr_mha_cross_ln_fwd_f32', False), 'ffn_ln_fwd': ('ldetr_ffn_ln_fwd_group_f32', True)}
+LN_FUSED = frozenset(w for w in _ENTRIES if '_ln_' in w)
+LN_FUSED_MAX_PARTS = 16
+LAUNCHES = []
+
+
+def note(what):
+    if LAUNCHES:
+        LAUNCHES[-1].append(what)
 
 
 def launch(what, args, flops=0.0, nbytes=0.0):
     entry, grouped = _ENTRIES[what]
     fn = getattr(core.lib(), entry)
     n = len(args)
-    arr = (type(args[0]) * n)(*args)
+    note(what)
+    if what in LN_FUSED:
+        lns = (_lib.LnArgs * n)(*[ln for ln, _ in args])
+        arr = (type(args[0][1]) * n)(*[a for _, a in args])
+        head = (lns, arr)
+    else:
+        head = ((type(args[0]) * n)(*args),)
     if grouped:
-        call = lambda: core.check(fn(arr, n, core.stream()), what)
+        call = lambda: core.check(fn(*head, n, core.stream()), what)
     else:
         assert n == 1
-        call = lambda: core.check(fn(arr, core.stream()), what)
+        call = lambda: core.check(fn(*head, core.stream()), what)
     if flops > 0:
         core.engine_call('ldetr_token_stack', flops, call, nbytes=nbytes)
     else:
diff --git a/layoutdetr_amd/hip/stacks.py b/layoutdetr_amd/hip/stacks.py
--- a/layoutdetr_amd/hip/stacks.py
+++ b/layoutdetr_amd/hip/stacks.py
@@ -8,6 +8,8 @@
 
 MAX_TOKENS, MAX_ROWS, MAX_CROSS_KEYS = 16, 512, 64
 ENABLED = core.knob('TOKEN_STACKS', 1) != 0
+
+LN_FUSED = core.knob('STACK_LN', 1) != 0
 
 NODE_RUNS = [0]
 
@@ -160,7 +162,7 @@
     sv.p1 = layer.dropout1.p if pr.training else 0.0
     sv.seed1, sv.z1, sv.mean1, sv.rstd1, sv.t1 = blocks.draw_seed(sv.p1), _new(dev, M, D), _new(dev, M), _new(dev, M), _new(dev, M, D)
     r, r_bias, r_parts = s.res
-    blocks.launch('layernorm_fwd', [blocks.ln_fwd(s.cur, r, W.n1_g, W.n1_b, layer.norm1.eps, sv.p1, sv.seed1, sv.t1, sv.z1, sv.mean1, sv.rstd1, r_parts=r_parts, r_bias=r_bias)])
+    norm1 = blocks.ln_fwd(s.cur, r, W.n1_g, W.n1_b, layer.norm1.eps, sv.p1, sv.seed1, sv.t1, sv.z1, sv.mean1, sv.rstd1, r_parts=r_parts, r_bias=r_bias)
     s.cur = sv.t1
     K, V = s.K[i], s.V[i]
     sv.p_c = layer.multihead_attn.dropout if pr.training else 0.0
@@ -170,10 +172,15 @@
                       and K.data_ptr() % 16 == 0 and V.data_ptr() % 16 == 0)
     if sv.cross_small:
         ypart = _new(dev, H, M, D)
-        _launch_sum('mha_cross_fwd', [blocks.mha_cross_fwd(sv.t1, Wq, Bq, K, V, W.ca_w_out, pr.mem_kpm, sv.qc, sv.oc, sv.lse_c, ypart, pr.B, pr.L, pr.S, sv.p_c, sv.seed_c)],
-                    [_fl_cross(pr)])
+        cross = blocks.mha_cross_fwd(sv.t1, Wq, Bq, K, V, W.ca_w_out, pr.mem_kpm, sv.qc, sv.oc, sv.lse_c, ypart, pr.B, pr.L, pr.S, sv.p_c, sv.seed_c)
+        if LN_FUSED:
+            _launch_sum('mha_cross_ln_fwd', [(norm1, cross)], [_fl_cross(pr)])
+        else:
+            blocks.launch('layernorm_fwd', [norm1])
+            _launch_sum('mha_cross_fwd', [cross], [_fl_cross(pr)])
         s.res = (ypart, W.ca_b_out, H)
     else:
+        blocks.launch('layernorm_fwd', [norm1])
         lib = core.lib()
         core.gemm(sv.t1, Wq, 0, 0, M, D, D, out=sv.qc, ep=core.epilogue(col_bias=Bq))
         core.check(lib.ldetr_attention_fwd_f32(
@@ -201,8 +208,12 @@
         ln_b.append(blocks.ln_fwd(sv.x1, parts, W.nb_g, W.nb_b, norm_b.eps, sv.p_b, sv.seed_b, y, sv.zb, sv.mean_b, sv.rstd_b, r_parts=ns, r_bias=W.b2))
         s.keep = (r, parts)
         s.cur, s.res = y, None
-    blocks.launch('layernorm_fwd', ln_a)
-    _launch_sum('ffn_fwd', ffn, [_fl_ffn(s.M, s.saved[i].F) for s in act])
+    costs = [_fl_ffn(s.M, s.saved[i].F) for s in act]
+    if LN_FUSED and all(0 < a.r_parts <= blocks.LN_FUSED_MAX_PARTS for a in ln_a):
+        _launch_sum('ffn_ln_fwd', list(zip(ln_a, ffn)), costs)
+    else:
+        blocks.launch('layernorm_fwd', ln_a)
+        _launch_sum('ffn_fwd', ffn, costs)
     blocks.launch('layernorm_fwd', ln_b)
 
 
@@ -343,6 +354,7 @@
         arr = (_lib.WgradDesc * len(chunk))(*chunk)
         wf = sum(2.0 * d.M * d.rows * d.cols for d in chunk)
         wb = sum(4.0 * (d.M * (d.rows + d.cols) + d.rows * d.cols) for d in chunk)
+        blocks.note('wgrad_multi')
         core.engine_call('ldetr_token_stack', wf, lambda: core.check(lib.ldetr_wgrad_multi_f32(arr, len(chunk), core.stream()), 'wgrad_multi'), nbytes=wb)
 
 
@@ -350,6 +362,7 @@
     if bw.need[1 + s.x_index]:
         g, M = s.g, s.M
         dx = _new(s.dev, M, D_MODEL)
+        blocks.note('sum_parts')
         core.check(core.lib().ldetr_sum_parts_f32(core.ptr(g.res), core.ptr(g.parts), g.n, M * D_MODEL, core.ptr(dx), M * D_MODEL, core.stream()), 'sum_parts')
         bw.grads[1 + s.x_index] = dx.reshape(bw.tensors[s.x_index].shape)
 
```

New measurement: 502.7. -1.7%, worse.
